# mumianyuxin/M3DSSD

Hardware: AMD Instinct MI355X
Metric: images/sec at 1280x384 bs=8, 1/2/4/8 MI355X; 3D-box Linf vs ref (higher is better)
Workload: dtype f32; 1 GPU; BASELINE.json configs[1]: full M3d_inference_align (DLA-34 + DCNv2 align + ANAB) forward + decode + top-3000 + NMS, bs=8/GPU, 1280x384, fp32, random-init synthetic weights and frames; per_gpu_batch=8, global_batch=8, parallelism=dp1 (batch sharded, 1 all-gather of [B,40,14] detections)

## Files before the change

### include/m3dssd_hip.h

```cpp
#ifndef M3DSSD_HIP_H
#define M3DSSD_HIP_H

#include <stdint.h>

#ifdef __cplusplus
extern "C" {
#endif

typedef void *m3d_stream_t;

enum {
    M3D_OK = 0,
    M3D_E_ARG = -1,
    M3D_E_HIP = -2,
    M3D_E_WORKSPACE = -3
};

const char *m3d_last_error(void);
#define M3D_ABI_VERSION 5
int m3d_abi_version(void);
const char *m3d_source_hashes(void);

typedef struct m3d_conv_desc {
    const float *in;
    int in_cs;
    int N, H, W, Cin;
    const float *wgt;
    long long wgt_img_stride;
    int Cout, Cout_pad;
    int kh, kw, stride, pad, dil;
    int Ho, Wo;
    float *out;
    int out_cs;
    int out_nchw;
    long long out_img_stride;
    const float *scale;
    const float *shift;
    const float *res;
    int res_cs;
    int res_mode;
    int act;
    int sigmoid_from;
    const float *dcn_offmask;
    int dcn_om_cs;
    float *splitk_ws;
    long long splitk_ws_bytes;
} m3d_conv_desc;

int m3d_conv2d_forward(const m3d_conv_desc *d, m3d_stream_t stream);
int m3d_conv2d_splitk_plan(const m3d_conv_desc *d, int *splits, long long *ws_bytes);

int m3d_conv_wave_applicable(const m3d_conv_desc *d);
int m3d_conv_wave_splitk_plan(const m3d_conv_desc *d, int *splits, long long *ws_bytes);
int m3d_conv_wave_forward(const m3d_conv_desc *d, m3d_stream_t stream);
int m3d_conv_wave_forward_wgsplit(const m3d_conv_desc *d, m3d_stream_t stream);
int m3d_conv_wave_wgsplit_width(const m3d_conv_desc *d, int *slices, int *width);

int m3d_wino_conv3x3_forward(const m3d_conv_desc *d, m3d_stream_t stream);
int m3d_wino_conv3x3_variant(const m3d_conv_desc *d);
int m3d_wino_conv3x3_splitk_plan(const m3d_conv_desc *d, int *splits, long long *ws_bytes);
int m3d_wino_conv3x3_forward_ex(const m3d_conv_desc *d, int variant, m3d_stream_t stream);
int m3d_wino44_applicable(const m3d_conv_desc *d);
int m3d_wino44_conv3x3_forward(const m3d_conv_desc *d, m3d_stream_t stream);
int m3d_wino44_conv3x3_forward_ex(const m3d_conv_desc *d, int nb, m3d_stream_t stream);
int m3d_wino44_kpair(const m3d_conv_desc *d);
int m3d_wino44_splitk_plan(const m3d_conv_desc *d, int *splits, long long *ws_bytes);
int m3d_wino44_conv3x3_forward_touch(const m3d_conv_desc *d, int nb, const void *touch, long long touch_bytes, m3d_stream_t stream);

int m3d_cache_touch(const void *p, long long bytes, m3d_stream_t stream);
int m3d_upload_indirect(const void *const *src_slot, void *dst, long long bytes, m3d_stream_t stream);

int m3d_conv2d_tile(const m3d_conv_desc *d, int *bm, int *bn, int *bk, int *grid);

typedef struct m3d_conv_bf16_desc {
    const void *in;
    int in_cs;
    int N, H, W, Cin;
    const void *wgt;
    long long wgt_img_stride;
    int Cout, Cout_pad, Kpad;
    int kh, kw, stride, pad;
    int Ho, Wo;
    void *out;
    int out_cs;
    int out_mode;
    long long out_img_stride;
    const float *scale;
    const float *shift;
    const void *res;
    int res_cs;
    int res_mode;
    int act;
    int sigmoid_from;
    const float *dcn_offmask;
    int dcn_om_cs;
    int groups;
    long long in_group_off, wgt_group_off, out_group_off;
    int ss_group_off;
    const void *wgt_f16;
    void *dcn_ws;
    long long dcn_ws_bytes;
    const void *wgt_wave;
} m3d_conv_bf16_desc;
int m3d_conv_bf16_forward(const m3d_conv_bf16_desc *d, m3d_stream_t stream);
long long m3d_conv_bf16_dcn_ws_bytes(int N, int Ho, int Wo);
int m3d_conv_bf16_variant(const m3d_conv_bf16_desc *d);

typedef struct m3d_tree_entry_bf16_desc {
    const void *in;
    int in_cs, N, H, W, Cin, Cout;
    const void *wfrag;
    const float *shift1, *shiftp;
    void *t; int t_cs;
    void *res; int res_cs;
    void *bottom; int bottom_cs;
} m3d_tree_entry_bf16_desc;
int m3d_tree_entry_bf16_applicable(const m3d_tree_entry_bf16_desc *d);
int m3d_tree_entry_bf16_forward(const m3d_tree_entry_bf16_desc *d, m3d_stream_t stream);

typedef struct m3d_head_bf16_desc {
    const void *in;
    int in_cs;
    long long M;
    int Cin;
    const void *w1, *w2, *w3;
    const float *s1, *t1, *s2, *t2, *s3, *t3;
    int Cout, Cout_pad;
    float *out;
    long long out_group_off, out_img_stride;
    int HW;
    int groups;
} m3d_head_bf16_desc;
int m3d_head_mlp_bf16_forward(const m3d_head_bf16_desc *d, m3d_stream_t stream);
typedef struct m3d_head2_bf16_desc {
    const void *in;
    int in_cs;
    long long M;
    const void *w1f, *w2f, *w3;
    const float *t1, *t2, *t3;
    int Cout;
    float *out;
    long long out_group_off, out_img_stride;
    int HW;
    int groups;
} m3d_head2_bf16_desc;
int m3d_head_mlp2_bf16_forward(const m3d_head2_bf16_desc *d, m3d_stream_t stream);
int m3d_head_mlp2_bf16_forward_rows(const m3d_head2_bf16_desc *d, const int *rows, const int *n_rows, m3d_stream_t stream);
typedef struct m3d_tail2_bf16_desc {
    const void *in;
    int in_cs;
    long long M;
    const void *waf, *wbf;
    const float *t1, *t2;
    int Cout;
    float *out;
    long long out_img_stride;
    int HW;
} m3d_tail2_bf16_desc;
int m3d_head_tail2_bf16_forward(const m3d_tail2_bf16_desc *d, m3d_stream_t stream);
typedef struct m3d_qkvs_bf16_desc {
    const void *in;
    int in_cs;
    long long M;
    const void *wf;
    void *q; int q_cs, q_rows;
    void *kv; int kv_cs, kv_rows;
    float *s; int s_cs, s_rows;
} m3d_qkvs_bf16_desc;
int m3d_anab_qkvs_bf16_forward(const m3d_qkvs_bf16_desc *d, m3d_stream_t stream);

int m3d_stem_conv7x7_bf16(const void *img, int is_u8, int img_h, int img_w, const float *mean3, const float *stds3,
                          const float *wgt, const float *scale, const float *shift, void *out, int out_cs, int N, int H, int W,
                          m3d_stream_t stream);
int m3d_frontend2_bf16_forward(const void *img, int is_u8, int img_h, int img_w, const float *mean3, const float *stds3,
                               const void *w_stem_frag, const float *t_stem, const void *w_l0, const float *t_l0,
                               const void *w_l1, const float *t_l1, void *out, int out_cs, int N, int H, int W,
                               m3d_stream_t stream);
int m3d_anab_attend_bf16(const void *q, int q_cs, const void *khat, const void *vhatT, int B, int HW, int Ck_pad, int keys,
                         int keys_pad, int Cv, const void *res, int res_cs, const float *scale, const float *shift, int act,
                         void *out, int out_cs, m3d_stream_t stream);
int m3d_anab_attend_bf16_rows(const void *q, int q_cs, const void *khat, const void *vhatT, int B, int HW, int Ck_pad, int keys,
                              int keys_pad, int Cv, const void *res, int res_cs, const float *scale, const float *shift, int act,
                              void *out, int out_cs, const int *rows, const int *n_rows, m3d_stream_t stream);
int m3d_maxpool2x2_bf16(const void *in, int in_cs, void *out, int out_cs, int N, int H, int W, int C, m3d_stream_t stream);
int m3d_upsample2x_add_bf16(const void *in, int in_cs, const float *wgt , const void *skip, int skip_cs,
                            void *out, int out_cs, int N, int H, int W, int C, m3d_stream_t stream);
int m3d_f32_to_bf16(const float *src, void *dst, long long n , m3d_stream_t stream);
int m3d_softmax_rows_bf16(const float *x, int rows, int valid, int cs, void *out, int out_cs, m3d_stream_t stream);

typedef struct m3d_mlp_desc {
    const float *in;
    int in_cs;
    long long M;
    int Cin;
    const float *w1, *s1, *t1;
    const float *w2, *s2, *t2;
    const float *w3, *s3, *t3;
    int Cout, Cout_pad;
    float *out;
    long long out_img_stride;
    int HW;
} m3d_mlp_desc;
int m3d_head_mlp_forward(const m3d_mlp_desc *d, m3d_stream_t stream);
int m3d_head_mlp_forward_batched(const m3d_mlp_desc *d, int n, m3d_stream_t stream);
int m3d_head_mlp_forward_rows(const m3d_mlp_desc *d, int n, const int *rows, const int *n_rows, unsigned int sparse_head_mask,
                              m3d_stream_t stream);

long long m3d_dcn_v2_workspace_bytes(int batch, int channels, int height, int width, int channels_out,
                                     int kernel_h, int kernel_w, int stride, int pad, int dilation);
long long m3d_dcn_v2_workspace_bytes_grouped(int batch, int channels, int height, int width, int channels_out,
                                             int kernel_h, int kernel_w, int stride, int pad, int dilation,
                                             int deformable_group);
int m3d_dcn_v2_forward(const float *input, const float *weight, const float *bias, const float *offset,
                       const float *mask, float *output, int batch, int channels, int height, int width,
                       int channels_out, int kernel_h, int kernel_w, int stride_h, int stride_w, int pad_h,
                       int pad_w, int dilation_h, int dilation_w, int deformable_group, void *workspace,
                       long long workspace_bytes, m3d_stream_t stream);

long long m3d_dcn_v2_backward_workspace_bytes(int batch, int channels, int height, int width, int channels_out,
                                              int kernel_h, int kernel_w, int stride, int pad, int dilation,
                                              int deformable_group);
int m3d_dcn_v2_backward(const float *input, const float *weight, const float *offset, const float *mask,
                        const float *grad_output,
                        float *grad_input, float *grad_offset, float *grad_mask, float *grad_weight, float *grad_bias,
                        int batch, int channels, int height, int width, int channels_out, int kernel_h, int kernel_w,
                        int stride_h, int stride_w, int pad_h, int pad_w, int dilation_h, int dilation_w,
                        int deformable_group, void *workspace, long long workspace_bytes, m3d_stream_t stream);

long long m3d_dcn_v2_workspace_bytes_bf16(int batch, int channels, int height, int width, int channels_out,
                                          int kernel_h, int kernel_w, int stride, int pad, int dilation, int deformable_group);
int m3d_dcn_v2_forward_bf16(const void *input, const void *weight, const float *bias, const void *offset, int offset_is_bf16,
                            const void *mask, int mask_is_bf16, void *output, int batch, int channels, int height, int width,
                            int channels_out, int kernel_h, int kernel_w, int stride_h, int stride_w, int pad_h, int pad_w,
                            int dilation_h, int dilation_w, int deformable_group, void *workspace, long long workspace_bytes,
                            m3d_stream_t stream);
long long m3d_dcn_v2_backward_workspace_bytes_bf16(int batch, int channels, int height, int width, int channels_out,
                                                   int kernel_h, int kernel_w, int stride, int pad, int dilation,
                                                   int deformable_group);
int m3d_dcn_v2_backward_bf16(const void *input, const void *weight, const void *offset, int offset_is_bf16, const void *mask,
                             int mask_is_bf16, const void *grad_output,
                             void *grad_input, float *grad_offset, float *grad_mask, void *grad_weight, float *grad_bias,
                             int batch, int channels, int height, int width, int channels_out, int kernel_h, int kernel_w,
                             int stride_h, int stride_w, int pad_h, int pad_w, int dilation_h, int dilation_w,
                             int deformable_group, void *workspace, long long workspace_bytes, m3d_stream_t stream);

long long m3d_dcn_v2_psroi_pooling_workspace_bytes(int batch, int channels, int height, int width, int num_rois,
                                                   int num_classes, int output_dim, int group_size, int pooled_size,
                                                   int backward);
int m3d_dcn_v2_psroi_pooling_forward(const float *data, const float *rois, const float *trans, float *out, float *top_count,
                                     int batch, int channels, int height, int width, int num_rois, int trans_rows,
                                     int num_classes, int no_trans, float spatial_scale, int output_dim, int group_size,
                                     int pooled_size, int part_size, int sample_per_part, float trans_std, void *workspace,
                                     long long workspace_bytes, m3d_stream_t stream);
int m3d_dcn_v2_psroi_pooling_backward(const float *grad_out, const float *data, const float *rois, const float *trans,
                                      float *grad_data, float *grad_trans, int batch, int channels, int height, int width,
                                      int num_rois, int trans_rows, int num_classes, int no_trans, float spatial_scale,
                                      int output_dim, int group_size, int pooled_size, int part_size, int sample_per_part,
                                      float trans_std, void *workspace, long long workspace_bytes, m3d_stream_t stream);

#define M3D_RPN_MAX_GT 128
#define M3D_RPN_GT_COLS 12
enum {
    M3D_RPN_CONF_MEANS = 0,
    M3D_RPN_CONF_STDS = 11,
    M3D_RPN_CONF_FG_THRESH = 22,
    M3D_RPN_CONF_IGN_THRESH = 23,
    M3D_RPN_CONF_BG_LO = 24,
    M3D_RPN_CONF_BG_HI = 25,
    M3D_RPN_CONF_BEST_THRESH = 26,
    M3D_RPN_CONF_BOX_SAMPLES = 27,
    M3D_RPN_CONF_FG_FRACTION = 28,
    M3D_RPN_CONF_FOCAL = 29,
    M3D_RPN_CONF_LAMBDA_CLS = 30,
    M3D_RPN_CONF_LAMBDA_IOU = 31,
    M3D_RPN_CONF_LAMBDA_2D = 32,
    M3D_RPN_CONF_LAMBDA_3D = 33,
    M3D_RPN_CONF_STRIDE = 34,
    M3D_RPN_CONF_COUNT = 35
};
enum {
    M3D_RPN_STAT_LOSS = 0,
    M3D_RPN_STAT_CLS = 1,
    M3D_RPN_STAT_BBOX_2D = 2,
    M3D_RPN_STAT_BBOX_3D = 3,
    M3D_RPN_STAT_IOU_LOSS = 4,
    M3D_RPN_STAT_Z = 5,
    M3D_RPN_STAT_RY = 6,
    M3D_RPN_STAT_IOU_ACC = 7,
    M3D_RPN_STAT_ACC_FG = 8,
    M3D_RPN_STAT_ACC_BG = 9,
    M3D_RPN_STAT_N_FG = 10,
    M3D_RPN_STAT_N_BG = 11,
    M3D_RPN_STAT_FG_NUM = 12,
    M3D_RPN_STAT_BG_NUM = 13,
    M3D_RPN_STAT_N_ACTIVE = 14,
    M3D_RPN_STAT_FG_WEIGHT = 15,
    M3D_RPN_STAT_COUNT = 16
};
long long m3d_rpn_loss_workspace_bytes(int B, long long R);
int m3d_rpn_targets(const double *anchors, int A, int H, int W, const double *conf, int n_conf, const double *gt_table, int B,
                    int Gmax, const float *cls, const float *prob, int C, short *labels, short *gt_index, float *targets,
                    float *scores, void *workspace, long long workspace_bytes, m3d_stream_t stream);
int m3d_rpn_loss(const double *anchors, int A, int H, int W, const double *conf, int n_conf, const double *gt_table, int B,
                 int Gmax, const float *cls, const float *bbox_2d, const float *bbox_3d, int C, const short *labels,
                 const float *targets, const float *scores, unsigned char *sampled, float *grad_cls, float *grad_bbox_2d,
                 float *grad_bbox_3d, float *loss, double *stats, void *workspace, long long workspace_bytes,
                 m3d_stream_t stream);

enum {
    M3D_RPN_SMP_STAT_BAD_LABELS = 16,
    M3D_RPN_SMP_STAT_COUNT = 17
};
int m3d_rpn_precompute_targets(const double *anchors, int A, int H, int W, const double *conf, int n_conf,
                               const double *gt_table, int B, int Gmax, short *labels, short *gt_index, float *bbox_2d_tar,
                               float *bbox_3d_tar, int *any_val, void *workspace, long long workspace_bytes,
                               m3d_stream_t stream);
int m3d_rpn_loss_smp(const double *anchors, int A, int H, int W, const double *conf, int n_conf, int B, const void *labels_in,
                     int label_bytes, const float *bbox_2d_tar, const float *bbox_3d_tar, const int *any_val, const float *cls,
                     const float *prob, const float *bbox_2d, const float *bbox_3d, int C, short *labels, float *targets,
                     float *scores, unsigned char *sampled, float *grad_cls, float *grad_bbox_2d, float *grad_bbox_3d,
                     float *loss, double *stats, void *workspace, long long workspace_bytes, m3d_stream_t stream);

#define M3D_RPN_TARGET_STATS_COLS 23
long long m3d_rpn_target_stats_workspace_bytes(int B, long long R);
int m3d_rpn_target_stats(const double *anchors, int A, int H, int W, const double *conf, int n_conf, const double *gt_table, int B,
                         int Gmax, const double *center, double *out, void *workspace, long long workspace_bytes,
                         m3d_stream_t stream);

int m3d_pack_conv_weight(const float *w, float *packed, int Cout, int Cout_pad, int Cin, int Cin_pad, int kh,
                         int kw, m3d_stream_t stream);
int m3d_nchw_to_nhwc(const float *in, float *out, int N, int C, int H, int W, int out_cs, m3d_stream_t stream);
int m3d_nhwc_to_nchw(const float *in, int in_cs, float *out, int N, int C, int H, int W, m3d_stream_t stream);

int m3d_stem_conv7x7(const float *img_nchw, const float *wgt , const float *scale,
                     const float *shift, float *out, int out_cs, int N, int H, int W, m3d_stream_t stream);
int m3d_preprocess_u8(const unsigned char *frames_bgr, int N, int img_h, int img_w, const float *mean3, const float *stds3,
                      float *out_nchw, int H, int W, m3d_stream_t stream);
int m3d_stem_conv7x7_u8(const unsigned char *frames_bgr, int img_h, int img_w, const float *mean3, const float *stds3,
                        const float *wgt, const float *scale, const float *shift, float *out, int out_cs, int N, int H, int W,
                        m3d_stream_t stream);
#define M3D_AUGMENT_PARAMS 14
int m3d_augment_u8(const unsigned char *frames_bgr, int N, int hmax, int wmax, const double *params, int param_stride,
                   const float *mean3, const float *stds3, float *out_nchw, int H, int W, m3d_stream_t stream);
int m3d_conv3x3_c16(const float *in, int in_cs, const float *wgt, const float *scale, const float *shift, float *out,
                    int out_cs, int N, int H, int W, m3d_stream_t stream);
int m3d_conv3x3_c16_wino(const float *in, int in_cs, const float *U, const float *scale, const float *shift, float *out,
                         int out_cs, int N, int H, int W, m3d_stream_t stream);
int m3d_maxpool2x2(const float *in, int in_cs, float *out, int out_cs, int N, int H, int W, int C,
                   m3d_stream_t stream);
int m3d_upsample2x_add(const float *in, int in_cs, const float *wgt, const float *skip, int skip_cs,
                       float *out, int out_cs, int N, int H, int W, int C, m3d_stream_t stream);

int m3d_anchor_select(const float *cls_planar, int B, int A, int num_classes, int HW, int *sel_idx,
                      float *sel_prob, float *fg_all, m3d_stream_t stream);
int m3d_anchor_select_keys(const float *cls_planar, int B, int A, int HW, int *sel_idx, float *sel_prob,
                           unsigned int *score_bits, m3d_stream_t stream);
int m3d_fg_top1(const float *prob, int B, int A, int HW, int *idx, float *val, m3d_stream_t stream);
int m3d_align_offsets(int mode, const int *sel_idx, const float *sel_prob, float thresh, const float *table,
                      const float *bbox_x, const float *bbox_y, const float *anchor_wh, float mean_x,
                      float std_x, float mean_y, float std_y, float *offmask, int om_cs, int B, int A, int HW,
                      int kk, long long box_img_stride, m3d_stream_t stream);
int m3d_align_offsets_gated(const int *sel_idx, const float *sel_prob, float thresh, const float *bbox_x, const float *bbox_y,
                            const float *anchor_wh, float mean_x, float std_x, float mean_y, float std_y,
                            const unsigned char *need, float *offmask, int om_cs, int B, int A, int HW,
                            long long box_img_stride, m3d_stream_t stream);

int m3d_anab_pool_partial(const float *kv, int kv_cs, const float *s, int s_cs, const int *items, int n_items,
                          const int *bin_scale, int n_bins, float *partial, int max_slots, int B, int H, int W,
                          int C, m3d_stream_t stream);
int m3d_anab_pool_finish(const float *partial, const int *bin_slots, const float *bin_inv_area, int n_bins,
                         int max_slots, int Ck, int Cv, float *khat, int keys_pad, int ck_pad, float *vhatT,
                         int B, int frag, m3d_stream_t stream);
long long m3d_anab_pool_nested_scratch_bytes(int B, int C);
int m3d_anab_pool_nested(const float *kv, int kv_cs, const float *s, int s_cs, int B, int H, int W, int Ck, int Cv,
                         float *scratch, float *khat, int keys_pad, int ck_pad, float *vhatT, int frag, m3d_stream_t stream);
int m3d_anab_pool_nested_bf16(const void *kv, int kv_cs, const float *s, int s_cs, int B, int H, int W, int Ck, int Cv,
                              float *scratch, float *khat, int keys_pad, int ck_pad, float *vhatT, int frag, m3d_stream_t stream);
int m3d_anab_pool_nested_bf16_ex(const void *kv, int kv_cs, const float *s, int s_cs, int B, int H, int W, int Ck, int Cv,
                                 float *scratch, float *khat, int keys_pad, int ck_pad, float *vhatT, int frag,
                                 void *khat16, void *vhat16, m3d_stream_t stream);
int m3d_anab_attend_f32(const float *q, int q_cs, const float *khat, int k_cs, const float *vhatT, int B, int HW, int Ck,
                        int keys, int keys_pad, int Cv, const float *res, int res_cs, int res_mode, const float *scale,
                        const float *shift, int act, float *out, int out_cs, m3d_stream_t stream);
int m3d_anab_attend_f32_rows(const float *q, int q_cs, const float *khat, int k_cs, const float *vhatT, int B, int HW, int Ck,
                             int keys, int keys_pad, int Cv, const float *res, int res_cs, int res_mode, const float *scale,
                             const float *shift, int act, float *out, int out_cs, const int *rows, const int *n_rows,
                             m3d_stream_t stream);
long long m3d_anab_attention_workspace_bytes(int B, int H, int W, int Ck, int Cv, int backward);
int m3d_anab_attention_forward(const float *q, const float *k, const float *v, const float *g, float *out, int B, int H, int W, int Ck,
                               int Cv, int q_cs, int k_cs, int v_cs, int g_cs, int out_cs, void *workspace, long long workspace_bytes,
                               m3d_stream_t stream);
int m3d_anab_attention_backward(const float *q, const float *k, const float *v, const float *g, const float *grad_out, float *grad_q,
                                float *grad_k, float *grad_v, float *grad_g, int B, int H, int W, int Ck, int Cv, int q_cs, int k_cs,
                                int v_cs, int g_cs, int go_cs, int gq_cs, int gk_cs, int gv_cs, int gg_cs, void *workspace,
                                long long workspace_bytes, m3d_stream_t stream);
long long m3d_anab_attention_workspace_bytes_bf16(int B, int H, int W, int Ck, int Cv, int backward);
int m3d_anab_attention_forward_bf16(const void *q, const void *k, const void *v, const void *g, void *out, int B, int H, int W, int Ck,
                                    int Cv, int q_cs, int k_cs, int v_cs, int g_cs, int out_cs, void *workspace,
                                    long long workspace_bytes, m3d_stream_t stream);
int m3d_anab_attention_backward_bf16(const void *q, const void *k, const void *v, const void *g, const void *grad_out, void *grad_q,
                                     void *grad_k, void *grad_v, void *grad_g, int B, int H, int W, int Ck, int Cv, int q_cs, int k_cs,
                                     int v_cs, int g_cs, int go_cs, int gq_cs, int gk_cs, int gv_cs, int gg_cs, void *workspace,
                                     long long workspace_bytes, m3d_stream_t stream);
int m3d_softmax_rows(float *x, int rows, int valid, int cs, m3d_stream_t stream);

int m3d_bundle_outputs(const float *cls_planar, const float *box_planar, float *cls, float *prob, float *bbox_2d,
                       float *bbox_3d, unsigned int *score_bits, int B, int A, int HW, m3d_stream_t stream);
int m3d_score_keys_planar(const float *cls_planar, unsigned int *score_bits, int B, int A, int HW, m3d_stream_t stream);
long long m3d_topk_decode_workspace_bytes(int B, int R);
int m3d_topk_decode(const unsigned int *score_bits, const float *prob, const float *bbox_2d, const float *bbox_3d,
                    const float *rois , const float *anchors , const float *means ,
                    const float *stds , float *aboxes, int *rows_out, void *workspace, long long workspace_bytes,
                    int B, int R, int k, m3d_stream_t stream);
int m3d_topk_decode_scaled(const unsigned int *score_bits, const float *prob, const float *bbox_2d, const float *bbox_3d,
                           const float *rois, const float *anchors, const float *means, const float *stds, const float *scale,
                           float *aboxes, int *rows_out, void *workspace, long long workspace_bytes, int B, int R, int k,
                           m3d_stream_t stream);
int m3d_topk_decode_planar(const unsigned int *score_bits, const float *cls_planar, const float *box_planar, const float *rois,
                           const float *anchors, const float *means, const float *stds, const float *scale, float *aboxes,
                           int *rows_out, void *workspace, long long workspace_bytes, int B, int A, int HW, int k,
                           m3d_stream_t stream);
long long m3d_topk_decode_mw_workspace_bytes(int B, int R, int k);
int m3d_topk_decode_planar_mw(const unsigned int *score_bits, const float *cls_planar, const float *box_planar, const float *rois,
                              const float *anchors, const float *means, const float *stds, const float *scale, float *aboxes,
                              int *rows_out, void *workspace, long long workspace_bytes, int B, int A, int HW, int k,
                              int wgs_per_image, m3d_stream_t stream);
long long m3d_need_rows_workspace_bytes(int B, int HW);
int m3d_need_rows(const unsigned int *score_bits, int B, int A, int HW, int k, unsigned int *thresh, unsigned char *need,
                  int *rows, int *n_rows, void *workspace, long long workspace_bytes, m3d_stream_t stream);
int m3d_decode_rows(const long long *rows , const float *prob, const float *bbox_2d,
                    const float *bbox_3d, const float *rois , const float *anchors ,
                    const float *means , const float *stds , float *aboxes, int B, int R,
                    int n_rows, m3d_stream_t stream);

long long m3d_nms_workspace_bytes(int B, int n);
int m3d_nms_sorted_dev(const float *boxes_dev, int B, int n, int box_stride, float thresh, void *mask_ws,
                       int *keep_dev, int *num_keep_dev, m3d_stream_t stream);
int m3d_select_post(const float *aboxes , const int *keep , const int *num_keep , int B, int n,
                    int post, float *block, int *counts, m3d_stream_t stream);
void _nms(int *keep_out, int *num_out, const float *boxes_host, int boxes_num, int boxes_dim,
          float nms_overlap_thresh, int device_id);

int m3d_refine_3d(const float *aboxes, const int *counts, int B, int K, const double *p2, const double *p2_inv,
                  double score_thresh, int hill_climbing, double step_r_init, double r_lim, double *out, m3d_stream_t stream);
int m3d_refine_3d_ex(const float *aboxes, const int *counts, int B, int K, const double *p2, const double *p2_inv,
                     const float *scale, const float *clip_wh, double score_thresh, int hill_climbing, double step_r_init,
                     double r_lim, double *out, m3d_stream_t stream);
int m3d_refine_3d_host(const float *aboxes, const int *counts, int B, int K, const double *p2, const double *p2_inv,
                       const float *scale, const float *clip_wh, double score_thresh, int hill_climbing, double step_r_init,
                       double r_lim, double *out);

int m3d_rotate_iou_eval(const float *boxes_dev, int N, const float *qboxes_dev, int K, int criterion, float *iou_dev,
                        m3d_stream_t stream);
int m3d_eval_image_box_overlap(const double *boxes, int N, const double *q, int K, int criterion, double *out);
int m3d_eval_d3_overlap(const double *boxes, int N, const double *qboxes, int K, double *rinc, int criterion);
int m3d_eval_statistics(const double *overlaps, long long ov_stride, const double *gt_datas, int gt_size, const double *dt_datas,
                        int det_size, const long long *ignored_gt, const long long *ignored_det, const double *dc_bboxes, int n_dc,
                        int metric, double min_overlap, double thresh, int compute_fp, int compute_aos, double *stats,
                        double *thresholds_out, int *n_thresholds);
int m3d_eval_fused_statistics(const double *overlaps, long long ov_stride, double *pr, const long long *gt_nums,
                              const long long *dt_nums, const long long *dc_nums, int n_images, const double *gt_datas,
                              const double *dt_datas, const double *dontcares, const long long *ignored_gts,
                              const long long *ignored_dets, int metric, double min_overlap, const double *thresholds,
                              int n_thresholds, int compute_aos);

int m3d_clock_probe(long long *out4_dev, double seconds, m3d_stream_t stream);
int m3d_event_create(void **ev);
int m3d_event_record(void *ev, m3d_stream_t stream);
int m3d_event_elapsed_ms(void *start, void *stop, float *ms);
int m3d_event_destroy(void *ev);

#ifdef __cplusplus
}
#endif
#endif
```

### m3dssd_amd/_hip.py

```python
import ctypes
import os
import subprocess

_HERE = os.path.dirname(os.path.abspath(__file__))
CSRC = os.path.join(_HERE, "csrc")
SO_PATH = os.environ.get("M3D_HIP_LIB") or os.path.join(CSRC, "build", "libm3dssd_hip.so")
HEADER = os.path.join(os.path.dirname(_HERE), "include", "m3dssd_hip.h")

c_int, c_float, c_ll, c_void_p = ctypes.c_int, ctypes.c_float, ctypes.c_longlong, ctypes.c_void_p


class ConvDesc(ctypes.Structure):
    _fields_ = [
        ("inp", c_void_p), ("in_cs", c_int),
        ("N", c_int), ("H", c_int), ("W", c_int), ("Cin", c_int),
        ("wgt", c_void_p), ("wgt_img_stride", c_ll),
        ("Cout", c_int), ("Cout_pad", c_int),
        ("kh", c_int), ("kw", c_int), ("stride", c_int), ("pad", c_int), ("dil", c_int),
        ("Ho", c_int), ("Wo", c_int),
        ("out", c_void_p), ("out_cs", c_int), ("out_nchw", c_int), ("out_img_stride", c_ll),
        ("scale", c_void_p), ("shift", c_void_p),
        ("res", c_void_p), ("res_cs", c_int), ("res_mode", c_int),
        ("act", c_int), ("sigmoid_from", c_int),
        ("dcn_offmask", c_void_p), ("dcn_om_cs", c_int),
        ("splitk_ws", c_void_p), ("splitk_ws_bytes", c_ll),
    ]


class MlpDesc(ctypes.Structure):
    _fields_ = [
        ("inp", c_void_p), ("in_cs", c_int), ("M", c_ll), ("Cin", c_int),
        ("w1", c_void_p), ("s1", c_void_p), ("t1", c_void_p),
        ("w2", c_void_p), ("s2", c_void_p), ("t2", c_void_p),
        ("w3", c_void_p), ("s3", c_void_p), ("t3", c_void_p),
        ("Cout", c_int), ("Cout_pad", c_int),
        ("out", c_void_p), ("out_img_stride", c_ll), ("HW", c_int),
    ]


class ConvBf16Desc(ctypes.Structure):
    _fields_ = [
        ("inp", c_void_p), ("in_cs", c_int),
        ("N", c_int), ("H", c_int), ("W", c_int), ("Cin", c_int),
        ("wgt", c_void_p), ("wgt_img_stride", c_ll),
        ("Cout", c_int), ("Cout_pad", c_int), ("Kpad", c_int),
        ("kh", c_int), ("kw", c_int), ("stride", c_int), ("pad", c_int),
        ("Ho", c_int), ("Wo", c_int),
        ("out", c_void_p), ("out_cs", c_int), ("out_mode", c_int), ("out_img_stride", c_ll),
        ("scale", c_void_p), ("shift", c_void_p),
        ("res", c_void_p), ("res_cs", c_int), ("res_mode", c_int),
        ("act", c_int), ("sigmoid_from", c_int),
        ("dcn_offmask", c_void_p), ("dcn_om_cs", c_int),
        ("groups", c_int),
        ("in_group_off", c_ll), ("wgt_group_off", c_ll), ("out_group_off", c_ll),
        ("ss_group_off", c_int),
        ("wgt_f16", c_void_p), ("dcn_ws", c_void_p), ("dcn_ws_bytes", c_ll),
        ("wgt_wave", c_void_p),
    ]


class HeadBf16Desc(ctypes.Structure):
    _fields_ = [
        ("inp", c_void_p), ("in_cs", c_int), ("M", c_ll), ("Cin", c_int),
        ("w1", c_void_p), ("w2", c_void_p), ("w3", c_void_p),
        ("s1", c_void_p), ("t1", c_void_p), ("s2", c_void_p), ("t2", c_void_p), ("s3", c_void_p), ("t3", c_void_p),
        ("Cout", c_int), ("Cout_pad", c_int),
        ("out", c_void_p), ("out_group_off", c_ll), ("out_img_stride", c_ll),
        ("HW", c_int), ("groups", c_int),
    ]


class Head2Bf16Desc(ctypes.Structure):
    _fields_ = [
        ("inp", c_void_p), ("in_cs", c_int), ("M", c_ll),
        ("w1f", c_void_p), ("w2f", c_void_p), ("w3", c_void_p),
        ("t1", c_void_p), ("t2", c_void_p), ("t3", c_void_p),
        ("Cout", c_int),
        ("out", c_void_p), ("out_group_off", c_ll), ("out_img_stride", c_ll),
        ("HW", c_int), ("groups", c_int),
    ]


class Tail2Bf16Desc(ctypes.Structure):
    _fields_ = [
        ("inp", c_void_p), ("in_cs", c_int), ("M", c_ll),
        ("waf", c_void_p), ("wbf", c_void_p), ("t1", c_void_p), ("t2", c_void_p),
        ("Cout", c_int),
        ("out", c_void_p), ("out_img_stride", c_ll),
        ("HW", c_int),
    ]


class TreeEntryBf16Desc(ctypes.Structure):
    _fields_ = [
        ("inp", c_void_p), ("in_cs", c_int), ("N", c_int), ("H", c_int), ("W", c_int), ("Cin", c_int), ("Cout", c_int),
        ("wfrag", c_void_p), ("shift1", c_void_p), ("shiftp", c_void_p),
        ("t", c_void_p), ("t_cs", c_int), ("res", c_void_p), ("res_cs", c_int), ("bottom", c_void_p), ("bottom_cs", c_int),
    ]


class QkvsBf16Desc(ctypes.Structure):
    _fields_ = [
        ("inp", c_void_p), ("in_cs", c_int), ("M", c_ll), ("wf", c_void_p),
        ("q", c_void_p), ("q_cs", c_int), ("q_rows", c_int),
        ("kv", c_void_p), ("kv_cs", c_int), ("kv_rows", c_int),
        ("s", c_void_p), ("s_cs", c_int), ("s_rows", c_int),
    ]


P = c_void_p
SIGNATURES = {
    "m3d_last_error": (ctypes.c_char_p, []),
    "m3d_abi_version": (c_int, []),
    "m3d_source_hashes": (ctypes.c_char_p, []),
    "m3d_conv2d_forward": (c_int, [ctypes.POINTER(ConvDesc), P]),
    "m3d_conv_bf16_forward": (c_int, [ctypes.POINTER(ConvBf16Desc), P]),
    "m3d_conv_bf16_dcn_ws_bytes": (c_ll, [c_int, c_int, c_int]),
    "m3d_conv_bf16_variant": (c_int, [ctypes.POINTER(ConvBf16Desc)]),
    "m3d_head_mlp_bf16_forward": (c_int, [ctypes.POINTER(HeadBf16Desc), P]),
    "m3d_head_mlp2_bf16_forward": (c_int, [ctypes.POINTER(Head2Bf16Desc), P]),
    "m3d_head_mlp2_bf16_forward_rows": (c_int, [ctypes.POINTER(Head2Bf16Desc), P, P, P]),
    "m3d_tree_entry_bf16_applicable": (c_int, [ctypes.POINTER(TreeEntryBf16Desc)]),
    "m3d_tree_entry_bf16_forward": (c_int, [ctypes.POINTER(TreeEntryBf16Desc), P]),
    "m3d_anab_qkvs_bf16_forward": (c_int, [ctypes.POINTER(QkvsBf16Desc), P]),
    "m3d_head_tail2_bf16_forward": (c_int, [ctypes.POINTER(Tail2Bf16Desc), P]),
    "m3d_stem_conv7x7_bf16": (c_int, [P, c_int, c_int, c_int, ctypes.POINTER(ctypes.c_float), ctypes.POINTER(ctypes.c_float),
                                      P, P, P, P, c_int, c_int, c_int, c_int, P]),
    "m3d_frontend2_bf16_forward": (c_int, [P, c_int, c_int, c_int, ctypes.POINTER(ctypes.c_float), ctypes.POINTER(ctypes.c_float)]
                                   + [P] * 7 + [c_int] * 4 + [P]),
    "m3d_anab_attend_bf16": (c_int, [P, c_int, P, P, c_int, c_int, c_int, c_int, c_int, c_int, P, c_int, P, P, c_int, P, c_int, P]),
    "m3d_anab_attend_bf16_rows": (c_int, [P, c_int, P, P, c_int, c_int, c_int, c_int, c_int, c_int, P, c_int, P, P, c_int, P, c_int,
                                          P, P, P]),
    "m3d_maxpool2x2_bf16": (c_int, [P, c_int, P, c_int] + [c_int] * 4 + [P]),
    "m3d_upsample2x_add_bf16": (c_int, [P, c_int, P, P, c_int, P, c_int] + [c_int] * 4 + [P]),
    "m3d_f32_to_bf16": (c_int, [P, P, c_ll, P]),
    "m3d_softmax_rows_bf16": (c_int, [P, c_int, c_int, c_int, P, c_int, P]),
    "m3d_head_mlp_forward": (c_int, [ctypes.POINTER(MlpDesc), P]),
    "m3d_head_mlp_forward_batched": (c_int, [ctypes.POINTER(MlpDesc), c_int, P]),
    "m3d_head_mlp_forward_rows": (c_int, [ctypes.POINTER(MlpDesc), c_int, P, P, ctypes.c_uint, P]),
    "m3d_wino_conv3x3_forward": (c_int, [ctypes.POINTER(ConvDesc), P]),
    "m3d_wino_conv3x3_forward_ex": (c_int, [ctypes.POINTER(ConvDesc), c_int, P]),
    "m3d_wino_conv3x3_splitk_plan": (c_int, [ctypes.POINTER(ConvDesc), ctypes.POINTER(c_int), ctypes.POINTER(c_ll)]),
    "m3d_wino_conv3x3_variant": (c_int, [ctypes.POINTER(ConvDesc)]),
    "m3d_wino44_applicable": (c_int, [ctypes.POINTER(ConvDesc)]),
    "m3d_wino44_conv3x3_forward": (c_int, [ctypes.POINTER(ConvDesc), P]),
    "m3d_wino44_conv3x3_forward_ex": (c_int, [ctypes.POINTER(ConvDesc), c_int, P]),
    "m3d_wino44_kpair": (c_int, [ctypes.POINTER(ConvDesc)]),
    "m3d_wino44_conv3x3_forward_touch": (c_int, [ctypes.POINTER(ConvDesc), c_int, P, c_ll, P]),
    "m3d_cache_touch": (c_int, [P, c_ll, P]),
    "m3d_upload_indirect": (c_int, [P, P, c_ll, P]),
    "m3d_wino44_splitk_plan": (c_int, [ctypes.POINTER(ConvDesc), ctypes.POINTER(c_int), ctypes.POINTER(c_ll)]),
    "m3d_conv_wave_applicable": (c_int, [ctypes.POINTER(ConvDesc)]),
    "m3d_conv_wave_splitk_plan": (c_int, [ctypes.POINTER(ConvDesc), ctypes.POINTER(c_int), ctypes.POINTER(c_ll)]),
    "m3d_conv_wave_forward": (c_int, [ctypes.POINTER(ConvDesc), P]),
    "m3d_conv_wave_forward_wgsplit": (c_int, [ctypes.POINTER(ConvDesc), P]),
    "m3d_conv_wave_wgsplit_width": (c_int, [ctypes.POINTER(ConvDesc), ctypes.POINTER(c_int), ctypes.POINTER(c_int)]),
    "m3d_conv2d_tile": (c_int, [ctypes.POINTER(ConvDesc)] + [ctypes.POINTER(c_int)] * 4),
    "m3d_conv2d_splitk_plan": (c_int, [ctypes.POINTER(ConvDesc), ctypes.POINTER(c_int), ctypes.POINTER(c_ll)]),
    "m3d_dcn_v2_workspace_bytes": (c_ll, [c_int] * 10),
    "m3d_dcn_v2_workspace_bytes_grouped": (c_ll, [c_int] * 11),
    "m3d_dcn_v2_forward": (c_int, [P] * 6 + [c_int] * 14 + [P, c_ll, P]),
    "m3d_dcn_v2_backward_workspace_bytes": (c_ll, [c_int] * 11),
    "m3d_dcn_v2_backward": (c_int, [P] * 10 + [c_int] * 14 + [P, c_ll, P]),
    "m3d_dcn_v2_workspace_bytes_bf16": (c_ll, [c_int] * 11),
    "m3d_dcn_v2_forward_bf16": (c_int, [P, P, P, P, c_int, P, c_int, P] + [c_int] * 14 + [P, c_ll, P]),
    "m3d_dcn_v2_backward_workspace_bytes_bf16": (c_ll, [c_int] * 11),
    "m3d_dcn_v2_backward_bf16": (c_int, [P, P, P, c_int, P, c_int, P] + [P] * 5 + [c_int] * 14 + [P, c_ll, P]),
    "m3d_dcn_v2_psroi_pooling_workspace_bytes": (c_ll, [c_int] * 10),
    "m3d_dcn_v2_psroi_pooling_forward": (c_int, [P] * 5 + [c_int] * 8 + [c_float] + [c_int] * 5 + [c_float, P, c_ll, P]),
    "m3d_dcn_v2_psroi_pooling_backward": (c_int, [P] * 6 + [c_int] * 8 + [c_float] + [c_int] * 5 + [c_float, P, c_ll, P]),
    "m3d_rpn_loss_workspace_bytes": (c_ll, [c_int, c_ll]),
    "m3d_rpn_targets": (c_int, [P, c_int, c_int, c_int, P, c_int, P, c_int, c_int, P, P, c_int, P, P, P, P, P, c_ll, P]),
    "m3d_rpn_loss": (c_int, [P, c_int, c_int, c_int, P, c_int, P, c_int, c_int, P, P, P, c_int, P, P, P, P, P, P, P, P, P, P, c_ll, P]),
    "m3d_rpn_precompute_targets": (c_int, [P, c_int, c_int, c_int, P, c_int, P, c_int, c_int, P, P, P, P, P, P, c_ll, P]),
    "m3d_rpn_loss_smp": (c_int, [P, c_int, c_int, c_int, P, c_int, c_int, P, c_int, P, P, P, P, P, P, P, c_int] + [P] * 10 + [c_ll, P]),
    "m3d_rpn_target_stats_workspace_bytes": (c_ll, [c_int, c_ll]),
    "m3d_rpn_target_stats": (c_int, [P, c_int, c_int, c_int, P, c_int, P, c_int, c_int, P, P, P, c_ll, P]),
    "m3d_pack_conv_weight": (c_int, [P, P] + [c_int] * 6 + [P]),
    "m3d_nchw_to_nhwc": (c_int, [P, P] + [c_int] * 5 + [P]),
    "m3d_nhwc_to_nchw": (c_int, [P, c_int, P] + [c_int] * 4 + [P]),
    "m3d_stem_conv7x7": (c_int, [P, P, P, P, P] + [c_int] * 4 + [P]),
    "m3d_refine_3d": (c_int, [P, P, c_int, c_int, P, P, ctypes.c_double, c_int, ctypes.c_double, ctypes.c_double, P, P]),
    "m3d_refine_3d_ex": (c_int, [P, P, c_int, c_int, P, P, P, P, ctypes.c_double, c_int, ctypes.c_double, ctypes.c_double, P, P]),
    "m3d_refine_3d_host": (c_int, [P, P, c_int, c_int, P, P, P, P, ctypes.c_double, c_int, ctypes.c_double, ctypes.c_double, P]),
    "m3d_preprocess_u8": (c_int, [P, c_int, c_int, c_int, ctypes.POINTER(ctypes.c_float), ctypes.POINTER(ctypes.c_float), P, c_int,
                                  c_int, P]),
    "m3d_augment_u8": (c_int, [P, c_int, c_int, c_int, ctypes.POINTER(ctypes.c_double), c_int, ctypes.POINTER(ctypes.c_float),
                               ctypes.POINTER(ctypes.c_float), P, c_int, c_int, P]),
    "m3d_stem_conv7x7_u8": (c_int, [P, c_int, c_int, ctypes.POINTER(ctypes.c_float), ctypes.POINTER(ctypes.c_float), P, P, P, P,
                                    c_int, c_int, c_int, c_int, P]),
    "m3d_conv3x3_c16": (c_int, [P, c_int, P, P, P, P, c_int, c_int, c_int, c_int, P]),
    "m3d_conv3x3_c16_wino": (c_int, [P, c_int, P, P, P, P, c_int, c_int, c_int, c_int, P]),
    "m3d_maxpool2x2": (c_int, [P, c_int, P, c_int] + [c_int] * 4 + [P]),
    "m3d_upsample2x_add": (c_int, [P, c_int, P, P, c_int, P, c_int] + [c_int] * 4 + [P]),
    "m3d_anchor_select": (c_int, [P] + [c_int] * 4 + [P, P, P, P]),
    "m3d_anchor_select_keys": (c_int, [P] + [c_int] * 3 + [P, P, P, P]),
    "m3d_fg_top1": (c_int, [P, c_int, c_int, c_int, P, P, P]),
    "m3d_align_offsets": (c_int, [c_int, P, P, c_float, P, P, P, P] + [c_float] * 4 + [P] + [c_int] * 5 + [c_ll, P]),
    "m3d_align_offsets_gated": (c_int, [P, P, c_float, P, P, P] + [c_float] * 4 + [P, P] + [c_int] * 4 + [c_ll, P]),
    "m3d_anab_pool_partial": (c_int, [P, c_int, P, c_int, P, c_int, P, c_int, P] + [c_int] * 5 + [P]),
    "m3d_anab_pool_finish": (c_int, [P, P, P] + [c_int] * 4 + [P, c_int, c_int, P, c_int, c_int, P]),
    "m3d_anab_pool_nested_scratch_bytes": (c_ll, [c_int, c_int]),
    "m3d_anab_pool_nested": (c_int, [P, c_int, P, c_int, c_int, c_int, c_int, c_int, c_int, P, P, c_int, c_int, P, c_int, P]),
    "m3d_anab_attend_f32": (c_int, [P, c_int, P, c_int, P, c_int, c_int, c_int, c_int, c_int, c_int, P, c_int, c_int, P, P, c_int, P, c_int, P]),
    "m3d_anab_attend_f32_rows": (c_int, [P, c_int, P, c_int, P, c_int, c_int, c_int, c_int, c_int, c_int, P, c_int, c_int, P, P, c_int, P, c_int,
                                         P, P, P]),
    "m3d_anab_pool_nested_bf16": (c_int, [P, c_int, P, c_int, c_int, c_int, c_int, c_int, c_int, P, P, c_int, c_int, P, c_int, P]),
    "m3d_anab_pool_nested_bf16_ex": (c_int, [P, c_int, P, c_int, c_int, c_int, c_int, c_int, c_int, P, P, c_int, c_int, P, c_int, P, P, P]),
    "m3d_anab_attention_workspace_bytes": (c_ll, [c_int] * 6),
    "m3d_anab_attention_forward": (c_int, [P] * 5 + [c_int] * 10 + [P, c_ll, P]),
    "m3d_anab_attention_backward": (c_int, [P] * 9 + [c_int] * 14 + [P, c_ll, P]),
    "m3d_anab_attention_workspace_bytes_bf16": (c_ll, [c_int] * 6),
    "m3d_anab_attention_forward_bf16": (c_int, [P] * 5 + [c_int] * 10 + [P, c_ll, P]),
    "m3d_anab_attention_backward_bf16": (c_int, [P] * 9 + [c_int] * 14 + [P, c_ll, P]),
    "m3d_softmax_rows": (c_int, [P, c_int, c_int, c_int, P]),
    "m3d_bundle_outputs": (c_int, [P] * 7 + [c_int] * 3 + [P]),
    "m3d_decode_rows": (c_int, [P] * 9 + [c_int] * 3 + [P]),
    "m3d_topk_decode_workspace_bytes": (c_ll, [c_int, c_int]),
    "m3d_topk_decode": (c_int, [P] * 11 + [c_ll] + [c_int] * 3 + [P]),
    "m3d_topk_decode_scaled": (c_int, [P] * 12 + [c_ll] + [c_int] * 3 + [P]),
    "m3d_score_keys_planar": (c_int, [P, P, c_int, c_int, c_int, P]),
    "m3d_topk_decode_planar": (c_int, [P] * 11 + [c_ll] + [c_int] * 4 + [P]),
    "m3d_topk_decode_mw_workspace_bytes": (c_ll, [c_int, c_int, c_int]),
    "m3d_need_rows_workspace_bytes": (c_ll, [c_int, c_int]),
    "m3d_need_rows": (c_int, [P] + [c_int] * 4 + [P] * 5 + [c_ll, P]),
    "m3d_topk_decode_planar_mw": (c_int, [P] * 11 + [c_ll] + [c_int] * 5 + [P]),
    "m3d_select_post": (c_int, [P] * 3 + [c_int] * 3 + [P, P, P]),
    "m3d_nms_workspace_bytes": (c_ll, [c_int, c_int]),
    "m3d_nms_sorted_dev": (c_int, [P, c_int, c_int, c_int, c_float, P, P, P, P]),
    "_nms": (None, [P, P, P, c_int, c_int, c_float, c_int]),
    "m3d_rotate_iou_eval": (c_int, [P, c_int, P, c_int, c_int, P, P]),
    "m3d_eval_image_box_overlap": (c_int, [P, c_int, P, c_int, c_int, P]),
    "m3d_eval_d3_overlap": (c_int, [P, c_int, P, c_int, P, c_int]),
    "m3d_eval_statistics": (c_int, [P, c_ll, P, c_int, P, c_int, P, P, P, c_int, c_int, ctypes.c_double, ctypes.c_double,
                                    c_int, c_int, P, P, ctypes.POINTER(c_int)]),
    "m3d_eval_fused_statistics": (c_int, [P, c_ll, P, P, P, P, c_int, P, P, P, P, P, c_int, ctypes.c_double, P, c_int, c_int]),
    "m3d_clock_probe": (c_int, [P, ctypes.c_double, P]),
    "m3d_event_create": (c_int, [ctypes.POINTER(c_void_p)]),
    "m3d_event_record": (c_int, [P, P]),
    "m3d_event_elapsed_ms": (c_int, [P, P, ctypes.POINTER(c_float)]),
    "m3d_event_destroy": (c_int, [P]),
}

_lib = None


def build(force=False, verbose=False):
    jobs = min(16, int(os.environ.get("MAX_JOBS") or 0) or os.cpu_count() or 4)
    cmd = ["make", "-C", CSRC, "-j", str(jobs)] + (["-B"] if force else [])
    res = subprocess.run(cmd, stdout=subprocess.PIPE, stderr=subprocess.STDOUT, text=True)
    if verbose or res.returncode != 0:
        print(res.stdout)
    if res.returncode != 0:
        raise RuntimeError("building libm3dssd_hip.so failed")
    return SO_PATH


def lib():
    global _lib
    if _lib is None:
        if not os.path.exists(SO_PATH):
            raise RuntimeError(
                "libm3dssd_hip.so is missing (%s): run `python -c 'import __graft_entry__ as g; g.build()'`; "
                "there is no non-HIP fallback for the M3DSSD hot path" % SO_PATH)
        import torch
        L = ctypes.CDLL(SO_PATH)
        for name, (res, args) in SIGNATURES.items():
            fn = getattr(L, name)
            fn.restype, fn.argtypes = res, args
        _lib = L
    return _lib


def lib_source_hashes():
    txt = lib().m3d_source_hashes().decode()
    return dict(item.split(":", 1) for item in txt.split(";") if item)


def tree_source_hashes():
    import hashlib
    files = [os.path.join(CSRC, f) for f in sorted(os.listdir(CSRC)) if f.endswith(".hip") or f.endswith(".h")] + [HEADER]
    return {os.path.basename(f): hashlib.sha256(open(f, "rb").read()).hexdigest()[:16] for f in files}


def check(status):
    if status != 0:
        raise RuntimeError("m3dssd_hip error %d: %s" % (status, lib().m3d_last_error().decode()))
```

### m3dssd_amd/csrc/common.h

```cpp
#pragma once
#include <hip/hip_runtime.h>
#include <stdarg.h>
#include <stdio.h>

#include <algorithm>

#include "m3dssd_hip.h"
#include "per_device.h"

typedef float f32x4 __attribute__((ext_vector_type(4)));
typedef float f32x16 __attribute__((ext_vector_type(16)));
typedef float f32x2 __attribute__((ext_vector_type(2)));
typedef unsigned u32x4 __attribute__((ext_vector_type(4)));

__device__ __forceinline__ int sign_smear(int x)
{
    int m;
    asm("v_ashrrev_i32 %0, 31, %1" : "=v"(m) : "v"(x));
    return m;
}
__device__ __forceinline__ void dcn_corners(float h_im, float w_im, int H, int W, int drop_all, float (&w)[4], int (&o)[4],
                                            int (&drop)[4])
{
    const float tin = fminf(fminf(h_im, w_im) + 1.f, -fmaxf(h_im - (float)H, w_im - (float)W));
    const unsigned xin = __float_as_uint(tin);
    const unsigned nonfinite = __float_as_uint((h_im - h_im) + (w_im - w_im)) & 0x7fffffffu;
    const int out = sign_smear((int)((xin - 1u) | xin)) | sign_smear(-(int)nonfinite) | drop_all;
    const int hl = (int)floorf(h_im), wl = (int)floorf(w_im);
    const float lh = h_im - (float)hl, lw = w_im - (float)wl;
    const float uh = 1.f - lh, uw = 1.f - lw;
    const int hr = (int)((unsigned)(H - 2) - (unsigned)hl), wr = (int)((unsigned)(W - 2) - (unsigned)wl);
    drop[0] = sign_smear(hl | wl) | out;
    drop[1] = sign_smear(hl | wr) | out;
    drop[2] = sign_smear(hr | wl) | out;
    drop[3] = sign_smear(hr | wr) | out;
    const unsigned row0 = (unsigned)__mul24(hl, W) + (unsigned)wl, row1 = row0 + (unsigned)W;
    o[0] = (int)row0; o[1] = (int)(row0 + 1u); o[2] = (int)row1; o[3] = (int)(row1 + 1u);
    const float wf[4] = {uh * uw, uh * lw, lh * uw, lh * lw};
#pragma unroll
    for (int q = 0; q < 4; ++q) w[q] = __uint_as_float(__float_as_uint(wf[q]) & ~(unsigned)drop[q]);
}

#define M3D_BUF_OOB 0x80000000u
__device__ __forceinline__ __amdgpu_buffer_rsrc_t make_rsrc(const void *base, unsigned bytes)
{
    return __builtin_amdgcn_make_buffer_rsrc(const_cast<void *>(base), 0, bytes, 0x00020000);
}
__device__ __forceinline__ void buf_store_f32x4_nop(f32x4 v, __amdgpu_buffer_rsrc_t r, unsigned voffset, unsigned soffset)
{
    asm volatile("buffer_store_dwordx4 %0, %1, %2, %3 offen\n\ts_nop 1" : : "v"(v), "v"(voffset), "s"(r), "s"(soffset) : "memory");
}
__device__ __forceinline__ void global_store_u32x4_nop(void *p, u32x4 v)
{
    asm volatile("global_store_dwordx4 %0, %1, off\n\ts_nop 1" : : "v"(p), "v"(v) : "memory");
}

__device__ __forceinline__ f32x4 buf_load_f32x4(__amdgpu_buffer_rsrc_t r, unsigned voffset, unsigned soffset)
{
    return __builtin_bit_cast(f32x4, __builtin_amdgcn_raw_buffer_load_b128(r, voffset, soffset, 0));
}
__device__ __forceinline__ f32x2 pk_sub2(f32x2 a, f32x2 b)
{
    f32x2 r;
    asm("v_pk_add_f32 %0, %1, %2 neg_lo:[0,1] neg_hi:[0,1]" : "=v"(r) : "v"(a), "v"(b));
    return r;
}
__device__ __forceinline__ f32x4 pk_sub(f32x4 a, f32x4 b)
{
    const f32x2 lo = pk_sub2(__builtin_shufflevector(a, a, 0, 1), __builtin_shufflevector(b, b, 0, 1));
    const f32x2 hi = pk_sub2(__builtin_shufflevector(a, a, 2, 3), __builtin_shufflevector(b, b, 2, 3));
    return __builtin_shufflevector(lo, hi, 0, 1, 2, 3);
}
__device__ __forceinline__ f32x4 pk_mul_s(float w, f32x4 x)
{
    const f32x2 w2 = {w, w};
    const f32x2 lo = w2 * __builtin_shufflevector(x, x, 0, 1), hi = w2 * __builtin_shufflevector(x, x, 2, 3);
    return __builtin_shufflevector(lo, hi, 0, 1, 2, 3);
}
__device__ __forceinline__ f32x4 pk_fma_s(float w, f32x4 x, f32x4 c)
{
    const f32x2 w2 = {w, w};
    const f32x2 lo = __builtin_elementwise_fma(w2, __builtin_shufflevector(x, x, 0, 1), __builtin_shufflevector(c, c, 0, 1));
    const f32x2 hi = __builtin_elementwise_fma(w2, __builtin_shufflevector(x, x, 2, 3), __builtin_shufflevector(c, c, 2, 3));
    return __builtin_shufflevector(lo, hi, 0, 1, 2, 3);
}
__device__ __forceinline__ f32x4 pk_add(f32x4 a, f32x4 b)
{
    const f32x2 lo = __builtin_shufflevector(a, a, 0, 1) + __builtin_shufflevector(b, b, 0, 1);
    const f32x2 hi = __builtin_shufflevector(a, a, 2, 3) + __builtin_shufflevector(b, b, 2, 3);
    return __builtin_shufflevector(lo, hi, 0, 1, 2, 3);
}

#define M3D_LEAKY_SLOPE 0.01f

void m3d_set_error(const char *fmt, ...);
int m3d_nchw_to_nhwc_slice(const float *in, int Ctot, int c0, float *out, int N, int C, int H, int W, int out_cs, m3d_stream_t stream);
int m3d_pack_conv_weight_slice(const float *w, int Ctot, int c0, float *packed, int Cout, int Cout_pad, int Cin, int Cin_pad, int kh,
                               int kw, m3d_stream_t stream);

#define M3D_REQUIRE(cond, ...)        \
    do {                              \
        if (!(cond)) {                \
            m3d_set_error(__VA_ARGS__); \
            return M3D_E_ARG;         \
        }                             \
    } while (0)

#define M3D_HIP(call)                                                             \
    do {                                                                          \
        hipError_t e__ = (call);                                                  \
        if (e__ != hipSuccess) {                                                  \
            m3d_set_error("%s failed: %s (%s:%d)", #call, hipGetErrorString(e__), \
                          __FILE__, __LINE__);                                    \
            return M3D_E_HIP;                                                     \
        }                                                                         \
    } while (0)

#define M3D_LAUNCH_CHECK()                                                          \
    do {                                                                            \
        hipError_t e__ = hipGetLastError();                                         \
        if (e__ != hipSuccess) {                                                    \
            m3d_set_error("kernel launch failed: %s (%s:%d)", hipGetErrorString(e__), \
                          __FILE__, __LINE__);                                      \
            return M3D_E_HIP;                                                       \
        }                                                                           \
    } while (0)

typedef PerDevice<int> m3d_lds_state;
int m3d_raise_dyn_lds_(const void *kernel, int bytes, m3d_lds_state &state, const char *what, const char *file, int line);
#define m3d_raise_dyn_lds(kernel, bytes, state) \
    m3d_raise_dyn_lds_(reinterpret_cast<const void *>(kernel), bytes, state, #kernel, __FILE__, __LINE__)
int m3d_cu_count();
int m3d_scratch_bytes_(const void *const *kernels, int n);
template <typename... K>
static inline int m3d_scratch_bytes(K... kernels)
{
    const void *const k[] = {reinterpret_cast<const void *>(kernels)...};
    return m3d_scratch_bytes_(k, (int)sizeof...(K));
}
int m3d_env_int(const char *name, int dflt);
static inline int m3d_knob_ablate() { static const int v = m3d_env_int("M3D_ABLATE", 0); return v; }

static inline int cdiv(long long a, long long b) { return (int)((a + b - 1) / b); }
static inline int imin(int a, int b) { return a < b ? a : b; }

__device__ __forceinline__ float leaky(float v) { return fmaxf(v, v * M3D_LEAKY_SLOPE); }
__device__ __forceinline__ float sigmoidf_(float v) { return 1.0f / (1.0f + expf(-v)); }

template <typename T>
__device__ __forceinline__ T conv_epi_affine(T v, T sc, T sh, T rv, bool has_res, int res_mode)
{
    if (has_res) return res_mode ? (v + rv) * sc + sh : v * sc + sh + rv;
    return v * sc + sh;
}
__device__ __forceinline__ float conv_epi_act(float v, bool sig, float slope) { return sig ? sigmoidf_(v) : fmaxf(v, v * slope); }
__device__ __forceinline__ f32x4 conv_epi_act4(f32x4 v, int c0, int sigmoid_from, bool any_sig, float slope)
{
    if (any_sig) {
#pragma unroll
        for (int e = 0; e < 4; ++e) v[e] = conv_epi_act(v[e], c0 + e >= sigmoid_from, slope);
        return v;
    }
    return __builtin_elementwise_max(v, v * slope);
}

__device__ __forceinline__ f32x4 class_softmax4(f32x4 l)
{
    const float mx = fmaxf(fmaxf(l[0], l[1]), fmaxf(l[2], l[3]));
    f32x4 e;
    float s = 0.f;
#pragma unroll
    for (int c = 0; c < 4; ++c) { e[c] = expf(l[c] - mx); s += e[c]; }
    f32x4 pr;
#pragma unroll
    for (int c = 0; c < 4; ++c) pr[c] = e[c] / s;
    return pr;
}
__device__ __forceinline__ float fg_score(f32x4 pr) { return fmaxf(fmaxf(pr[1], pr[2]), pr[3]); }
__device__ __forceinline__ unsigned int f32_sortable(float f)
{
    unsigned int u = __float_as_uint(f);
    return (u & 0x80000000u) ? ~u : (u | 0x80000000u);
}

__device__ __forceinline__ int rows_lower_bound(const int *rows, const int n, const int target)
{
    const int lane = threadIdx.x & 63;
    int lo = 0, len = n;
    while (len > 0) {
        const int step = (len + 63) >> 6;
        const int idx = lo + (lane + 1) * step - 1;
        const bool less = idx < lo + len && rows[idx] < target;
        const int c = __popcll(__ballot(less));
        const int end = lo + len;
        lo += c * step;
        len = min(step - 1, end - lo);
    }
    return __builtin_amdgcn_readfirstlane(lo);
}

struct SplitkReduceArgs {
    const float *ws, *scale, *shift, *res;
    float *out;
    int M, Cout, Cout_pad, splits, out_cs, res_cs, res_mode, act, sigmoid_from;
};
int m3d_launch_splitk_reduce(const SplitkReduceArgs &a, hipStream_t stream);
```

### m3dssd_amd/csrc/dcn_wave.hip

```cpp

#include <type_traits>

#include "common.h"

struct ConvWaveArgs {
    const float *in, *wfrag, *scale, *shift, *res, *om;
    float *out;
    int in_cs, out_cs, res_cs, om_cs;
    int H, W, Cin, Ho, Wo, HoWo, Cout;
    int kh, kw, stride, pad, dil;
    int M, KG, tiles_n;
    int act, res_mode, sigmoid_from;
    int vec_out;
    long long w_img_stride;
    unsigned in_bytes, out_bytes, res_bytes, w_bytes;
    float *ws;
    int splits, ss_per, base_waves;
    unsigned ws_bytes;
#ifdef CONV_TRACE
    long long *trace;
#endif
};


#ifdef CONV_TRACE
static long long *g_conv_trace = nullptr;
extern "C" void m3d_conv_wave_set_trace(void *buf) { g_conv_trace = (long long *)buf; }
static int g_conv_variant = 0;
extern "C" void m3d_conv_wave_set_variant(int v) { g_conv_variant = v; }
#define TRACE_INIT() long long *trp = (a.trace && threadIdx.x < 64) ? a.trace + (size_t)blockIdx.x * 128 : nullptr; int tri = 0
#define TRACE() do { if (trp && lane == 0 && tri < 128) trp[tri++] = __builtin_readcyclecounter(); } while (0)
#else
#define TRACE_INIT()
#define TRACE()
#endif

template <bool DEFORM, int NT, int NCQ = 4, int WPE = (DEFORM ? 2 : 3), int S = 1>
__global__ __launch_bounds__(64 * S) __attribute__((amdgpu_waves_per_eu(WPE))) void conv_wave_kernel(const ConvWaveArgs a)
{
    __shared__ __attribute__((aligned(16))) float tileS[S * 32 * 32];
    __shared__ __attribute__((aligned(16))) float tapst[(DEFORM ? 9 : 1) * 32 * 8];
    const int lane = threadIdx.x & 63, l31 = lane & 31, h = lane >> 5;
    const int wv = S > 1 ? __builtin_amdgcn_readfirstlane((int)threadIdx.x >> 6) : 0;
    float *const tileA = tileS + wv * 1024;
    const int gp = lane >> 3, gc = lane & 7;
    TRACE_INIT();
    TRACE();
    int blk;
    {
        const int nblk = gridDim.x, bid = blockIdx.x;
        const int q = nblk >> 3, r = nblk & 7, xcd = bid & 7, loc = bid >> 3;
        blk = (xcd < r ? xcd * (q + 1) : r * (q + 1) + (xcd - r) * q) + loc;
    }
    int split = wv;
    if (S == 1 && a.splits > 1) {
        split = blk / a.base_waves;
        blk -= split * a.base_waves;
    }
    const int bm = blk / a.tiles_n, bn = blk - bm * a.tiles_n;
    const int m0 = bm * 32;
    const int KK = a.kh * a.kw, C32 = a.Cin / 32;
    const bool idle = S > 1 && wv >= a.splits;
    const int ss0 = idle ? 0 : split * a.ss_per, ss1 = idle ? 0 : min(KK * C32, ss0 + a.ss_per);

    const __amdgpu_buffer_rsrc_t rin = make_rsrc(a.in, a.in_bytes);
    const __amdgpu_buffer_rsrc_t rw =
        make_rsrc(a.wfrag + (size_t)(m0 / a.HoWo) * a.w_img_stride + (size_t)bn * NT * a.KG * 256, a.w_bytes);
    const unsigned wlane = (unsigned)lane * 16u;
    const unsigned wstride = (unsigned)a.KG * 1024u;

    int o_pix = 0, o_hi0 = 0, o_wi0 = 0;
    bool o_valid = false;
    int o_inv = -1;
    const float *o_om = a.om;
    int g_pix[4], g_hi0[4], g_wi0[4];
    bool g_valid[4];
    {
        const int m = m0 + l31;
        o_valid = m < a.M;
        o_inv = sign_smear(a.M - 1 - m);
        const int mm = o_valid ? m : 0;
        const int n = mm / a.HoWo, rem = mm - n * a.HoWo;
        const int ho = rem / a.Wo, wo = rem - ho * a.Wo;
        o_pix = n * a.H * a.W;
        o_hi0 = ho * a.stride - a.pad;
        o_wi0 = wo * a.stride - a.pad;
        if (DEFORM) o_om = a.om + (size_t)mm * a.om_cs;
    }
    if constexpr (!DEFORM) {
#pragma unroll
        for (int g = 0; g < 4; ++g) {
            const int m = m0 + 8 * g + gp;
            g_valid[g] = m < a.M;
            const int mm = g_valid[g] ? m : 0;
            const int n = mm / a.HoWo, rem = mm - n * a.HoWo;
            const int ho = rem / a.Wo, wo = rem - ho * a.Wo;
            g_pix[g] = n * a.H * a.W;
            g_hi0[g] = ho * a.stride - a.pad;
            g_wi0[g] = wo * a.stride - a.pad;
        }
    }

    unsigned doff[4][DEFORM ? 4 : 1];
    float bw[DEFORM ? 4 : 1][4];
    if constexpr (DEFORM) {
        constexpr int TPW = (9 + S - 1) / S;
        float raws[TPW][3];
#pragma unroll
        for (int i = 0; i < TPW; ++i) {
            const int tp = min(wv + i * S, KK - 1);
            raws[i][0] = o_om[2 * tp];
            raws[i][1] = o_om[2 * tp + 1];
            raws[i][2] = o_om[2 * KK + tp];
        }
#pragma unroll
        for (int i = 0; i < TPW; ++i) {
            const int t = wv + i * S;
            if (t < KK) {
                const int ti = t / a.kw, tj = t - ti * a.kw;
                const float mk = raws[i][2];
                const float h_im = (float)(o_hi0 + ti * a.dil) + raws[i][0];
                const float w_im = (float)(o_wi0 + tj * a.dil) + raws[i][1];
                float wq[4];
                int oq[4], drop[4];
                dcn_corners(h_im, w_im, a.H, a.W, o_inv, wq, oq, drop);
                u32x4 ob;
#pragma unroll
                for (int q = 0; q < 4; ++q) {
                    const unsigned off = ((unsigned)o_pix + (unsigned)oq[q]) * (unsigned)a.in_cs * 4u;
                    ob[q] = (off & ~(unsigned)drop[q]) | (M3D_BUF_OOB & (unsigned)drop[q]);
                }
                if (h == 0) {
                    *reinterpret_cast<u32x4 *>(&tapst[t * 256 + l31 * 8]) = ob;
                    *reinterpret_cast<f32x4 *>(&tapst[t * 256 + l31 * 8 + 4]) = f32x4{wq[0] * mk, wq[1] * mk, wq[2] * mk, wq[3] * mk};
                }
            }
        }
        if constexpr (S > 1) __syncthreads();
    }
    auto setup_tap = [&](int tap) {
        if constexpr (DEFORM) {
#pragma unroll
            for (int g = 0; g < 4; ++g) {
                const u32x4 ov = *reinterpret_cast<const u32x4 *>(&tapst[tap * 256 + (8 * g + gp) * 8]);
                const f32x4 wv = *reinterpret_cast<const f32x4 *>(&tapst[tap * 256 + (8 * g + gp) * 8 + 4]);
#pragma unroll
                for (int q = 0; q < 4; ++q) {
                    doff[g][q] = ov[q] + (unsigned)gc * 16u;
                    bw[g][q] = wv[q];
                }
            }
        } else {
            const int ti = tap / a.kw, tj = tap - ti * a.kw;
#pragma unroll
            for (int g = 0; g < 4; ++g) {
                const int hi = g_hi0[g] + ti * a.dil, wi = g_wi0[g] + tj * a.dil;
                const bool ok = g_valid[g] && hi >= 0 && hi < a.H && wi >= 0 && wi < a.W;
                doff[g][0] = ok ? ((unsigned)(g_pix[g] + hi * a.W + wi) * (unsigned)a.in_cs + (unsigned)gc * 4u) * 4u
                                : M3D_BUF_OOB;
            }
        }
    };

    constexpr int NC = DEFORM ? NCQ : 1;
    f32x4 cr[4][NC];
    f32x4 bfA[NT], bfB[NT];
    auto issue_gather = [&](int c32) {
#pragma unroll
        for (int g = 0; g < 4; ++g)
#pragma unroll
            for (int q = 0; q < NC; ++q) cr[g][q] = buf_load_f32x4(rin, doff[g][q], (unsigned)c32 * 128u);
    };
    auto issue_b = [&](int kg, f32x4 (&bf)[NT]) {
        const unsigned bsoff = (unsigned)min(kg, a.KG - 1) * 1024u;
#pragma unroll
        for (int nt = 0; nt < NT; ++nt) bf[nt] = buf_load_f32x4(rw, wlane, bsoff + nt * wstride);
    };

    f32x16 acc[NT];
#pragma unroll
    for (int nt = 0; nt < NT; ++nt)
#pragma unroll
        for (int r = 0; r < 16; ++r) acc[nt][r] = 0.f;

    int tap, c32;
    constexpr bool cmaj = DEFORM;
    if constexpr (cmaj) { c32 = ss0 / KK; tap = ss0 - c32 * KK; }
    else { tap = ss0 / C32; c32 = ss0 - tap * C32; }
    setup_tap(tap);
    issue_gather(c32);
    issue_b((tap * C32 + c32) * 4, bfA);

    unsigned wr_off[4], rd_off[4];
#pragma unroll
    for (int g = 0; g < 4; ++g) {
        const int r = 8 * g + gp;
        wr_off[g] = (unsigned)(r * 32 + ((gc ^ ((r >> 1) & 7)) * 4));
    }
#pragma unroll
    for (int j = 0; j < 4; ++j) rd_off[j] = (unsigned)(l31 * 32 + (((2 * j + h) ^ ((l31 >> 1) & 7)) * 4));

    TRACE();
    for (int st = ss0; st < ss1; ++st) {
        TRACE();
        const int kg0 = (tap * C32 + c32) * 4;
#pragma unroll
        for (int g = 0; g < 4; ++g) {
            f32x4 v;
            if constexpr (DEFORM && NCQ == 4)
                v = pk_fma_s(bw[g][0], cr[g][0], pk_fma_s(bw[g][1], cr[g][1], pk_fma_s(bw[g][2], cr[g][2], pk_mul_s(bw[g][3], cr[g][3]))));
            else if constexpr (DEFORM && NCQ == 2)
                v = pk_fma_s(bw[g][0], cr[g][0], pk_mul_s(bw[g][1], cr[g][1]));
            else if constexpr (DEFORM)
                v = pk_mul_s(bw[g][0], cr[g][0]);
            else
                v = cr[g][0];
            *reinterpret_cast<f32x4 *>(&tileA[wr_off[g]]) = v;
        }
        if constexpr (cmaj) {
            if (++tap == KK) { tap = 0; ++c32; }
            setup_tap(tap);
            issue_gather(min(c32, C32 - 1));
        } else {
            if (++c32 == C32) {
                c32 = 0;
                ++tap;
                setup_tap(min(tap, KK - 1));
            }
            issue_gather(c32);
        }
        const int kgn = (min(tap, KK - 1) * C32 + min(c32, C32 - 1)) * 4;
        TRACE();
        f32x4 A[4];
#pragma unroll
        for (int j = 0; j < 4; ++j) A[j] = *reinterpret_cast<const f32x4 *>(&tileA[rd_off[j]]);
        __builtin_amdgcn_sched_barrier(0);
        auto group = [&](int j, int kg_next, f32x4 (&bf)[NT], f32x4 (&bfn)[NT]) {
            issue_b(kg_next, bfn);
            __builtin_amdgcn_sched_barrier(0);
#pragma unroll
            for (int t = 0; t < 4; ++t)
#pragma unroll
                for (int nt = 0; nt < NT; ++nt)
                    acc[nt] = __builtin_amdgcn_mfma_f32_32x32x2f32(A[j][t], bf[nt][t], acc[nt], 0, 0, 0);
            __builtin_amdgcn_sched_barrier(0);
        };
        group(0, kg0 + 1, bfA, bfB);
        group(1, kg0 + 2, bfB, bfA);
        group(2, kg0 + 3, bfA, bfB);
        group(3, kgn, bfB, bfA);
    }

    TRACE();
    const __amdgpu_buffer_rsrc_t rout = make_rsrc(a.out, a.out_bytes);
    const __amdgpu_buffer_rsrc_t rres = make_rsrc(a.res ? a.res : a.out, a.res ? a.res_bytes : 0u);
    const int n0 = bn * 32 * NT;
    const int mb = m0 + 4 * h;
    if constexpr (S > 1) {
        constexpr int Q = S == 2 ? 2 : 1;
        const int tid = threadIdx.x;
        const bool worker = S < 8 || wv < 4;
        const float slope = a.act == 1 ? M3D_LEAKY_SLOPE : 1.f;
        const int c4 = lane & 7;
        int px[Q];
        unsigned oq[Q], rq[Q];
#pragma unroll
        for (int q = 0; q < Q; ++q) {
            px[q] = ((tid + q * 64 * S) >> 3) & 31;
            const int m = m0 + px[q];
            const bool ok = worker && m < a.M;
            oq[q] = ok ? (unsigned)m * (unsigned)a.out_cs * 4u : M3D_BUF_OOB;
            rq[q] = ok ? (unsigned)m * (unsigned)a.res_cs * 4u : M3D_BUF_OOB;
        }
        f32x4 scv[NT], shv[NT];
#pragma unroll
        for (int nt = 0; nt < NT; ++nt) {
            const int c = n0 + nt * 32 + 4 * c4;
            scv[nt] = f32x4{1.f, 1.f, 1.f, 1.f};
            shv[nt] = f32x4{0.f, 0.f, 0.f, 0.f};
            if (a.vec_out && c + 3 < a.Cout) {
                if (a.scale) scv[nt] = *reinterpret_cast<const f32x4 *>(a.scale + c);
                if (a.shift) shv[nt] = *reinterpret_cast<const f32x4 *>(a.shift + c);
            } else {
#pragma unroll
                for (int e = 0; e < 4; ++e)
                    if (c + e < a.Cout) {
                        if (a.scale) scv[nt][e] = a.scale[c + e];
                        if (a.shift) shv[nt][e] = a.shift[c + e];
                    }
            }
        }
#pragma unroll
        for (int nt = 0; nt < NT; ++nt) {
            const int c = n0 + nt * 32 + 4 * c4;
            const bool full = a.vec_out && c + 3 < a.Cout;
            f32x4 rv[Q];
            if (a.res) {
#pragma unroll
                for (int q = 0; q < Q; ++q) {
                    if (full) {
                        rv[q] = __builtin_bit_cast(f32x4, __builtin_amdgcn_raw_buffer_load_b128(rres, rq[q] + (unsigned)c * 4u, 0, 0));
                    } else {
#pragma unroll
                        for (int e = 0; e < 4; ++e)
                            rv[q][e] = __builtin_bit_cast(float, __builtin_amdgcn_raw_buffer_load_b32(
                                rres, c + e < a.Cout ? rq[q] + (unsigned)(c + e) * 4u : M3D_BUF_OOB, 0, 0));
                    }
                }
            }
            if (nt) __syncthreads();
#pragma unroll
            for (int r = 0; r < 16; ++r) tileA[((r & 3) + 8 * (r >> 2) + 4 * h) * 32 + l31] = acc[nt][r];
            __syncthreads();
            if (worker) {
                const bool tile_sig = a.sigmoid_from >= 0 && n0 + nt * 32 + 31 >= a.sigmoid_from;
#pragma unroll
                for (int q = 0; q < Q; ++q) {
                    const float *p = &tileS[px[q] * 32 + 4 * c4];
                    f32x4 v = *reinterpret_cast<const f32x4 *>(p);
#pragma unroll
                    for (int s = 1; s < S; ++s)
                        if (s < a.splits) v = v + *reinterpret_cast<const f32x4 *>(p + s * 1024);
                    v = conv_epi_affine(v, scv[nt], shv[nt], a.res ? rv[q] : v, a.res != nullptr, a.res_mode);
                    v = conv_epi_act4(v, c, a.sigmoid_from, tile_sig, slope);
                    if (full) {
                        __builtin_amdgcn_raw_buffer_store_b128(__builtin_bit_cast(u32x4, v), rout, oq[q] + (unsigned)c * 4u, 0, 0);
                    } else {
#pragma unroll
                        for (int e = 0; e < 4; ++e) {
                            const float pe = v[e];
                            __builtin_amdgcn_raw_buffer_store_b32(__builtin_bit_cast(unsigned, pe), rout,
                                                                  c + e < a.Cout ? oq[q] + (unsigned)(c + e) * 4u : M3D_BUF_OOB, 0, 0);
                        }
                    }
                }
            }
        }
        TRACE();
        return;
    }
    if (a.splits > 1) {
        const __amdgpu_buffer_rsrc_t rws = make_rsrc(a.ws, a.ws_bytes);
        const unsigned sbase = (unsigned)split * (unsigned)a.M;
        const unsigned cpad = (unsigned)(a.tiles_n * 32 * NT);
#pragma unroll
        for (int nt = 0; nt < NT; ++nt) {
            const unsigned co = (unsigned)(n0 + nt * 32 + l31);
#pragma unroll
            for (int r = 0; r < 16; ++r) {
                const int m = mb + (r & 3) + 8 * (r >> 2);
                const unsigned oo = m < a.M ? ((sbase + (unsigned)m) * cpad + co) * 4u : M3D_BUF_OOB;
                const float pv = acc[nt][r];
                __builtin_amdgcn_raw_buffer_store_b32(__builtin_bit_cast(unsigned, pv), rws, oo, 0, 0);
            }
        }
        return;
    }
    if (a.vec_out) {
        const float slope = a.act == 1 ? M3D_LEAKY_SLOPE : 1.f;
        const int pr = lane >> 3, c4 = lane & 7;
        unsigned oq[4], rq[4];
#pragma unroll
        for (int q = 0; q < 4; ++q) {
            const int m = m0 + pr + 8 * q;
            oq[q] = m < a.M ? (unsigned)m * (unsigned)a.out_cs * 4u : M3D_BUF_OOB;
            rq[q] = m < a.M ? (unsigned)m * (unsigned)a.res_cs * 4u : M3D_BUF_OOB;
        }
        f32x4 scv[NT], shv[NT];
#pragma unroll
        for (int nt = 0; nt < NT; ++nt) {
            const int c = n0 + nt * 32 + 4 * c4;
            scv[nt] = f32x4{1.f, 1.f, 1.f, 1.f};
            shv[nt] = f32x4{0.f, 0.f, 0.f, 0.f};
            if (c + 3 < a.Cout) {
                if (a.scale) scv[nt] = *reinterpret_cast<const f32x4 *>(a.scale + c);
                if (a.shift) shv[nt] = *reinterpret_cast<const f32x4 *>(a.shift + c);
            } else {
#pragma unroll
                for (int e = 0; e < 4; ++e)
                    if (c + e < a.Cout) {
                        if (a.scale) scv[nt][e] = a.scale[c + e];
                        if (a.shift) shv[nt][e] = a.shift[c + e];
                    }
            }
        }
#pragma unroll
        for (int nt = 0; nt < NT; ++nt) {
            const int c = n0 + nt * 32 + 4 * c4;
            f32x4 rv[4];
            if (a.res) {
#pragma unroll
                for (int q = 0; q < 4; ++q) {
                    if (c + 3 < a.Cout) {
                        rv[q] = __builtin_bit_cast(f32x4, __builtin_amdgcn_raw_buffer_load_b128(rres, rq[q] + (unsigned)c * 4u, 0, 0));
                    } else {
#pragma unroll
                        for (int e = 0; e < 4; ++e)
                            rv[q][e] = __builtin_bit_cast(float, __builtin_amdgcn_raw_buffer_load_b32(
                                rres, c + e < a.Cout ? rq[q] + (unsigned)(c + e) * 4u : M3D_BUF_OOB, 0, 0));
                    }
                }
            }
#pragma unroll
            for (int r = 0; r < 16; ++r) tileA[((r & 3) + 8 * (r >> 2) + 4 * h) * 32 + l31] = acc[nt][r];
            const bool tile_sig = a.sigmoid_from >= 0 && n0 + nt * 32 + 31 >= a.sigmoid_from;
#pragma unroll
            for (int q = 0; q < 4; ++q) {
                f32x4 v = *reinterpret_cast<const f32x4 *>(&tileA[(pr + 8 * q) * 32 + 4 * c4]);
                v = conv_epi_affine(v, scv[nt], shv[nt], a.res ? rv[q] : v, a.res != nullptr, a.res_mode);
                v = conv_epi_act4(v, c, a.sigmoid_from, tile_sig, slope);
                if (c + 3 < a.Cout) {
                    __builtin_amdgcn_raw_buffer_store_b128(__builtin_bit_cast(u32x4, v), rout, oq[q] + (unsigned)c * 4u, 0, 0);
                } else {
#pragma unroll
                    for (int e = 0; e < 4; ++e) {
                        const float pe = v[e];
                        __builtin_amdgcn_raw_buffer_store_b32(__builtin_bit_cast(unsigned, pe), rout,
                                                              c + e < a.Cout ? oq[q] + (unsigned)(c + e) * 4u : M3D_BUF_OOB, 0, 0);
                    }
                }
            }
        }
        TRACE();
        return;
    }
#pragma unroll
    for (int nt = 0; nt < NT; ++nt) {
        const int co = n0 + nt * 32 + l31;
        const bool cok = co < a.Cout;
        const float sc = (cok && a.scale) ? a.scale[co] : 1.f;
        const float sh = (cok && a.shift) ? a.shift[co] : 0.f;
        float rv[16];
        if (a.res) {
#pragma unroll
            for (int r = 0; r < 16; ++r) {
                const int m = mb + (r & 3) + 8 * (r >> 2);
                const unsigned ro = (cok && m < a.M) ? ((unsigned)m * (unsigned)a.res_cs + (unsigned)co) * 4u : M3D_BUF_OOB;
                rv[r] = __builtin_bit_cast(float, __builtin_amdgcn_raw_buffer_load_b32(rres, ro, 0, 0));
            }
        }
#pragma unroll
        for (int r = 0; r < 16; ++r) {
            const int m = mb + (r & 3) + 8 * (r >> 2);
            float v = conv_epi_affine(acc[nt][r], sc, sh, a.res ? rv[r] : 0.f, a.res != nullptr, a.res_mode);
            v = conv_epi_act(v, a.sigmoid_from >= 0 && co >= a.sigmoid_from, a.act == 1 ? M3D_LEAKY_SLOPE : 1.f);
            const unsigned oo = (cok && m < a.M) ? ((unsigned)m * (unsigned)a.out_cs + (unsigned)co) * 4u : M3D_BUF_OOB;
            __builtin_amdgcn_raw_buffer_store_b32(__builtin_bit_cast(unsigned, v), rout, oo, 0, 0);
        }
    }
    TRACE();
}

static int conv_wave_plan(const m3d_conv_desc *d, bool enforce_min, int *splits, int *ss_per, bool allow32 = false)
{
    *splits = 1;
    *ss_per = d->kh * d->kw * (d->Cin / 32);
    if (d->out_nchw) return 0;
    if (d->dcn_offmask && d->kh * d->kw > 9) return 0;
    if (d->Cin % 32 != 0 || d->Cout_pad % 32 != 0) return 0;
    if (d->Cout_pad % 64 != 0 && (!allow32 || d->dcn_offmask || d->wgt_img_stride)) return 0;
    const int cw = d->Cout_pad % 128 == 0 ? 128 : (d->Cout_pad % 64 == 0 ? 64 : 32);
    if (d->wgt_img_stride && (d->Ho * d->Wo) % 32 != 0) return 0;
    const long long M = (long long)d->N * d->Ho * d->Wo;
    const long long base = ((M + 31) / 32) * (d->Cout_pad / cw);
    if (base >= (1ll << 28)) return 0;
    static const int wave_min = m3d_env_int("M3D_CONV_WAVE_MIN", 900);
    static const int dcn_min = m3d_env_int("M3D_DCN_WAVE_MIN", 1500);
    static const int splitk = m3d_env_int("M3D_CONV_WAVE_SPLITK", 1);
    const long long need = d->dcn_offmask ? dcn_min : wave_min;
    const int nss = *ss_per;
    if (base < need && splitk && d->splitk_ws) {
        int s = (int)((1800 + base - 1) / base);
        if (s > nss / 4) s = nss / 4;
        if (s > 8) s = 8;
        if (s >= 2) {
            *ss_per = (nss + s - 1) / s;
            *splits = (nss + *ss_per - 1) / *ss_per;
        }
    }
    if (enforce_min && base * *splits < need) { *splits = 1; *ss_per = nss; return 0; }
    return (int)(base * *splits);
}

extern "C" int m3d_conv_wave_applicable(const m3d_conv_desc *d)
{
    int s, p;
    return d ? conv_wave_plan(d, true, &s, &p) : 0;
}

extern "C" int m3d_conv_wave_splitk_plan(const m3d_conv_desc *d, int *splits, long long *ws_bytes)
{
    M3D_REQUIRE(d && splits && ws_bytes, "conv_wave_splitk_plan: null pointer");
    m3d_conv_desc t = *d;
    static float dummy;
    t.splitk_ws = &dummy;
    int p;
    const int waves = conv_wave_plan(&t, true, splits, &p, true);
    if (waves == 0) *splits = 1;
    *ws_bytes = (*splits > 1 && d->Cout_pad % 64 == 0) ? (long long)*splits * d->N * d->Ho * d->Wo * d->Cout_pad * 4 : 0;
    return M3D_OK;
}

template <bool DEFORM, int NT>
static void launch_wgsplit(const ConvWaveArgs &a, int S, int wgs, hipStream_t stream)
{
    constexpr int WPE = DEFORM ? 2 : 3;
    switch (S) {
    case 2: hipLaunchKernelGGL((conv_wave_kernel<DEFORM, NT, 4, WPE, 2>), dim3(wgs), dim3(128), 0, stream, a); break;
    case 4: hipLaunchKernelGGL((conv_wave_kernel<DEFORM, NT, 4, WPE, 4>), dim3(wgs), dim3(256), 0, stream, a); break;
    default: hipLaunchKernelGGL((conv_wave_kernel<DEFORM, NT, 4, WPE, 8>), dim3(wgs), dim3(512), 0, stream, a); break;
    }
}

static int conv_wave_run(const m3d_conv_desc *d_, hipStream_t stream, bool wgsplit)
{
    M3D_REQUIRE(d_ && d_->in && d_->wgt && d_->out, "conv_wave: null pointer");
    m3d_conv_desc dd = *d_;
    static float dummy;
    if (wgsplit) { dd.splitk_ws = &dummy; dd.splitk_ws_bytes = 0; }
    const m3d_conv_desc *d = &dd;
    int splits = 1, ss_per = 0;
    const int waves = conv_wave_plan(d, false, &splits, &ss_per, wgsplit);
    M3D_REQUIRE(waves > 0, "conv_wave: needs Cin %% 32 == 0, Cout_pad %% 64 == 0 (%% 32: plain, shared weights, wgsplit entry), NHWC output, "
                           "Ho*Wo %% 32 == 0 with per-image weights");
    const int ho = (d->H + 2 * d->pad - (d->dil * (d->kh - 1) + 1)) / d->stride + 1;
    const int wo = (d->W + 2 * d->pad - (d->dil * (d->kw - 1) + 1)) / d->stride + 1;
    M3D_REQUIRE(ho == d->Ho && wo == d->Wo, "conv_wave: Ho/Wo mismatch");
    M3D_REQUIRE(d->in_cs % 32 == 0 && d->in_cs >= d->Cin && ((uintptr_t)d->in & 127) == 0 && ((uintptr_t)d->wgt & 15) == 0,
                "conv_wave: the input view must be 128-byte aligned with in_cs %% 32 == 0");
    const long long M = (long long)d->N * d->Ho * d->Wo;
    M3D_REQUIRE(!d->wgt_img_stride || (d->wgt_img_stride % 4 == 0 && d->stride == 1 && d->Ho == d->H && d->Wo == d->W),
                "conv_wave: per-image weights need an image-aligned 16-byte stride and a same-size output");
    M3D_REQUIRE((long long)d->N * d->H * d->W * d->in_cs * 4 < (1ll << 31) && M * d->out_cs * 4 < (1ll << 31) &&
                M * d->res_cs * 4 < (1ll << 31) && (long long)d->Cout_pad * d->kh * d->kw * d->Cin * 4 < (1ll << 31),
                "conv_wave: views must be < 2 GiB");
    ConvWaveArgs a;
    a.in = d->in; a.wfrag = d->wgt; a.scale = d->scale; a.shift = d->shift; a.res = d->res; a.om = d->dcn_offmask;
    a.out = d->out;
    a.in_cs = d->in_cs; a.out_cs = d->out_cs; a.res_cs = d->res_cs; a.om_cs = d->dcn_om_cs;
    a.H = d->H; a.W = d->W; a.Cin = d->Cin; a.Ho = d->Ho; a.Wo = d->Wo; a.HoWo = d->Ho * d->Wo; a.Cout = d->Cout;
    a.kh = d->kh; a.kw = d->kw; a.stride = d->stride; a.pad = d->pad; a.dil = d->dil;
    const int cw = d->Cout_pad % 128 == 0 ? 128 : (d->Cout_pad % 64 == 0 ? 64 : 32);
    a.M = (int)M; a.KG = d->kh * d->kw * d->Cin / 8; a.tiles_n = d->Cout_pad / cw;
    a.act = d->act; a.res_mode = d->res_mode; a.sigmoid_from = d->sigmoid_from; a.w_img_stride = d->wgt_img_stride;
    static const int vec_epi = m3d_env_int("M3D_WAVE_VEC_EPILOGUE", 1);
    a.vec_out = vec_epi && d->out_cs % 4 == 0 && ((uintptr_t)d->out & 15) == 0 &&
                (!d->res || (d->res_cs % 4 == 0 && ((uintptr_t)d->res & 15) == 0)) &&
                (!d->scale || ((uintptr_t)d->scale & 15) == 0) && (!d->shift || ((uintptr_t)d->shift & 15) == 0);
    a.in_bytes = (unsigned)((long long)d->N * d->H * d->W * d->in_cs * 4);
    a.out_bytes = (unsigned)(M * d->out_cs * 4);
    a.res_bytes = (unsigned)(M * d->res_cs * 4);
    a.w_bytes = (unsigned)((long long)cw * d->kh * d->kw * d->Cin * 4);
#ifdef CONV_TRACE
    a.trace = g_conv_trace;
#endif
    a.ws = nullptr; a.splits = 1; a.ss_per = ss_per; a.base_waves = waves; a.ws_bytes = 0;
    if (splits > 1 && wgsplit) {
        const int S = splits <= 2 ? 2 : (splits <= 4 ? 4 : 8);
        M3D_REQUIRE(splits <= 8, "conv_wave: %d K slices do not fit a workgroup", splits);
        a.splits = splits; a.base_waves = waves / splits;
        if (cw == 128) {
            if (d->dcn_offmask) launch_wgsplit<true, 4>(a, S, a.base_waves, stream);
            else launch_wgsplit<false, 4>(a, S, a.base_waves, stream);
        } else if (cw == 64) {
            if (d->dcn_offmask) launch_wgsplit<true, 2>(a, S, a.base_waves, stream);
            else launch_wgsplit<false, 2>(a, S, a.base_waves, stream);
        } else {
            launch_wgsplit<false, 1>(a, S, a.base_waves, stream);
        }
        M3D_LAUNCH_CHECK();
        return M3D_OK;
    }
    if (splits > 1) {
        const long long need = (long long)splits * M * d->Cout_pad * 4;
        M3D_REQUIRE(need <= d->splitk_ws_bytes && need < (1ll << 31) && ((uintptr_t)d->splitk_ws & 15) == 0,
                    "conv_wave: split-K workspace too small (%lld bytes, see m3d_conv_wave_splitk_plan), >= 2 GiB or misaligned",
                    d->splitk_ws_bytes);
        a.ws = d->splitk_ws; a.splits = splits; a.base_waves = waves / splits; a.ws_bytes = (unsigned)need;
    }
#ifdef CONV_TRACE
    if (g_conv_variant && d->dcn_offmask && cw == 128) {
        switch (g_conv_variant) {
        case 1: hipLaunchKernelGGL((conv_wave_kernel<true, 4, 1, 2>), dim3(waves), dim3(64), 0, stream, a); break;
        case 2: hipLaunchKernelGGL((conv_wave_kernel<true, 4, 1, 3>), dim3(waves), dim3(64), 0, stream, a); break;
        case 3: hipLaunchKernelGGL((conv_wave_kernel<true, 4, 2, 2>), dim3(waves), dim3(64), 0, stream, a); break;
        case 4: hipLaunchKernelGGL((conv_wave_kernel<true, 4, 2, 3>), dim3(waves), dim3(64), 0, stream, a); break;
        default: hipLaunchKernelGGL((conv_wave_kernel<true, 4, 4, 3>), dim3(waves), dim3(64), 0, stream, a); break;
        }
        M3D_LAUNCH_CHECK();
        return M3D_OK;
    }
#endif
    if (cw == 128) {
        if (d->dcn_offmask) hipLaunchKernelGGL((conv_wave_kernel<true, 4>), dim3(waves), dim3(64), 0, stream, a);
        else hipLaunchKernelGGL((conv_wave_kernel<false, 4>), dim3(waves), dim3(64), 0, stream, a);
    } else if (cw == 32) {
        hipLaunchKernelGGL((conv_wave_kernel<false, 1>), dim3(waves), dim3(64), 0, stream, a);
    } else {
        if (d->dcn_offmask) hipLaunchKernelGGL((conv_wave_kernel<true, 2>), dim3(waves), dim3(64), 0, stream, a);
        else hipLaunchKernelGGL((conv_wave_kernel<false, 2>), dim3(waves), dim3(64), 0, stream, a);
    }
    M3D_LAUNCH_CHECK();
    if (splits > 1) {
        SplitkReduceArgs r;
        r.ws = a.ws; r.scale = d->scale; r.shift = d->shift; r.res = d->res; r.out = d->out;
        r.M = (int)M; r.Cout = d->Cout; r.Cout_pad = d->Cout_pad; r.splits = splits; r.out_cs = d->out_cs; r.res_cs = d->res_cs;
        r.res_mode = d->res_mode; r.act = d->act; r.sigmoid_from = d->sigmoid_from;
        return m3d_launch_splitk_reduce(r, stream);
    }
    return M3D_OK;
}

extern "C" int m3d_conv_wave_forward(const m3d_conv_desc *d, m3d_stream_t stream)
{
    return conv_wave_run(d, (hipStream_t)stream, false);
}

extern "C" int m3d_conv_wave_wgsplit_width(const m3d_conv_desc *d, int *slices, int *width)
{
    M3D_REQUIRE(d && slices && width, "conv_wave_wgsplit_width: null pointer");
    m3d_conv_desc t = *d;
    static float dummy;
    t.splitk_ws = &dummy;
    int p;
    const int waves = conv_wave_plan(&t, false, slices, &p, true);
    M3D_REQUIRE(waves > 0 && *slices <= 8, "conv_wave_wgsplit_width: the wave kernel does not apply to this descriptor");
    *width = *slices <= 1 ? 1 : (*slices <= 2 ? 2 : (*slices <= 4 ? 4 : 8));
    return M3D_OK;
}

extern "C" int m3d_conv_wave_forward_wgsplit(const m3d_conv_desc *d, m3d_stream_t stream)
{
    return conv_wave_run(d, (hipStream_t)stream, true);
}
```

### m3dssd_amd/csrc/wino44_conv.hip

```cpp
#include <type_traits>

#include "common.h"

struct Wino44Args {
    const float *in;
    const float *U;
    float *out;
    const float *scale, *shift, *res;
    int in_cs, out_cs, res_cs;
    unsigned in_bytes, out_bytes, res_bytes;
    int N, H, W, Cin, Cout;
    int TH, TW, NT;
    int act, res_mode;
    int nsl;
    long long ws_slice;
    const char *touch;
    int touch_lines;
#ifdef WINO_TRACE
    long long *trace;
#endif
};

#define W44_LA 4

#ifdef WINO_TRACE
static long long *g_w44_trace = nullptr;
extern "C" void m3d_wino44_set_trace(void *p) { g_w44_trace = (long long *)p; }
#define W44_TRACE_INIT() long long *trp = (a.trace && (wave == 0 || wave == 3)) ? a.trace + ((size_t)(blockIdx.y * gridDim.x + blockIdx.x) * 2 + (wave ? 1 : 0)) * 64 : nullptr; int tri = 0
#define W44_TRACE() do { if (trp && lane == 0 && tri < 64) trp[tri++] = __builtin_readcyclecounter(); } while (0)
#else
#define W44_TRACE_INIT()
#define W44_TRACE()
#endif

__device__ __forceinline__ void w44_load_dword(float &dst, __amdgpu_buffer_rsrc_t r, unsigned voff, unsigned soff)
{
    asm volatile("buffer_load_dword %0, %1, %2, %3 offen" : "=v"(dst) : "v"(voff), "s"(r), "s"(soff) : "memory");
}
__device__ __forceinline__ void w44_load_x4(f32x4 &dst, __amdgpu_buffer_rsrc_t r, unsigned voff, unsigned soff)
{
    asm volatile("buffer_load_dwordx4 %0, %1, %2, %3 offen" : "=v"(dst) : "v"(voff), "s"(r), "s"(soff) : "memory");
}
template <int N, int NB>
__device__ __forceinline__ void w44_wait(f32x4 (&u)[2])
{
    if constexpr (NB == 2) asm volatile("s_waitcnt vmcnt(%2)" : "+v"(u[0]), "+v"(u[1]) : "n"(N));
    else asm volatile("s_waitcnt vmcnt(%1)" : "+v"(u[0]) : "n"(N));
}

template <int I, int N, typename F>
__device__ __forceinline__ void w44_static_for(F &&f)
{
    if constexpr (I < N) {
        f(std::integral_constant<int, I>{});
        w44_static_for<I + 1, N>(f);
    }
}

__device__ __forceinline__ int w44_vswz(int t, int c) { return c ^ ((t >> 3) << 3); }

__device__ __forceinline__ void w44_bt(const float x0, const float x1, const float x2, const float x3, const float x4, const float x5,
                                       float &y0, float &y1, float &y2, float &y3, float &y4, float &y5)
{
    y0 = fmaf(4.f, x0, fmaf(-5.f, x2, x4));
    const float a = fmaf(-4.f, x2, x4), b = fmaf(-4.f, x1, x3);
    y1 = a + b;
    y2 = a - b;
    const float c = x4 - x2, e = x3 - x1;
    y3 = fmaf(2.f, e, c);
    y4 = fmaf(-2.f, e, c);
    y5 = fmaf(4.f, x1, fmaf(-5.f, x3, x5));
}
template <typename VT>
__device__ __forceinline__ void w44_at(const VT m0, const VT m1, const VT m2, const VT m3, const VT m4, const VT m5,
                                       VT &y0, VT &y1, VT &y2, VT &y3)
{
    const VT s1 = m1 + m2, d1 = m1 - m2, s2 = m3 + m4, d2 = m3 - m4;
    y0 = m0 + s1 + s2;
    y1 = d2 * 2.f + d1;
    y2 = s2 * 4.f + s1;
    y3 = d2 * 8.f + d1 + m5;
}

template <int NB, int OCC, int KS = 1>
__global__ __launch_bounds__(256 * KS) __attribute__((amdgpu_waves_per_eu(OCC, OCC))) void wino44_kernel(const Wino44Args a)
{
    static_assert(KS == 1 || (KS == 2 && NB == 1 && OCC == 2), "K-pair form: 64-channel waves, two per SIMD");
    __shared__ __attribute__((aligned(16))) float Vs_all[KS * 2 * 36 * 256];
    __shared__ int pixb[16];
    const int tid8 = threadIdx.x, lane = tid8 & 63;
    const int kh = KS == 2 ? __builtin_amdgcn_readfirstlane(tid8 >> 8) : 0;
    const int tid = tid8 & 255;
    float *const Vs = Vs_all + kh * (2 * 36 * 256);
    const int wave = __builtin_amdgcn_readfirstlane(tid >> 6);
    const int NS = a.nsl;
    int bx = blockIdx.x, by = blockIdx.y, bz = blockIdx.z;
    {
        const int X = gridDim.x, C = gridDim.y * gridDim.z;
        if (gridDim.z > 1 && (C & 7) == 0) {
            const int lin = (blockIdx.z * gridDim.y + blockIdx.y) * X + blockIdx.x, xcd = lin & 7, idx = lin >> 3;
            const int combo = xcd * (C >> 3) + idx / X;
            bx = idx % X;
            by = combo % (int)gridDim.y;
            bz = combo / (int)gridDim.y;
        }
    }
    const int s0 = (bz * KS + kh) * a.nsl;
    W44_TRACE_INIT();
    W44_TRACE();

    const int ut = tid >> 4, uc = tid & 15;
    unsigned vM[6], v0[6], v5[6];
    {
        const int t = bx * 16 + ut;
        const bool tv = t < a.NT;
        const int tt = tv ? t : 0;
        const int n = tt / (a.TH * a.TW), rem = tt - n * a.TH * a.TW;
        const int ty = rem / a.TW, tx = rem - ty * a.TW;
        if (uc == 0 && kh == 0) pixb[ut] = tv ? (n * a.H + 4 * ty) * a.W + 4 * tx : -1;
        const bool c5ok = 4 * tx + 4 < a.W;
#pragma unroll
        for (int r = 0; r < 6; ++r) {
            const int hi = 4 * ty - 1 + r;
            const bool ok = tv && hi >= 0 && hi < a.H;
            const unsigned base = ((unsigned)((n * a.H + hi) * a.W + 4 * tx) * (unsigned)a.in_cs + (unsigned)uc) * 4u;
            vM[r] = ok ? base : M3D_BUF_OOB;
            v0[r] = (ok && tx > 0) ? base - (unsigned)a.in_cs * 4u : M3D_BUF_OOB;
            v5[r] = (ok && c5ok) ? base : M3D_BUF_OOB;
        }
    }
    const unsigned cs4 = (unsigned)a.in_cs * 4u;
    const __amdgpu_buffer_rsrc_t rin = make_rsrc(a.in + s0 * 16, a.in_bytes - (unsigned)s0 * 64u);
    const int cb16 = (by * 4 + wave) * NB;
    const int cb32 = cb16 >> 1, j0 = cb16 & 1;
    const __amdgpu_buffer_rsrc_t ru = make_rsrc(a.U + ((size_t)cb32 * (a.Cin >> 4) + s0) * (36 * 2 * 256), (unsigned)NS * (36u * 2u * 1024u));
    const unsigned ulane = (unsigned)lane * 16u + (unsigned)j0 * 1024u;

    float d[36];
    auto load_patch = [&](int s) __attribute__((always_inline)) {
        const unsigned so = (unsigned)s * 64u;
#pragma unroll
        for (int r = 0; r < 6; ++r) {
            w44_load_dword(d[r * 6 + 0], rin, v0[r], so);
#pragma unroll
            for (int c = 1; c < 5; ++c) w44_load_dword(d[r * 6 + c], rin, vM[r], so + (unsigned)(c - 1) * cs4);
            w44_load_dword(d[r * 6 + 5], rin, v5[r], so + 4u * cs4);
        }
    };
    auto load_patch_one = [&](int s, auto qtag) __attribute__((always_inline)) {
        constexpr int q = decltype(qtag)::value, r = q / 6, c = q % 6;
        const unsigned so = (unsigned)s * 64u;
        if constexpr (c == 0) w44_load_dword(d[q], rin, v0[r], so);
        else if constexpr (c == 5) w44_load_dword(d[q], rin, v5[r], so + 4u * cs4);
        else w44_load_dword(d[q], rin, vM[r], so + (unsigned)(c - 1) * cs4);
    };
    auto transform_col = [&](auto ctag) __attribute__((always_inline)) {
        constexpr int c = decltype(ctag)::value;
        float t0, t1, t2, t3, t4, t5;
        w44_bt(d[0 * 6 + c], d[1 * 6 + c], d[2 * 6 + c], d[3 * 6 + c], d[4 * 6 + c], d[5 * 6 + c], t0, t1, t2, t3, t4, t5);
        d[0 * 6 + c] = t0; d[1 * 6 + c] = t1; d[2 * 6 + c] = t2; d[3 * 6 + c] = t3; d[4 * 6 + c] = t4; d[5 * 6 + c] = t5;
    };
    auto transform_row = [&](int buf, auto rtag) __attribute__((always_inline)) {
        constexpr int r = decltype(rtag)::value;
        float *vb = Vs + buf * (36 * 256) + ut * 16 + w44_vswz(ut, uc);
        float v[6];
        w44_bt(d[r * 6 + 0], d[r * 6 + 1], d[r * 6 + 2], d[r * 6 + 3], d[r * 6 + 4], d[r * 6 + 5], v[0], v[1], v[2], v[3], v[4], v[5]);
#pragma unroll
        for (int c = 0; c < 6; ++c) vb[(r * 6 + c) * 256] = v[c];
    };
    auto transform_store = [&](int buf) __attribute__((always_inline)) {
        transform_col(std::integral_constant<int, 0>{}); transform_col(std::integral_constant<int, 1>{});
        transform_col(std::integral_constant<int, 2>{}); transform_col(std::integral_constant<int, 3>{});
        transform_col(std::integral_constant<int, 4>{}); transform_col(std::integral_constant<int, 5>{});
        transform_row(buf, std::integral_constant<int, 0>{}); transform_row(buf, std::integral_constant<int, 1>{});
        transform_row(buf, std::integral_constant<int, 2>{}); transform_row(buf, std::integral_constant<int, 3>{});
        transform_row(buf, std::integral_constant<int, 4>{}); transform_row(buf, std::integral_constant<int, 5>{});
    };
    auto tie_patch = [&]() __attribute__((always_inline)) {
        asm volatile("" : "+v"(d[0]), "+v"(d[1]), "+v"(d[2]), "+v"(d[3]), "+v"(d[4]), "+v"(d[5]), "+v"(d[6]), "+v"(d[7]), "+v"(d[8]),
                          "+v"(d[9]), "+v"(d[10]), "+v"(d[11]), "+v"(d[12]), "+v"(d[13]), "+v"(d[14]), "+v"(d[15]), "+v"(d[16]), "+v"(d[17]));
        asm volatile("" : "+v"(d[18]), "+v"(d[19]), "+v"(d[20]), "+v"(d[21]), "+v"(d[22]), "+v"(d[23]), "+v"(d[24]), "+v"(d[25]), "+v"(d[26]),
                          "+v"(d[27]), "+v"(d[28]), "+v"(d[29]), "+v"(d[30]), "+v"(d[31]), "+v"(d[32]), "+v"(d[33]), "+v"(d[34]), "+v"(d[35]));
    };

    f32x4 Uf[4][2];
    auto load_u = [&](int s, int xi, auto slot_tag) __attribute__((always_inline)) {
        constexpr int SL = decltype(slot_tag)::value;
        const unsigned so = (unsigned)__builtin_amdgcn_readfirstlane((s * 36 + xi) * 2) * 1024u;
        w44_load_x4(Uf[SL][0], ru, ulane, so);
        if constexpr (NB == 2) w44_load_x4(Uf[SL][1], ru, ulane, so + 1024u);
    };

    float touched = 0.f;
    if (a.touch) {
        const int nwg = gridDim.x * gridDim.y * gridDim.z;
        const int wg = (blockIdx.z * gridDim.y + blockIdx.y) * gridDim.x + blockIdx.x;
        for (int i = wg * (256 * KS) + tid8; i < a.touch_lines; i += nwg * (256 * KS))
            asm volatile("global_load_dword %0, %1, off" : "=v"(touched) : "v"(a.touch + (size_t)i * 128) : "memory");
    }
    load_patch(0);
    f32x4 acc[36][NB];
#pragma unroll
    for (int x = 0; x < 36; ++x)
#pragma unroll
        for (int j = 0; j < NB; ++j) acc[x][j] = f32x4{0.f, 0.f, 0.f, 0.f};
    asm volatile("s_waitcnt vmcnt(0)" : "+v"(touched) : : "memory");
    tie_patch();
    W44_TRACE();
    transform_store(0);
    W44_TRACE();
    constexpr bool INTERLEAVE = NB == 1;
    if (INTERLEAVE && NS > 1) load_patch(1);
    load_u(0, 0, std::integral_constant<int, 0>{});
    load_u(0, 1, std::integral_constant<int, 1>{});
    load_u(0, 2, std::integral_constant<int, 2>{});
    load_u(0, 3, std::integral_constant<int, 3>{});
    if (!INTERLEAVE && NS > 1) load_patch(1);
    __syncthreads();
    W44_TRACE();

    const int atile = lane & 15, aq = lane >> 4;
    auto stage = [&](int s, auto last_tag, auto issue_tag) __attribute__((always_inline)) {
        constexpr bool LAST = decltype(last_tag)::value, ISSUE = decltype(issue_tag)::value;
        const float *vbuf = Vs + (s & 1) * (36 * 256) + atile * 16 + w44_vswz(atile, aq * 4);
        f32x4 anext = *reinterpret_cast<const f32x4 *>(vbuf);
        w44_static_for<0, 36>([&](auto xtag) __attribute__((always_inline)) {
            constexpr int xi = decltype(xtag)::value;
            constexpr int nx = xi + W44_LA;
            constexpr int plo = xi - 4 > 17 ? xi - 4 : 17, phi = xi - 1 < 28 ? xi - 1 : 28;
            constexpr int pyoung = !INTERLEAVE ? (xi < W44_LA ? 36 : 0)
                                               : ((ISSUE && phi >= plo) ? 3 * (phi - plo + 1) : 0);
            if constexpr (!LAST) w44_wait<3 * NB + pyoung, NB>(Uf[xi % 4]);
            else if constexpr (xi <= 32) w44_wait<3 * NB, NB>(Uf[xi % 4]);
            else w44_wait<(35 - xi) * NB, NB>(Uf[xi % 4]);
            const f32x4 av = anext;
            if constexpr (xi + 1 < 36) anext = *reinterpret_cast<const f32x4 *>(vbuf + (xi + 1) * 256);
            __builtin_amdgcn_sched_barrier(0);
#pragma unroll
            for (int e = 0; e < 4; ++e)
#pragma unroll
                for (int j = 0; j < NB; ++j)
                    acc[xi][j] = __builtin_amdgcn_mfma_f32_16x16x4f32(av[e], Uf[xi % 4][j][e], acc[xi][j], 0, 0, 0);
            if constexpr (!LAST) {
                if constexpr (xi == 4) tie_patch();
                if constexpr (xi >= 5 && xi <= 10) transform_col(std::integral_constant<int, xi - 5>{});
                if constexpr (xi >= 11 && xi <= 16) transform_row((s + 1) & 1, std::integral_constant<int, xi - 11>{});
            }
            __builtin_amdgcn_sched_barrier(0);
            if constexpr (nx < 36) load_u(s, nx, std::integral_constant<int, nx % 4>{});
            else if constexpr (!LAST) load_u(s + 1, nx - 36, std::integral_constant<int, nx % 4>{});
            if constexpr (INTERLEAVE && ISSUE && xi >= 17 && xi <= 28) {
                load_patch_one(s + 2, std::integral_constant<int, 3 * (xi - 17)>{});
                load_patch_one(s + 2, std::integral_constant<int, 3 * (xi - 17) + 1>{});
                load_patch_one(s + 2, std::integral_constant<int, 3 * (xi - 17) + 2>{});
            }
            __builtin_amdgcn_sched_barrier(0);
        });
        W44_TRACE();
        if constexpr (!LAST) {
            if constexpr (!INTERLEAVE) { if (s + 2 < NS) load_patch(s + 2); }
            __builtin_amdgcn_sched_barrier(0);
            W44_TRACE();
            __syncthreads();
            W44_TRACE();
        }
    };
    if constexpr (INTERLEAVE) {
        for (int s = 0; s + 2 < NS; ++s) stage(s, std::false_type{}, std::true_type{});
        if (NS > 1) stage(NS - 2, std::false_type{}, std::false_type{});
    } else {
        for (int s = 0; s + 1 < NS; ++s) stage(s, std::false_type{}, std::false_type{});
    }
    stage(NS - 1, std::true_type{}, std::false_type{});

    __syncthreads();
    constexpr int NI = KS == 2 ? 2 : 4;
    constexpr int NTW = KS == 2 ? 8 : 16;
    using VT = std::conditional_t<KS == 2, f32x2, f32x4>;
    const int ioff = KS == 2 ? 2 * kh : 0;
    VT accv[36][NB];
    if constexpr (KS == 2) {
        f32x2 *xb = reinterpret_cast<f32x2 *>(Vs_all);
#pragma unroll
        for (int x = 0; x < 36; ++x) {
            const f32x4 v = acc[x][0];
            xb[(kh * 36 + x) * 256 + tid] = kh == 0 ? f32x2{v[2], v[3]} : f32x2{v[0], v[1]};
        }
        __syncthreads();
#pragma unroll
        for (int x = 0; x < 36; ++x) {
            const f32x4 v = acc[x][0];
            const f32x2 o = xb[((kh ^ 1) * 36 + x) * 256 + tid];
            accv[x][0] = (kh == 0 ? f32x2{v[0], v[1]} : f32x2{v[2], v[3]}) + o;
            if (x % 6 == 5) __builtin_amdgcn_sched_barrier(0);
        }
        __syncthreads();
    } else {
#pragma unroll
        for (int x = 0; x < 36; ++x)
#pragma unroll
            for (int j = 0; j < NB; ++j) accv[x][j] = __builtin_bit_cast(VT, acc[x][j]);
    }
    const __amdgpu_buffer_rsrc_t rout = make_rsrc(a.out + (size_t)bz * a.ws_slice, a.out_bytes);
    const __amdgpu_buffer_rsrc_t rres = make_rsrc(a.res ? a.res : a.out, a.res ? a.res_bytes : 0u);
    float *ot = Vs_all + (kh * 4 + wave) * (NTW * 272);
    const int opx = lane >> 2, ocq = lane & 3;
    const unsigned pixoff = (unsigned)((opx >> 2) * a.W + (opx & 3));
    auto tile_of = [&](int lt) __attribute__((always_inline)) { return KS == 2 ? 4 * (lt >> 1) + ioff + (lt & 1) : lt; };
#pragma unroll
    for (int j = 0; j < NB; ++j) {
        const int c0 = (cb16 + j) * 16 + ocq * 4;
        const bool blockfull = (cb16 + j) * 16 + 16 <= a.Cout;
        const unsigned ovoff = (pixoff * (unsigned)a.out_cs + (unsigned)c0) * 4u, rvoff = (pixoff * (unsigned)a.res_cs + (unsigned)c0) * 4u;
        f32x4 rvv[NTW];
        {
            VT z[4][6];
#pragma unroll
            for (int b = 0; b < 6; ++b)
                w44_at(accv[0 * 6 + b][j], accv[1 * 6 + b][j], accv[2 * 6 + b][j], accv[3 * 6 + b][j], accv[4 * 6 + b][j], accv[5 * 6 + b][j],
                       z[0][b], z[1][b], z[2][b], z[3][b]);
            if (a.res && blockfull) {
#pragma unroll
                for (int k = 0; k < NTW; ++k) {
                    const int pb = __builtin_amdgcn_readfirstlane(pixb[tile_of(k)]);
                    rvv[k] = buf_load_f32x4(rres, rvoff, pb >= 0 ? (unsigned)pb * (unsigned)a.res_cs * 4u : M3D_BUF_OOB);
                }
            }
            float *op = ot + (NI * aq) * 272 + atile;
#pragma unroll
            for (int yy = 0; yy < 4; ++yy) {
                VT y[4];
                w44_at(z[yy][0], z[yy][1], z[yy][2], z[yy][3], z[yy][4], z[yy][5], y[0], y[1], y[2], y[3]);
#pragma unroll
                for (int xx = 0; xx < 4; ++xx)
#pragma unroll
                    for (int i = 0; i < NI; ++i) op[i * 272 + (yy * 4 + xx) * 16] = y[xx][i];
            }
        }
        f32x4 sc = {1.f, 1.f, 1.f, 1.f}, sh = {0.f, 0.f, 0.f, 0.f};
#pragma unroll
        for (int e = 0; e < 4; ++e)
            if (c0 + e < a.Cout) {
                if (a.scale) sc[e] = a.scale[c0 + e];
                if (a.shift) sh[e] = a.shift[c0 + e];
            }
        if (blockfull) {
            const float slope = a.act == 1 ? M3D_LEAKY_SLOPE : 1.f;
            auto body = [&](auto mode_tag) __attribute__((always_inline)) {
                constexpr int MODE = decltype(mode_tag)::value;
#pragma unroll
                for (int k = 0; k < NTW; ++k) {
                    const int pb = __builtin_amdgcn_readfirstlane(pixb[tile_of(k)]);
                    const unsigned osoff = pb >= 0 ? (unsigned)pb * (unsigned)a.out_cs * 4u : M3D_BUF_OOB;
                    f32x4 v = *reinterpret_cast<const f32x4 *>(ot + k * 272 + lane * 4);
                    if constexpr (MODE == 2) v = (v + rvv[k]) * sc + sh;
                    else if constexpr (MODE == 1) v = v * sc + sh + rvv[k];
                    else v = v * sc + sh;
                    v = __builtin_elementwise_max(v, v * slope);
                    buf_store_f32x4_nop(v, rout, ovoff, osoff);
                }
            };
            if (!a.res) body(std::integral_constant<int, 0>{});
            else if (a.res_mode) body(std::integral_constant<int, 2>{});
            else body(std::integral_constant<int, 1>{});
        } else {
            for (int k = 0; k < NTW; ++k) {
                const int pb = __builtin_amdgcn_readfirstlane(pixb[tile_of(k)]);
                const unsigned osoff = pb >= 0 ? (unsigned)pb * (unsigned)a.out_cs * 4u : M3D_BUF_OOB;
                const unsigned rsoff = pb >= 0 ? (unsigned)pb * (unsigned)a.res_cs * 4u : M3D_BUF_OOB;
                const f32x4 v0 = *reinterpret_cast<const f32x4 *>(ot + k * 272 + lane * 4);
#pragma unroll
                for (int e = 0; e < 4; ++e) {
                    const unsigned em = c0 + e < a.Cout ? (unsigned)e * 4u : M3D_BUF_OOB;
                    float v = v0[e];
                    if (a.res) {
                        const float rv = __builtin_bit_cast(float, __builtin_amdgcn_raw_buffer_load_b32(rres, rvoff + em, rsoff, 0));
                        if (a.res_mode) v = fmaf(v + rv, sc[e], sh[e]);
                        else v = fmaf(v, sc[e], sh[e]) + rv;
                    } else {
                        v = fmaf(v, sc[e], sh[e]);
                    }
                    if (a.act == 1) v = fmaxf(v, v * M3D_LEAKY_SLOPE);
                    __builtin_amdgcn_raw_buffer_store_b32(__builtin_bit_cast(unsigned, v), rout, ovoff + em, osoff, 0);
                }
            }
        }
    }
    W44_TRACE();
}

__device__ __forceinline__ void w44_at1(const float m0, const float m1, const float m2, const float m3, const float m4, const float m5,
                                        float &y0, float &y1, float &y2, float &y3)
{
    const float s1 = m1 + m2, d1 = m1 - m2, s2 = m3 + m4, d2 = m3 - m4;
    y0 = m0 + s1 + s2;
    y1 = fmaf(2.f, d2, d1);
    y2 = fmaf(4.f, s2, s1);
    y3 = fmaf(8.f, d2, d1) + m5;
}

struct Wino44C16Args {
    const float *in, *U, *scale, *shift;
    float *out;
    int in_cs, out_cs;
    unsigned in_bytes, out_bytes;
    int H, W, TH, TW, NT;
};

__global__ __launch_bounds__(256) void wino44_c16_kernel(const Wino44C16Args a)
{
    __shared__ __attribute__((aligned(16))) float Vs[36 * 256];
    const int tid = threadIdx.x, lane = tid & 63;
    const int wave = __builtin_amdgcn_readfirstlane(tid >> 6);
    const int ut = tid >> 4, uc = tid & 15;
    f32x4 ub[9];
#pragma unroll
    for (int k = 0; k < 9; ++k) ub[k] = *reinterpret_cast<const f32x4 *>(a.U + ((wave * 9 + k) * 64 + lane) * 4);

    const int t = blockIdx.x * 16 + ut;
    const bool tv = t < a.NT;
    const int tt = tv ? t : 0;
    const int n = tt / (a.TH * a.TW), rem = tt - n * a.TH * a.TW;
    const int ty = rem / a.TW, tx = rem - ty * a.TW;
    const __amdgpu_buffer_rsrc_t rin = make_rsrc(a.in, a.in_bytes);
    const unsigned cs4 = (unsigned)a.in_cs * 4u;
    float d[36];
    {
        const unsigned org = tv ? ((unsigned)((n * a.H + 4 * ty) * a.W + 4 * tx) * (unsigned)a.in_cs + (unsigned)uc) * 4u : M3D_BUF_OOB;
        const bool r0ok = tv && ty > 0, r5ok = 4 * ty + 4 < a.H, c0ok = tv && tx > 0, c5ok = 4 * tx + 4 < a.W;
        const unsigned rowb = (unsigned)a.W * cs4;
        const unsigned orgR = r0ok ? org - rowb : M3D_BUF_OOB, orgC = c0ok ? org - cs4 : M3D_BUF_OOB;
        const unsigned orgRC = (r0ok && c0ok) ? org - rowb - cs4 : M3D_BUF_OOB;
#pragma unroll
        for (int r = 0; r < 6; ++r)
#pragma unroll
            for (int c = 0; c < 6; ++c) {
                unsigned vo = (r == 0 && c == 0) ? orgRC : (r == 0 ? orgR : (c == 0 ? orgC : org));
                if (r == 5) vo = r5ok ? vo : M3D_BUF_OOB;
                if (c == 5) vo = c5ok ? vo : M3D_BUF_OOB;
                const int rr = r == 0 ? 0 : r - 1, cc = c == 0 ? 0 : c - 1;
                const unsigned so = (unsigned)__builtin_amdgcn_readfirstlane(rr * a.W + cc) * cs4;
                d[r * 6 + c] = __builtin_bit_cast(float, __builtin_amdgcn_raw_buffer_load_b32(rin, vo, so, 0));
            }
    }
#pragma unroll
    for (int c = 0; c < 6; ++c) {
        float t0, t1, t2, t3, t4, t5;
        w44_bt(d[0 * 6 + c], d[1 * 6 + c], d[2 * 6 + c], d[3 * 6 + c], d[4 * 6 + c], d[5 * 6 + c], t0, t1, t2, t3, t4, t5);
        d[0 * 6 + c] = t0; d[1 * 6 + c] = t1; d[2 * 6 + c] = t2; d[3 * 6 + c] = t3; d[4 * 6 + c] = t4; d[5 * 6 + c] = t5;
    }
    float *vb = Vs + ut * 16 + w44_vswz(ut, uc);
#pragma unroll
    for (int r = 0; r < 6; ++r) {
        float v[6];
        w44_bt(d[r * 6 + 0], d[r * 6 + 1], d[r * 6 + 2], d[r * 6 + 3], d[r * 6 + 4], d[r * 6 + 5], v[0], v[1], v[2], v[3], v[4], v[5]);
#pragma unroll
        for (int c = 0; c < 6; ++c) vb[(r * 6 + c) * 256] = v[c];
    }
    __syncthreads();

    {
        const int atile = lane & 15, aq = lane >> 4;
        float *slot = Vs + wave * 9 * 256;
        f32x4 av[9];
#pragma unroll
        for (int k = 0; k < 9; ++k) av[k] = *reinterpret_cast<const f32x4 *>(slot + k * 256 + atile * 16 + w44_vswz(atile, aq * 4));
#pragma unroll
        for (int k = 0; k < 9; ++k) {
            f32x4 acc = {0.f, 0.f, 0.f, 0.f};
#pragma unroll
            for (int e = 0; e < 4; ++e) acc = __builtin_amdgcn_mfma_f32_16x16x4f32(av[k][e], ub[k][e], acc, 0, 0, 0);
#pragma unroll
            for (int i = 0; i < 4; ++i) slot[k * 256 + (4 * aq + i) * 16 + atile] = acc[i];
        }
    }
    __syncthreads();

    {
        float m[36];
#pragma unroll
        for (int x = 0; x < 36; ++x) m[x] = Vs[x * 256 + ut * 16 + uc];
        float z[4][6];
#pragma unroll
        for (int b = 0; b < 6; ++b)
            w44_at1(m[0 * 6 + b], m[1 * 6 + b], m[2 * 6 + b], m[3 * 6 + b], m[4 * 6 + b], m[5 * 6 + b], z[0][b], z[1][b], z[2][b], z[3][b]);
        const float sc = a.scale[uc], sh = a.shift[uc];
        const __amdgpu_buffer_rsrc_t rout = make_rsrc(a.out, a.out_bytes);
        const unsigned obase = tv ? ((unsigned)((n * a.H + 4 * ty) * a.W + 4 * tx) * (unsigned)a.out_cs + (unsigned)uc) * 4u : M3D_BUF_OOB;
        const unsigned ocs4 = (unsigned)a.out_cs * 4u;
#pragma unroll
        for (int yy = 0; yy < 4; ++yy) {
            float y[4];
            w44_at1(z[yy][0], z[yy][1], z[yy][2], z[yy][3], z[yy][4], z[yy][5], y[0], y[1], y[2], y[3]);
#pragma unroll
            for (int xx = 0; xx < 4; ++xx) {
                float v = fmaf(y[xx], sc, sh);
                v = fmaxf(v, v * M3D_LEAKY_SLOPE);
                __builtin_amdgcn_raw_buffer_store_b32(__builtin_bit_cast(unsigned, v), rout, obase,
                                                      (unsigned)__builtin_amdgcn_readfirstlane(yy * a.W + xx) * ocs4, 0);
            }
        }
    }
}

extern "C" int m3d_conv3x3_c16_wino(const float *in, int in_cs, const float *U, const float *scale, const float *shift, float *out,
                                    int out_cs, int N, int H, int W, m3d_stream_t stream)
{
    M3D_REQUIRE(in && U && scale && shift && out && in_cs >= 16 && out_cs >= 16 && N >= 1, "conv3x3_c16_wino: bad arguments");
    M3D_REQUIRE(H % 4 == 0 && W % 4 == 0 && H >= 4 && W >= 4, "conv3x3_c16_wino: H and W must be multiples of 4");
    M3D_REQUIRE(((uintptr_t)U & 15) == 0, "conv3x3_c16_wino: U must be 16-byte aligned");
    const long long ib = (long long)N * H * W * in_cs * 4, ob = (long long)N * H * W * out_cs * 4;
    M3D_REQUIRE(ib < (1ll << 31) && ob < (1ll << 31), "conv3x3_c16_wino: views must be < 2 GiB");
    Wino44C16Args a;
    a.in = in; a.U = U; a.scale = scale; a.shift = shift; a.out = out; a.in_cs = in_cs; a.out_cs = out_cs;
    a.in_bytes = (unsigned)ib; a.out_bytes = (unsigned)ob;
    a.H = H; a.W = W; a.TH = H / 4; a.TW = W / 4; a.NT = N * a.TH * a.TW;
    hipLaunchKernelGGL(wino44_c16_kernel, dim3(cdiv(a.NT, 16)), dim3(256), 0, (hipStream_t)stream, a);
    M3D_LAUNCH_CHECK();
    return M3D_OK;
}

static int w44_scratch_bytes()
{
#ifndef WINO_TRACE
    static const int v = m3d_scratch_bytes(&wino44_kernel<1, 1>, &wino44_kernel<2, 1>, &wino44_kernel<1, 2>, &wino44_kernel<1, 2, 2>);
    return v < 0 ? 0 : v;
#else
    return 0;
#endif
}
static int w44_build_ok() { return w44_scratch_bytes() == 0 ? 1 : 0; }

extern "C" int m3d_wino44_applicable(const m3d_conv_desc *d)
{
    if (!d || d->kh != 3 || d->kw != 3 || d->stride != 1 || d->pad != 1 || d->dil > 1) return 0;
    if (d->dcn_offmask || d->out_nchw || d->wgt_img_stride || d->sigmoid_from >= 0) return 0;
    if (d->H % 4 || d->W % 4 || d->Cin % 16 || d->Cout_pad % 64 || d->in_cs % 4) return 0;
    return w44_build_ok();
}

static int w44_split_nb() { static const int v = m3d_env_int("M3D_W44_SPLIT_NB", 1); return (v == 2 || v == 3) ? v : 1; }
static int w44_occ2() { static const int v = m3d_env_int("M3D_W44_OCC2", 1); return v; }
static int w44_split_fill()
{
    static const int v = m3d_env_int("M3D_W44_SPLIT_FILL", 0);
    return v > 0 ? v : (w44_split_nb() == 1 ? 400 : 200);
}

extern "C" int m3d_wino44_splitk_plan(const m3d_conv_desc *d, int *splits, long long *ws_bytes)
{
    M3D_REQUIRE(d && splits && ws_bytes, "wino44_splitk_plan: null pointer");
    *splits = 1; *ws_bytes = 0;
    const int cw = w44_split_nb() == 2 ? 128 : 64;
    if (!m3d_wino44_applicable(d) || d->Cout_pad % cw) return M3D_OK;
    const long long wgs = (long long)cdiv(d->N * (d->H / 4) * (d->W / 4), 16) * (d->Cout_pad / cw);
    const int kp = w44_split_nb() == 3 ? 2 : 1;
    const int ns = d->Cin / 16 / kp, fill = w44_split_fill();
    if (wgs >= fill || (d->Cin / 16) % kp) return M3D_OK;
    for (int sp = 2; sp <= 8; sp *= 2) {
        if (ns % sp || ns / sp < 4) break;
        if (wgs * sp >= fill) {
            const long long need = (long long)sp * d->N * d->H * d->W * d->Cout_pad * 4;
            if (need / sp < (1ll << 31)) { *splits = sp; *ws_bytes = need; }
            break;
        }
    }
    return M3D_OK;
}

extern "C" int m3d_wino44_kpair(const m3d_conv_desc *d)
{
    if (!d || !m3d_wino44_applicable(d)) return 0;
    static const int kpair_max = m3d_env_int("M3D_W44_KPAIR_MAX", 300);
    const int ns = d->Cin / 16;
    const long long wgs = (long long)cdiv(d->N * (d->H / 4) * (d->W / 4), 16) * (d->Cout_pad / 64);
    return (w44_occ2() && wgs <= kpair_max && ns % 2 == 0 && ns / 2 >= 4) ? 1 : 0;
}

extern "C" int m3d_wino44_conv3x3_forward_touch(const m3d_conv_desc *d, int nb, const void *touch, long long touch_bytes,
                                                m3d_stream_t stream)
{
    M3D_REQUIRE(d && d->in && d->wgt && d->out, "wino44: null pointer");
    M3D_REQUIRE(m3d_wino44_applicable(d), "wino44: 3x3 / stride 1 / pad 1, H %% 4 == W %% 4 == 0, Cin %% 16 == 0, Cout_pad %% 64 == 0 only");
    M3D_REQUIRE(d->Ho == d->H && d->Wo == d->W, "wino44: Ho/Wo mismatch");
    Wino44Args a;
    a.in = d->in; a.U = d->wgt; a.out = d->out; a.scale = d->scale; a.shift = d->shift; a.res = d->res;
    a.in_cs = d->in_cs; a.out_cs = d->out_cs; a.res_cs = d->res_cs;
    const long long pix = (long long)d->N * d->H * d->W;
    M3D_REQUIRE(pix * d->in_cs * 4 < (1ll << 31) && pix * d->out_cs * 4 < (1ll << 31), "wino44: views must be < 2 GiB");
    a.in_bytes = (unsigned)(pix * d->in_cs * 4);
    a.out_bytes = (unsigned)(pix * d->out_cs * 4);
    a.res_bytes = d->res ? (unsigned)(pix * d->res_cs * 4) : 0u;
    a.N = d->N; a.H = d->H; a.W = d->W; a.Cin = d->Cin; a.Cout = d->Cout;
    a.TH = d->H / 4; a.TW = d->W / 4; a.NT = d->N * a.TH * a.TW;
    a.act = d->act; a.res_mode = d->res_mode;
    a.nsl = d->Cin / 16; a.ws_slice = 0;
    M3D_REQUIRE(touch_bytes >= 0 && touch_bytes / 128 < (1ll << 31), "wino44: touch range");
    a.touch = touch_bytes >= 128 ? (const char *)touch : nullptr; a.touch_lines = touch ? (int)(touch_bytes / 128) : 0;
#ifdef WINO_TRACE
    a.trace = g_w44_trace;
#endif
    M3D_REQUIRE(w44_scratch_bytes() == 0, "wino44: this build of the kernel uses %d bytes of scratch memory per lane (register spills)",
                w44_scratch_bytes());
    const int strips = cdiv(a.NT, 16);
    M3D_REQUIRE(nb >= 0 && nb <= 2 && !(nb == 2 && d->Cout_pad % 128), "wino44: nb = 0 (automatic), 1 or 2 (needs Cout_pad %% 128 == 0)");
    if (d->splitk_ws && (nb == 0 || nb == (w44_split_nb() == 2 ? 2 : 1))) {
        int splits = 1;
        long long need = 0;
        if (const int rc = m3d_wino44_splitk_plan(d, &splits, &need)) return rc;
        if (splits > 1) {
            M3D_REQUIRE(need <= d->splitk_ws_bytes && ((uintptr_t)d->splitk_ws & 15) == 0,
                        "wino44: split-K workspace too small (%lld bytes, see m3d_wino44_splitk_plan) or misaligned", d->splitk_ws_bytes);
            a.out = d->splitk_ws; a.out_cs = d->Cout_pad; a.out_bytes = (unsigned)(pix * d->Cout_pad * 4);
            a.ws_slice = pix * d->Cout_pad; a.nsl = d->Cin / 16 / splits;
            a.scale = a.shift = a.res = nullptr; a.res_bytes = 0; a.act = 0; a.res_mode = 0; a.Cout = d->Cout_pad;
            if (w44_split_nb() == 1)
                hipLaunchKernelGGL((wino44_kernel<1, 2>), dim3(strips, d->Cout_pad / 64, splits), dim3(256), 0, (hipStream_t)stream, a);
            else if (w44_split_nb() == 3) {
                a.nsl = d->Cin / 16 / (splits * 2);
                hipLaunchKernelGGL((wino44_kernel<1, 2, 2>), dim3(strips, d->Cout_pad / 64, splits), dim3(512), 0, (hipStream_t)stream, a);
            } else
                hipLaunchKernelGGL((wino44_kernel<2, 1>), dim3(strips, d->Cout_pad / 128, splits), dim3(256), 0, (hipStream_t)stream, a);
            M3D_LAUNCH_CHECK();
            SplitkReduceArgs r;
            r.ws = d->splitk_ws; r.scale = d->scale; r.shift = d->shift; r.res = d->res; r.out = d->out;
            r.M = (int)pix; r.Cout = d->Cout; r.Cout_pad = d->Cout_pad; r.splits = splits; r.out_cs = d->out_cs;
            r.res_cs = d->res_cs; r.res_mode = d->res_mode; r.act = d->act; r.sigmoid_from = d->sigmoid_from;
            return m3d_launch_splitk_reduce(r, (hipStream_t)stream);
        }
    }
    const bool nb2 = d->Cout_pad % 128 == 0 && nb == 2;
    if (!nb2 && m3d_wino44_kpair(d)) {
        a.nsl = d->Cin / 16 / 2;
        hipLaunchKernelGGL((wino44_kernel<1, 2, 2>), dim3(strips, d->Cout_pad / 64), dim3(512), 0, (hipStream_t)stream, a);
        M3D_LAUNCH_CHECK();
        return M3D_OK;
    }
    if (nb2) hipLaunchKernelGGL((wino44_kernel<2, 1>), dim3(strips, d->Cout_pad / 128), dim3(256), 0, (hipStream_t)stream, a);
    else if (w44_occ2()) hipLaunchKernelGGL((wino44_kernel<1, 2>), dim3(strips, d->Cout_pad / 64), dim3(256), 0, (hipStream_t)stream, a);
    else hipLaunchKernelGGL((wino44_kernel<1, 1>), dim3(strips, d->Cout_pad / 64), dim3(256), 0, (hipStream_t)stream, a);
    M3D_LAUNCH_CHECK();
    return M3D_OK;
}

extern "C" int m3d_wino44_conv3x3_forward_ex(const m3d_conv_desc *d, int nb, m3d_stream_t stream)
{
    return m3d_wino44_conv3x3_forward_touch(d, nb, nullptr, 0, stream);
}

extern "C" int m3d_wino44_conv3x3_forward(const m3d_conv_desc *d, m3d_stream_t stream)
{
    return m3d_wino44_conv3x3_forward_touch(d, 0, nullptr, 0, stream);
}
```

### m3dssd_amd/engine.py

```python
import ctypes
import math
import os

import numpy as np
import torch

from . import _hip
from ._hip import ConvDesc, MlpDesc
from .config import model_flags

BN_EPS = 1e-5
SELECT_KEYS = os.environ.get("M3D_SELECT_KEYS", "1") != "0"
SPARSE_HEADS_MAX_FRACTION = 0.5
PSP_SIZES = (1, 4, 8, 16)
BACKBONE_CHANNELS = {"dla34": (16, 32, 64, 128, 256, 512), "dla102": (16, 32, 128, 256, 512, 1024)}
DLA102_LEVELS = (1, 1, 1, 3, 4, 1)


def _rup(a, b):
    return (a + b - 1) // b * b


class View:
    __slots__ = ("t", "ptr", "n", "h", "w", "c", "cs", "keep")

    def __init__(self, t, n, h, w, c, cs=None, ptr=None):
        self.t, self.n, self.h, self.w, self.c = t, n, h, w, c
        self.cs = c if cs is None else cs
        self.ptr = t.data_ptr() if ptr is None else ptr

    def slice(self, c0, c):
        assert c0 % 4 == 0 and c0 + c <= self.cs
        return View(self.t, self.n, self.h, self.w, c, self.cs, self.ptr + 4 * c0)

    def torch_nchw(self):
        full = self.t.view(self.n, self.h, self.w, self.cs)
        off = (self.ptr - self.t.data_ptr()) // 4
        return full[..., off:off + self.c].permute(0, 3, 1, 2).contiguous()


class _Stream:
    @staticmethod
    def current(device=None):
        return ctypes.c_void_p(torch.cuda.current_stream(device).cuda_stream)


class PackedConv:

    def __init__(self, eng, weight, bias=None, bn=None, cout_pad_to=32, cin_pad=None):
        w = weight.detach().to(eng.device, torch.float32).contiguous()
        self.cout, self.cin, self.kh, self.kw = w.shape
        self.cin_pad = self.cin if cin_pad is None else cin_pad
        self.cout_pad = _rup(self.cout, cout_pad_to)
        self.wp = torch.empty(self.cout_pad * self.kh * self.kw * self.cin_pad, device=eng.device, dtype=torch.float32)
        _hip.check(eng.L.m3d_pack_conv_weight(w.data_ptr(), self.wp.data_ptr(), self.cout, self.cout_pad, self.cin,
                                              self.cin_pad, self.kh, self.kw, _Stream.current()))
        scale = torch.ones(self.cout, device=eng.device, dtype=torch.float32)
        shift = torch.zeros(self.cout, device=eng.device, dtype=torch.float32)
        if bias is not None:
            shift = bias.detach().to(eng.device, torch.float32).clone()
        if bn is not None:
            g, b, m, v = (t.detach().to(eng.device, torch.float32) for t in bn)
            s = g / torch.sqrt(v + BN_EPS)
            shift = (shift - m) * s + b
            scale = s
        self.scale, self.shift = scale.contiguous(), shift.contiguous()
        self.has_affine = (bias is not None) or (bn is not None)
        self._eng_device = eng.device
        self._frag = None
        self.wino = None
        self._w_cpu = None
        if USE_WINO and self.kh == 3 and self.kw == 3 and self.cin_pad == self.cin and self.cin % 16 == 0 and self.cin >= 32:
            self.wino = pack_wino(w, self.cout_pad, eng.device)
            if USE_WINO44 and self.cout_pad % 64 == 0:
                self._w_cpu = w.detach().cpu()
        self._wino44 = None

    def wino44(self):
        if self._wino44 is None and self._w_cpu is not None:
            self._wino44 = pack_wino44(self._w_cpu, self.cout_pad, self._eng_device)
        return self._wino44


    def frag(self):
        if self._frag is None:
            k = self.kh * self.kw * self.cin_pad
            self._frag = pack_frag(self.wp.view(self.cout_pad, k), self.cout_pad, self._eng_device)
        return self._frag


def pack_frag(weight2d, rows_pad, device):
    w = weight2d.detach().to(device, torch.float32)
    r, k = w.shape
    assert k % 8 == 0 and rows_pad % 32 == 0 and rows_pad >= r
    if rows_pad != r:
        w = torch.cat([w, w.new_zeros(rows_pad - r, k)], 0)
    return w.view(rows_pad // 32, 32, k // 8, 2, 4).permute(0, 2, 3, 1, 4).contiguous().view(-1)


_WINO_G = torch.tensor([[1.0, 0.0, 0.0], [0.5, 0.5, 0.5], [0.5, -0.5, 0.5], [0.0, 0.0, 1.0]], dtype=torch.float64)


def pack_wino(weight, cout_pad, device):
    g = weight.detach().to("cpu", torch.float64)
    co, ci = g.shape[0], g.shape[1]
    assert g.shape[2:] == (3, 3) and ci % 8 == 0 and cout_pad % 32 == 0 and cout_pad >= co
    u = torch.einsum("ai,ocij,bj->aboc", _WINO_G, g, _WINO_G).reshape(16, co, ci)
    if cout_pad != co:
        u = torch.cat([u, u.new_zeros(16, cout_pad - co, ci)], 1)
    u = u.view(16, cout_pad // 32, 32, ci // 8, 2, 4).permute(0, 1, 3, 4, 2, 5).contiguous()
    return u.to(torch.float32).reshape(-1).to(device)


_WINO44_G = torch.tensor([[1 / 4, 0, 0], [-1 / 6, -1 / 6, -1 / 6], [-1 / 6, 1 / 6, -1 / 6], [1 / 24, 1 / 12, 1 / 6], [1 / 24, -1 / 12, 1 / 6],
                          [0, 0, 1]], dtype=torch.float64)


def pack_wino44(weight, cout_pad, device):
    g = weight.detach().to("cpu", torch.float64)
    co, ci = g.shape[0], g.shape[1]
    assert g.shape[2:] == (3, 3) and ci % 16 == 0 and cout_pad % 32 == 0 and cout_pad >= co
    u = torch.einsum("ai,ocij,bj->aboc", _WINO44_G, g, _WINO44_G).reshape(36, co, ci)
    if cout_pad != co:
        u = torch.cat([u, u.new_zeros(36, cout_pad - co, ci)], 1)
    u = u.view(36, cout_pad // 32, 2, 16, ci // 16, 4, 4).permute(1, 4, 0, 2, 5, 3, 6).contiguous()
    return u.to(torch.float32).reshape(-1).to(device)


def pack_wino44_c16(weight, device):
    g = weight.detach().to("cpu", torch.float64)
    assert tuple(g.shape) == (16, 16, 3, 3)
    u = torch.einsum("ai,ocij,bj->abco", _WINO44_G, g, _WINO44_G).reshape(36, 4, 4, 16)
    return u.permute(0, 1, 3, 2).contiguous().to(torch.float32).reshape(-1).to(device)


WINO_MIN_BLOCKS = int(os.environ.get("M3D_WINO_MIN_BLOCKS", "128"))
FUSED_ANAB = os.environ.get("M3D_FUSED_ANAB", "1") != "0"
ANAB_ROWS = os.environ.get("M3D_ANAB_ROWS", "1") != "0"
USE_ANAB_WAVE = os.environ.get("M3D_ANAB_WAVE", "1") != "0"
USE_ANAB_NESTED = os.environ.get("M3D_ANAB_NESTED", "1") != "0"
USE_DCN_WAVE = os.environ.get("M3D_DCN_WAVE", "1") != "0"
USE_CONV_WAVE = os.environ.get("M3D_CONV_WAVE", "1") != "0"
USE_CONV_WAVE_WGSPLIT = os.environ.get("M3D_CONV_WAVE_WGSPLIT", "1") != "0"
USE_OFFMASK_WAVE = os.environ.get("M3D_OFFMASK_WAVE", "1") != "0"
USE_WINO = os.environ.get("M3D_WINO", "1") != "0"
USE_WINO44 = os.environ.get("M3D_WINO44", "1") != "0"
WINO44_TOUCH = os.environ.get("M3D_WINO44_TOUCH", "1") != "0"
WINO44_TOUCH_SPAN = int(os.environ.get("M3D_WINO44_TOUCH_SPAN", "2"))
USE_WINO44_SPLITK = os.environ.get("M3D_WINO44_SPLITK", "1") != "0"
W44_SPLIT_NB = 2 if os.environ.get("M3D_W44_SPLIT_NB", "1") == "2" else 1
W44_SPLIT_KPAIR = os.environ.get("M3D_W44_SPLIT_NB", "1") == "3"
WINO44_MIN_WGS = int(os.environ.get("M3D_WINO44_MIN_WGS", "1000000"))
WINO44_MIN_WGS_NB1 = int(os.environ.get("M3D_WINO44_MIN_WGS_NB1", "200"))


class OpCost:

    def __init__(self, hbm_bytes):
        self.hbm_bytes = int(hbm_bytes)


def lo_hi_contains(start, end, n, br):
    lo, hi = start, (n if end is None else end)
    return lo <= br[0] and br[2] <= hi


class _Plan:

    def __init__(self):
        self.ops = []
        self.keep = []
        self.named = {}
        self.w44_prev = None
        self.branches = []
        self.tail = None
        self.tail_start = None


class Engine:
    def __init__(self, state_dict, conf, device=None, backbone_only=False):
        self.L = _hip.lib()
        self.backbone_only = backbone_only
        self.device = torch.device(device if device is not None else conf.device)
        if self.device.type != "cuda":
            raise NotImplementedError("the M3DSSD HIP engine runs on a ROCm device only (got %s)" % self.device)
        if self.device.index is None:
            self.device = torch.device("cuda", torch.cuda.current_device())
        self.conf = conf
        self.back_bone = str(conf.back_bone) if "back_bone" in conf else "dla34"
        if self.back_bone not in BACKBONE_CHANNELS:
            raise NotImplementedError("back_bone %r: the engine runs %s" % (self.back_bone, " / ".join(BACKBONE_CHANNELS)))
        if getattr(self, "compute_dtype", "f32") == "bf16" and self.back_bone != "dla34":
            raise NotImplementedError("the bf16 engine runs the dla34 backbone only; run back_bone %r in fp32" % self.back_bone)
        sd = {k[7:] if k.startswith("module.") else k: v for k, v in state_dict.items()}
        self.sd = sd
        self.A = int(np.asarray(conf.anchors).shape[0]) if not backbone_only else 0
        self.NC = len(conf.lbls) + 1 if not backbone_only else 0
        self.stride = int(conf.feat_stride)
        self.flags = model_flags(conf) if not backbone_only else (False, False, False)
        with torch.cuda.device(self.device):
            self._pack(sd)
        self.plans = {}
        self.profile = None
        self.profile_kinds = None
        self._pending = []

    def _bn(self, p):
        sd = self.sd
        return (sd[p + ".weight"], sd[p + ".bias"], sd[p + ".running_mean"], sd[p + ".running_var"])

    def _pc(self, conv, bn=None, **kw):
        sd = self.sd
        return PackedConv(self, sd[conv + ".weight"], sd.get(conv + ".bias"), self._bn(bn) if bn else None, **kw)

    def _pack(self, sd):
        dev = self.device
        P = {}
        b = "base.base"
        w = sd[b + ".base_layer.0.weight"].detach().to(dev, torch.float32)
        P["stem.w"] = w.permute(2, 3, 1, 0).contiguous()
        g, be, m, v = (t.detach().to(dev, torch.float32) for t in self._bn(b + ".base_layer.1"))
        s = g / torch.sqrt(v + BN_EPS)
        P["stem.scale"], P["stem.shift"] = s.contiguous(), (be - m * s).contiguous()
        P["level0"] = self._pc(b + ".level0.0", b + ".level0.1")
        w0 = sd[b + ".level0.0.weight"].detach().to(dev, torch.float32)
        P["level0.direct"] = w0.permute(2, 3, 1, 0).contiguous() if tuple(w0.shape) == (16, 16, 3, 3) else None
        P["level0.wino44"] = pack_wino44_c16(w0, self.device) if (USE_WINO44 and tuple(w0.shape) == (16, 16, 3, 3)) else None
        P["level1"] = self._pc(b + ".level1.0", b + ".level1.1")

        def block(p):
            P[p + ".conv1"] = self._pc(p + ".conv1", p + ".bn1")
            P[p + ".conv2"] = self._pc(p + ".conv2", p + ".bn2")

        def tree1(p):
            block(p + ".tree1")
            block(p + ".tree2")
            P[p + ".root"] = self._pc(p + ".root.conv", p + ".root.bn")
            if (p + ".project.0.weight") in sd:
                P[p + ".project"] = self._pc(p + ".project.0", p + ".project.1")

        def bottleneck(p):
            for i in (1, 2, 3):
                P["%s.conv%d" % (p, i)] = self._pc("%s.conv%d" % (p, i), "%s.bn%d" % (p, i))

        def tree(p, levels):
            if levels == 1:
                bottleneck(p + ".tree1")
                bottleneck(p + ".tree2")
                P[p + ".root"] = self._pc(p + ".root.conv", p + ".root.bn")
                if (p + ".project.0.weight") in sd:
                    P[p + ".project"] = self._pc(p + ".project.0", p + ".project.1")
            else:
                tree(p + ".tree1", levels - 1)
                tree(p + ".tree2", levels - 1)

        if self.back_bone == "dla102":
            for lv in (2, 3, 4, 5):
                tree("%s.level%d" % (b, lv), DLA102_LEVELS[lv])
        else:
            tree1(b + ".level2")
            for lv in (3, 4):
                tree1("%s.level%d.tree1" % (b, lv))
                tree1("%s.level%d.tree2" % (b, lv))
            tree1(b + ".level5")

        def deform(p):
            P[p + ".om"] = self._pc(p + ".conv.conv_offset_mask")
            P[p + ".dcn"] = PackedConv(self, sd[p + ".conv.weight"], sd[p + ".conv.bias"], self._bn(p + ".actf.0"),
                                       cout_pad_to=64)

        def ida(p, n):
            for i in range(1, n):
                deform("%s.proj_%d" % (p, i))
                deform("%s.node_%d" % (p, i))
                up = sd["%s.up_%d.weight" % (p, i)].detach().to(dev, torch.float32)
                P["%s.up_%d" % (p, i)] = up[:, 0].permute(1, 2, 0).contiguous()

        ida("base.dla_up.ida_0", 2)
        ida("base.dla_up.ida_1", 3)
        ida("base.ida_up", 2)

        self.P = P
        if not self.backbone_only:
            self._pack_heads(sd, P)
        torch.cuda.synchronize(self.device)

    def _pack_anab(self, P, wq, wk, wv, ws):
        self.ck, self.cv, self.ns = wq.shape[0], wv.shape[0], ws.shape[0]
        self.ck_pad = _rup(self.ck, 32)
        cin = wq.shape[1]
        zpad = torch.zeros(self.ck_pad - self.ck, cin, 1, 1)
        wall = torch.cat([wq.detach().cpu().float(), zpad, wk.detach().cpu().float(), wv.detach().cpu().float(),
                          ws.detach().cpu().float()], 0)
        P["anab.qkvs"] = PackedConv(self, wall, None, None)
        self.anab_off = dict(q=0, k=self.ck_pad, v=self.ck_pad + self.ck, s=self.ck_pad + self.ck + self.cv)
        self.anab_ctot = wall.shape[0]

    def _pack_heads(self, sd, P):
        dev = self.device

        def head(p):
            P[p + ".0"] = self._pc(p + ".0", p + ".1")
            P[p + ".3"] = self._pc(p + ".3", p + ".4")
            P[p + ".6"] = self._pc(p + ".6", cout_pad_to=256 if p == "cls" else 64)
            for li, rows in ((".0", 256), (".3", 256), (".6", P[p + ".6"].cout_pad)):
                wt = sd[p + li + ".weight"]
                if wt.shape[2] == 1:
                    P[p + li + ".frag"] = pack_frag(wt.reshape(wt.shape[0], wt.shape[1]), rows, dev)

        self.box_heads = ["bbox_x", "bbox_y", "bbox_w", "bbox_h", "bbox_x3d", "bbox_y3d", "bbox_z3d", "bbox_w3d",
                          "bbox_h3d", "bbox_l3d", "bbox_rY3d"]
        for h in ["cls"] + self.box_heads:
            head(h)
        with_shape, with_center, with_anab = self.flags
        for p in ("shape_align",) * with_shape + ("center_align2d", "center_align3d") * with_center:
            P[p] = PackedConv(self, sd[p + ".align.weight"], sd[p + ".align.bias"], None, cout_pad_to=64)

        if with_anab:
            a = "bbox_z3d_gl.0"
            self._pack_anab(P, sd[a + ".query_conv.weight"], sd[a + ".key_conv.weight"], sd[a + ".value_conv.weight"],
                            sd[a + ".spatial_conv.weight"])
            g, be, m, v = (t.detach().to(dev, torch.float32) for t in self._bn("bbox_z3d_gl.1"))
            s = g / torch.sqrt(v + BN_EPS)
            P["anab.bn.scale"], P["anab.bn.shift"] = s.contiguous(), (be - m * s).contiguous()

        anchors = torch.as_tensor(np.asarray(self.conf.anchors), dtype=torch.float32)
        aw = (anchors[:, 2] - anchors[:, 0])
        ah = (anchors[:, 3] - anchors[:, 1])
        tab = torch.zeros(self.A, 18, dtype=torch.float32)
        h_step, w_step = ah / self.stride / 3, aw / self.stride / 3
        for i in range(3):
            for j in range(3):
                k = i * 3 + j
                tab[:, 2 * k] = (h_step - 1) * (i - 3 / 2 + 0.5)
                tab[:, 2 * k + 1] = (w_step - 1) * (j - 3 / 2 + 0.5)
        P["shape.table"] = tab.to(dev).contiguous()
        P["anchor_wh"] = torch.stack([aw / self.stride, ah / self.stride], 1).to(dev).contiguous()
        P["anchors"] = anchors.to(dev).contiguous()
        P["means"] = torch.as_tensor(np.asarray(self.conf.bbox_means), dtype=torch.float32).reshape(-1).to(dev)
        P["stds"] = torch.as_tensor(np.asarray(self.conf.bbox_stds), dtype=torch.float32).reshape(-1).to(dev)

    def _buf(self, plan, n, h, w, c, cs=None, name=None, zero=False):
        cs = c if cs is None else cs
        t = (torch.zeros if zero else torch.empty)(n * h * w * cs, device=self.device, dtype=torch.float32)
        plan.keep.append(t)
        v = View(t, n, h, w, c, cs)
        if name:
            plan.named[name] = v
        return v

    def _conv(self, plan, name, pc, x, out, stride=1, pad=0, act=0, res=None, res_mode=0, sigmoid_from=-1, om=None,
              planar=None, affine=True, wgt_ptr=None, wgt_img_stride=0, cout=None, cout_pad=None, scale=None, shift=None,
              kh=None, kw=None, cin_true=None, wgt_frag=False):
        d = ConvDesc()
        d.inp, d.in_cs, d.N, d.H, d.W, d.Cin = x.ptr, x.cs, x.n, x.h, x.w, x.c
        kh = pc.kh if kh is None else kh
        kw = pc.kw if kw is None else kw
        d.wgt = pc.wp.data_ptr() if wgt_ptr is None else wgt_ptr
        d.wgt_img_stride = wgt_img_stride
        d.Cout = pc.cout if cout is None else cout
        d.Cout_pad = pc.cout_pad if cout_pad is None else cout_pad
        d.kh, d.kw, d.stride, d.pad, d.dil = kh, kw, stride, pad, 1
        d.Ho = (x.h + 2 * pad - kh) // stride + 1
        d.Wo = (x.w + 2 * pad - kw) // stride + 1
        if planar is not None:
            t, img_stride, ch_off = planar
            d.out, d.out_nchw, d.out_img_stride = t.data_ptr() + 4 * ch_off * d.Ho * d.Wo, 1, img_stride
        else:
            assert out.h == d.Ho and out.w == d.Wo and out.c >= d.Cout, (name, out.h, out.w, d.Ho, d.Wo)
            d.out, d.out_cs = out.ptr, out.cs
        if scale is not None:
            d.scale, d.shift = scale.data_ptr(), shift.data_ptr()
            plan.keep += [scale, shift]
        elif affine and pc is not None and pc.has_affine:
            d.scale, d.shift = pc.scale.data_ptr(), pc.shift.data_ptr()
        if res is not None:
            d.res, d.res_cs, d.res_mode = res.ptr, res.cs, res_mode
        d.act, d.sigmoid_from = act, sigmoid_from
        if om is not None:
            d.dcn_offmask, d.dcn_om_cs = om.ptr, om.cs
        L = self.L
        ref = ctypes.byref(d)
        wino_blocks = -(-(x.n * x.h * x.w) // 256) * (d.Cout_pad // 32)
        strips = -(-(x.n * x.h * x.w) // 256)
        nb = 2 if (d.Cout_pad % 128 == 0 and strips * (d.Cout_pad // 128) >= WINO44_MIN_WGS) else \
            (1 if strips * (d.Cout_pad // 64) >= WINO44_MIN_WGS_NB1 else 0)
        w44ok = (pc is not None and wgt_ptr is None and getattr(pc, "_w_cpu", None) is not None and om is None and planar is None
                 and sigmoid_from < 0 and L.m3d_wino44_applicable(ref) == 1)
        ks44 = 1
        if w44ok and not nb and USE_WINO44_SPLITK:
            ssplits, sbytes = ctypes.c_int(), ctypes.c_longlong()
            _hip.check(L.m3d_wino44_splitk_plan(ref, ctypes.byref(ssplits), ctypes.byref(sbytes)))
            if ssplits.value > 1:
                ws = torch.empty(sbytes.value // 4, device=self.device, dtype=torch.float32)
                plan.keep.append(ws)
                d.splitk_ws, d.splitk_ws_bytes = ws.data_ptr(), sbytes.value
                nb, ks44 = W44_SPLIT_NB, ssplits.value
        if w44ok and nb:
            u44 = pc.wino44()
            plan.keep.append(u44)
            d.wgt = u44.data_ptr()
            flops = 2.0 * x.n * d.Ho * d.Wo * d.Cout * 9 * pc.cin
            nxt = {"ptr": None, "bytes": 0}
            if WINO44_TOUCH:
                nbytes = u44.numel() * 4
                if plan.w44_prev is not None and len(plan.ops) - plan.w44_prev[0] <= WINO44_TOUCH_SPAN:
                    plan.w44_prev[1]["ptr"], plan.w44_prev[1]["bytes"] = u44.data_ptr(), nbytes
                else:
                    plan.ops.append((name + ".touch", "touch", 0.0,
                                     lambda st: _hip.check(L.m3d_cache_touch(u44.data_ptr(), nbytes, st)), OpCost(nbytes)))
            plan.w44_prev = (len(plan.ops), nxt)
            kp = ",kpair" if (nb == 1 and ((ks44 == 1 and L.m3d_wino44_kpair(ref) == 1) or (ks44 > 1 and W44_SPLIT_KPAIR))) else ""
            plan.ops.append((name, "wino44<16,%d%s%s>" % (16 * nb, ",splitk%d" % ks44 if ks44 > 1 else "", kp), flops,
                             lambda st: _hip.check(L.m3d_wino44_conv3x3_forward_touch(ref, nb, nxt["ptr"], nxt["bytes"], st)), d))
            return
        if (pc is not None and wgt_ptr is None and getattr(pc, "wino", None) is not None and kh == 3 and kw == 3
                and stride == 1 and pad == 1 and om is None and planar is None and x.h % 2 == 0 and x.w % 2 == 0
                and wino_blocks >= WINO_MIN_BLOCKS):
            d.wgt = pc.wino.data_ptr()
            flops = 2.0 * x.n * d.Ho * d.Wo * d.Cout * 9 * pc.cin
            ssplits, sbytes = ctypes.c_int(), ctypes.c_longlong()
            _hip.check(L.m3d_wino_conv3x3_splitk_plan(ref, ctypes.byref(ssplits), ctypes.byref(sbytes)))
            if ssplits.value > 1:
                ws = torch.empty(sbytes.value // 4, device=self.device, dtype=torch.float32)
                plan.keep.append(ws)
                d.splitk_ws, d.splitk_ws_bytes = ws.data_ptr(), sbytes.value
            if L.m3d_wino_conv3x3_variant(ref) == 1:
                kind = "wino_wave<32,32%s>" % (",splitk%d" % ssplits.value if ssplits.value > 1 else "")
            else:
                kind = "wino_lds<64,32,16>"
            plan.ops.append((name, kind, flops, lambda st: _hip.check(L.m3d_wino_conv3x3_forward(ref, st)), d))
            return
        flops_true = 2.0 * x.n * d.Ho * d.Wo * d.Cout * kh * kw * (
            cin_true if cin_true is not None else (pc.cin if (pc is not None and wgt_ptr is None) else x.c))
        if wgt_frag:
            assert wgt_ptr is not None and planar is None and x.cs % 32 == 0 and x.ptr % 128 == 0, name
            if L.m3d_conv_wave_applicable(ref) <= 0:
                raise RuntimeError("%s: fragment-ordered weights but the wave kernel does not apply" % name)
            plan.ops.append((name, "conv_wave", flops_true, lambda st: _hip.check(L.m3d_conv_wave_forward(ref, st)), d))
            return
        if (pc is not None and wgt_ptr is None and planar is None and (USE_DCN_WAVE if om is not None else USE_CONV_WAVE)
                and x.cs % 32 == 0 and x.ptr % 128 == 0 and pc.cin_pad == x.c):
            wsplits, wbytes = ctypes.c_int(), ctypes.c_longlong()
            _hip.check(L.m3d_conv_wave_splitk_plan(ref, ctypes.byref(wsplits), ctypes.byref(wbytes)))
            if wsplits.value > 1 and USE_CONV_WAVE_WGSPLIT and (d.Cout_pad % 64 == 0 or (USE_OFFMASK_WAVE and wsplits.value <= 4)):
                frag = pc.frag()
                d.wgt = frag.data_ptr()
                kind = "conv_wave<%s>" % ",".join((["deform"] if om is not None else []) + ["wgsplit%d" % wsplits.value])
                plan.ops.append((name, kind, flops_true, lambda st: _hip.check(L.m3d_conv_wave_forward_wgsplit(ref, st)), d))
                return
            ws = None
            if wsplits.value > 1 and wbytes.value > 0:
                ws = torch.empty(wbytes.value // 4, device=self.device, dtype=torch.float32)
                d.splitk_ws, d.splitk_ws_bytes = ws.data_ptr(), wbytes.value
            if L.m3d_conv_wave_applicable(ref) > 0:
                frag = pc.frag()
                d.wgt = frag.data_ptr()
                if ws is not None:
                    plan.keep.append(ws)
                kind = "conv_wave%s" % ("<%s>" % ",".join(
                    (["deform"] if om is not None else []) + (["splitk%d" % wsplits.value] if wsplits.value > 1 else []))
                    if (om is not None or wsplits.value > 1) else "")
                plan.ops.append((name, kind, flops_true, lambda st: _hip.check(L.m3d_conv_wave_forward(ref, st)), d))
                return
            d.splitk_ws, d.splitk_ws_bytes = None, 0
        bm, bn, bk, grid = ctypes.c_int(), ctypes.c_int(), ctypes.c_int(), ctypes.c_int()
        _hip.check(L.m3d_conv2d_tile(ref, ctypes.byref(bm), ctypes.byref(bn), ctypes.byref(bk), ctypes.byref(grid)))
        splits, ws_bytes = ctypes.c_int(), ctypes.c_longlong()
        _hip.check(L.m3d_conv2d_splitk_plan(ref, ctypes.byref(splits), ctypes.byref(ws_bytes)))
        if splits.value > 1:
            ws = torch.empty(ws_bytes.value // 4, device=self.device, dtype=torch.float32)
            plan.keep.append(ws)
            d.splitk_ws, d.splitk_ws_bytes = ws.data_ptr(), ws_bytes.value
        kind = "igemm<%d,%d,%d%s%s%s>" % (bm.value, bn.value, bk.value, ",deform" if om is not None else "",
                                          ",planar" if planar is not None else "",
                                          ",splitk%d" % splits.value if splits.value > 1 else "")
        if cin_true is None:
            cin_true = pc.cin if (pc is not None and wgt_ptr is None) else x.c
        flops = 2.0 * x.n * d.Ho * d.Wo * d.Cout * kh * kw * cin_true
        plan.ops.append((name, kind, flops, lambda st: _hip.check(L.m3d_conv2d_forward(ref, st)), d))

    def _op(self, plan, name, kind, fn, flops=0.0, nbytes=None):
        plan.ops.append((name, kind, float(flops), fn, OpCost(nbytes) if nbytes is not None else None))

    def _build_plan(self, B, H, W):
        L, P = self.L, self.P
        plan = _Plan()
        chs = BACKBONE_CHANNELS[self.back_bone]
        b = "base.base"
        in_ptr = [0]
        plan.named["input_ptr"] = in_ptr
        s0 = self._buf(plan, B, H, W, 16)
        in_u8 = [0, 0, 0]
        plan.named["input_u8"] = in_u8
        mean3 = (ctypes.c_float * 3)(*[float(v) for v in self.conf.image_means])
        stds3 = (ctypes.c_float * 3)(*[float(v) for v in self.conf.image_stds])

        def stem(st):
            if in_u8[0]:
                _hip.check(L.m3d_stem_conv7x7_u8(in_u8[0], in_u8[1], in_u8[2], mean3, stds3, P["stem.w"].data_ptr(),
                                                 P["stem.scale"].data_ptr(), P["stem.shift"].data_ptr(), s0.ptr, s0.cs, B, H,
                                                 W, st))
            else:
                _hip.check(L.m3d_stem_conv7x7(in_ptr[0], P["stem.w"].data_ptr(), P["stem.scale"].data_ptr(),
                                              P["stem.shift"].data_ptr(), s0.ptr, s0.cs, B, H, W, st))
        self._op(plan, "stem", "stem", stem, flops=2.0 * B * H * W * 16 * 147, nbytes=B * H * W * (3 + 16) * 4)
        l0 = self._buf(plan, B, H, W, 16, name="level0")
        if P.get("level0.wino44") is not None and H % 4 == 0 and W % 4 == 0 and os.environ.get("M3D_LEVEL0_WINO44", "1") != "0":
            pc0 = P["level0"]
            self._op(plan, "level0", "wino44_c16", lambda st: _hip.check(L.m3d_conv3x3_c16_wino(
                s0.ptr, s0.cs, P["level0.wino44"].data_ptr(), pc0.scale.data_ptr(), pc0.shift.data_ptr(), l0.ptr, l0.cs,
                B, H, W, st)), flops=2.0 * B * H * W * 16 * 144, nbytes=B * H * W * 32 * 4)
        elif P["level0.direct"] is not None and os.environ.get("M3D_LEVEL0_IGEMM", "0") != "1":
            pc0 = P["level0"]
            self._op(plan, "level0", "conv3x3_c16", lambda st: _hip.check(L.m3d_conv3x3_c16(
                s0.ptr, s0.cs, P["level0.direct"].data_ptr(), pc0.scale.data_ptr(), pc0.shift.data_ptr(), l0.ptr, l0.cs,
                B, H, W, st)), flops=2.0 * B * H * W * 16 * 144, nbytes=B * H * W * 32 * 4)
        else:
            self._conv(plan, "level0", P["level0"], s0, l0, 1, 1, act=1)
        l1 = self._buf(plan, B, H // 2, W // 2, 32, name="level1")
        self._conv(plan, "level1", P["level1"], l0, l1, 2, 1, act=1)

        def maxpool(name, x, out):
            self._op(plan, name, "maxpool", lambda st: _hip.check(L.m3d_maxpool2x2(
                x.ptr, x.cs, out.ptr, out.cs, x.n, x.h, x.w, x.c, st)), nbytes=x.n * x.h * x.w * x.c * 5)

        if self.back_bone == "dla102":
            l3, l4, l5 = self._dla102_levels(plan, l1, maxpool)
        else:
            def block(p, x, res, out, stride):
                co = P[p + ".conv1"].cout
                t = self._buf(plan, B, out.h, out.w, co)
                self._conv(plan, p + ".conv1", P[p + ".conv1"], x, t, stride, 1, act=1)
                self._conv(plan, p + ".conv2", P[p + ".conv2"], t, out, 1, 1, act=1, res=res)

            def tree1(p, x, co, stride, out, bottom=None):
                h, w = x.h // stride, x.w // stride
                cat = self._buf(plan, B, h, w, 2 * co)
                x2v, x1v = cat.slice(0, co), cat.slice(co, co)
                if stride == 1:
                    bottom = x
                elif bottom is None:
                    bottom = self._buf(plan, B, h, w, x.c)
                    maxpool(p + ".downsample", x, bottom)
                if (p + ".project") in P:
                    res = self._buf(plan, B, h, w, co)
                    self._conv(plan, p + ".project", P[p + ".project"], bottom, res, 1, 0, act=0)
                else:
                    res = bottom
                block(p + ".tree1", x, res, x1v, stride)
                block(p + ".tree2", x1v, x1v, x2v, 1)
                self._conv(plan, p + ".root", P[p + ".root"], cat, out, 1, 0, act=1)

            l2 = self._buf(plan, B, H // 4, W // 4, 64, name="level2")
            tree1(b + ".level2", l1, 64, 2, l2)

            def tree2(p, x, co, out):
                ci = x.c
                h, w = x.h // 2, x.w // 2
                catb = self._buf(plan, B, h, w, 2 * co + ci + co)
                bottom = catb.slice(2 * co, ci)
                X1 = catb.slice(2 * co + ci, co)
                maxpool(p + ".downsample", x, bottom)
                tree1(p + ".tree1", x, co, 2, X1, bottom=bottom)
                x2v, x1v = catb.slice(0, co), catb.slice(co, co)
                block(p + ".tree2.tree1", X1, X1, x1v, 1)
                block(p + ".tree2.tree2", x1v, x1v, x2v, 1)
                self._conv(plan, p + ".tree2.root", P[p + ".tree2.root"], catb, out, 1, 0, act=1)

            l3 = self._buf(plan, B, H // 8, W // 8, 128, name="level3")
            tree2(b + ".level3", l2, 128, l3)
            l4 = self._buf(plan, B, H // 16, W // 16, 256, name="level4")
            tree2(b + ".level4", l3, 256, l4)
            l5 = self._buf(plan, B, H // 32, W // 32, 512, name="level5")
            h5, w5 = H // 32, W // 32
            cat5 = self._buf(plan, B, h5, w5, 1024 + 256)
            bottom5 = cat5.slice(1024, 256)
            maxpool(b + ".level5.downsample", l4, bottom5)
            res5 = self._buf(plan, B, h5, w5, 512)
            self._conv(plan, b + ".level5.project", P[b + ".level5.project"], bottom5, res5, 1, 0, act=0)
            block(b + ".level5.tree1", l4, res5, cat5.slice(512, 512), 2)
            block(b + ".level5.tree2", cat5.slice(512, 512), cat5.slice(512, 512), cat5.slice(0, 512), 1)
            self._conv(plan, b + ".level5.root", P[b + ".level5.root"], cat5, l5, 1, 0, act=1)

        def deform(p, x, out):
            om = self._buf(plan, B, x.h, x.w, 27, 28)
            self._conv(plan, p + ".offset_mask", P[p + ".om"], x, om, 1, 1, act=0, sigmoid_from=18)
            self._conv(plan, p + ".dcn", P[p + ".dcn"], x, out, 1, 1, act=1, om=om)
            plan.named[p + ".out"] = out

        def ida_step(p, i, x, skip, co):
            proj = self._buf(plan, B, x.h, x.w, co)
            deform("%s.proj_%d" % (p, i), x, proj)
            summed = self._buf(plan, B, 2 * x.h, 2 * x.w, co)
            upw = P["%s.up_%d" % (p, i)]
            self._op(plan, "%s.up_%d" % (p, i), "upsample", lambda st: _hip.check(L.m3d_upsample2x_add(
                proj.ptr, proj.cs, upw.data_ptr(), skip.ptr, skip.cs, summed.ptr, summed.cs, B, proj.h, proj.w, co, st)),
                flops=2.0 * B * 4 * proj.h * proj.w * co * 4, nbytes=B * proj.h * proj.w * co * 4 * (1 + 4 + 4))
            node = self._buf(plan, B, 2 * x.h, 2 * x.w, co)
            deform("%s.node_%d" % (p, i), summed, node)
            return node

        c3, c4 = chs[3], chs[4]
        L5a = ida_step("base.dla_up.ida_0", 1, l5, l4, c4)
        L4b = ida_step("base.dla_up.ida_1", 1, l4, l3, c3)
        L5b = ida_step("base.dla_up.ida_1", 2, L5a, L4b, c3)
        feats0 = ida_step("base.ida_up", 1, L5a, L5b, c3)
        plan.named["feats0"] = feats0

        plan.feat = (feats0.h, feats0.w)
        if self.backbone_only:
            return plan

        fh, fw = feats0.h, feats0.w
        HW = fh * fw
        A, NC = self.A, self.NC
        R = A * HW
        cls_pl = torch.empty(B * NC * A * HW, device=self.device, dtype=torch.float32)
        box_pl = torch.empty(B * 11 * A * HW, device=self.device, dtype=torch.float32)
        plan.keep += [cls_pl, box_pl]
        plan.named["cls_planar"], plan.named["box_planar"] = cls_pl, box_pl
        plan.named["planar_first_op"] = len(plan.ops)

        def head_desc(p, x, planar, first):
            t, img_stride, ch_off = planar
            d = MlpDesc()
            d.inp, d.in_cs, d.M, d.Cin = x.ptr, x.cs, B * HW, x.c
            if first is not None:
                d.w1, d.s1, d.t1 = P[p + ".0.frag"].data_ptr(), first.scale.data_ptr(), first.shift.data_ptr()
            mid, last = P[p + ".3"], P[p + ".6"]
            d.w2, d.s2, d.t2 = P[p + ".3.frag"].data_ptr(), mid.scale.data_ptr(), mid.shift.data_ptr()
            d.w3, d.s3, d.t3 = P[p + ".6.frag"].data_ptr(), last.scale.data_ptr(), last.shift.data_ptr()
            d.Cout, d.Cout_pad = last.cout, last.cout_pad
            d.out, d.out_img_stride, d.HW = t.data_ptr() + 4 * ch_off * HW, img_stride, HW
            flops = 2.0 * B * HW * ((x.c * 256 if first is not None else 0) + 256 * 256 + 256 * last.cout)
            return d, flops

        def heads(items):
            arr = (MlpDesc * len(items))()
            flops = 0.0
            for i, (p, x, planar) in enumerate(items):
                arr[i], f = head_desc(p, x, planar, P[p + ".0"])
                flops += f
            n = len(items)
            name = "+".join(p for p, _, _ in items) + ".mlp"
            plan.ops.append((name, "head_mlp<3,%d>" % arr[0].Cout_pad, flops,
                             lambda st: _hip.check(L.m3d_head_mlp_forward_batched(arr, n, st)), arr))

        def head(p, x, planar, k0=1):
            if k0 == 1:
                return heads([(p, x, planar)])
            h1 = self._buf(plan, B, fh, fw, 256)
            self._conv(plan, p + ".0", P[p + ".0"], x, h1, 1, k0 // 2, act=1)
            d, flops = head_desc(p, h1, planar, None)
            ref = ctypes.byref(d)
            plan.ops.append((p + ".mlp", "head_mlp<2,%d>" % d.Cout_pad, flops,
                             lambda st: _hip.check(L.m3d_head_mlp_forward(ref, st)), d))

        head("cls", feats0, (cls_pl, NC * A * HW, 0), 3)
        sel_idx = torch.empty(B * HW, device=self.device, dtype=torch.int32)
        sel_prob = torch.empty(B * HW, device=self.device, dtype=torch.float32)
        plan.keep += [sel_idx, sel_prob]
        plan.named["sel_idx"], plan.named["sel_prob"] = sel_idx, sel_prob
        if NC == 4 and A >= 4 and SELECT_KEYS:
            plan.named["keys_by_select"] = True
            plan.named["score_bits_first_write_op"] = len(plan.ops)
            self._op(plan, "anchor_select", "select", lambda st: _hip.check(L.m3d_anchor_select_keys(
                cls_pl.data_ptr(), B, A, HW, sel_idx.data_ptr(), sel_prob.data_ptr(), plan.named["score_bits"].data_ptr(), st)),
                nbytes=B * HW * (A * NC + 2 + A) * 4)
        else:
            self._op(plan, "anchor_select", "select", lambda st: _hip.check(L.m3d_anchor_select(
                cls_pl.data_ptr(), B, A, NC, HW, sel_idx.data_ptr(), sel_prob.data_ptr(), None, st)),
                nbytes=B * HW * (A * NC + 2) * 4)

        means = np.asarray(self.conf.bbox_means, dtype=np.float32).reshape(-1)
        stds = np.asarray(self.conf.bbox_stds, dtype=np.float32).reshape(-1)

        def box_planar(k):
            return (box_pl, 11 * A * HW, k * A)

        def box_ptr(k):
            return box_pl.data_ptr() + 4 * k * A * HW

        with_shape, with_center, with_anab = self.flags
        if with_shape:
            om_sa = self._buf(plan, B, fh, fw, 27, 28)
            self._op(plan, "shape_align.offsets", "align", lambda st: _hip.check(L.m3d_align_offsets(
                0, sel_idx.data_ptr(), sel_prob.data_ptr(), 0.5, P["shape.table"].data_ptr(), None, None, None, 0.0, 1.0, 0.0,
                1.0, om_sa.ptr, om_sa.cs, B, A, HW, 9, 0, st)), nbytes=B * HW * (2 + 28) * 4)
            feats = self._buf(plan, B, fh, fw, c3, name="feats")
            self._conv(plan, "shape_align.dcn", P["shape_align"], feats0, feats, 1, 1, act=0, res=feats0, om=om_sa)
        else:
            feats = plan.named["feats"] = feats0

        align_args = {}

        def center_align(p, x, kx, ky, mi, out):
            om = self._buf(plan, B, fh, fw, 3, 4)
            align_args[p] = (om, kx, ky, mi)
            self._op(plan, p + ".offsets", "align", lambda st: _hip.check(L.m3d_align_offsets(
                1, sel_idx.data_ptr(), sel_prob.data_ptr(), 0.5, None, box_ptr(kx), box_ptr(ky),
                P["anchor_wh"].data_ptr(), float(means[mi]), float(stds[mi]), float(means[mi + 1]),
                float(stds[mi + 1]), om.ptr, om.cs, B, A, HW, 1, 11 * A * HW, st)), nbytes=B * HW * (2 + 2 + 4) * 4)
            self._conv(plan, p + ".dcn", P[p], x, out, 1, 0, act=0, res=x, om=om)

        z3d_now = [] if with_anab else ["bbox_z3d"]
        if with_center:
            heads([("bbox_x", feats, box_planar(0)), ("bbox_y", feats, box_planar(1)),
                   ("bbox_x3d", feats, box_planar(4)), ("bbox_y3d", feats, box_planar(5))])
            f2d = self._buf(plan, B, fh, fw, c3, name="feats_align2d")
            center_align("center_align2d", feats, 0, 1, 0, f2d)
            f3d = self._buf(plan, B, fh, fw, c3, name="feats_align3d")
            center_align("center_align3d", feats, 4, 5, 4, f3d)
            heads([("bbox_w", f2d, box_planar(2)), ("bbox_h", f2d, box_planar(3))] +
                  [(h, f3d, box_planar(self.box_heads.index(h))) for h in z3d_now + ["bbox_w3d", "bbox_h3d", "bbox_l3d", "bbox_rY3d"]])
        else:
            f2d = f3d = plan.named["feats_align2d"] = plan.named["feats_align3d"] = feats
            heads([(h, feats, box_planar(k)) for k, h in enumerate(self.box_heads) if h != "bbox_z3d" or not with_anab])

        if with_anab:
            gl = self._buf(plan, B, fh, fw, c3, name="feats_gl", zero=True)
            self._anab_ops(plan, f3d, gl, P["anab.bn.scale"], P["anab.bn.shift"], act=1, res_mode=1)
            head("bbox_z3d", gl, box_planar(6))
        else:
            plan.named["feats_gl"] = f3d

        cls = torch.empty(B, R, NC, device=self.device, dtype=torch.float32)
        prob = torch.empty(B, R, NC, device=self.device, dtype=torch.float32)
        b2 = torch.empty(B, R, 4, device=self.device, dtype=torch.float32)
        b3 = torch.empty(B, R, 7, device=self.device, dtype=torch.float32)
        key = torch.empty(B, R, device=self.device, dtype=torch.int32)
        plan.named.update(cls=cls, prob=prob, bbox_2d=b2, bbox_3d=b3, score_bits=key)
        assert NC == 4, "bundle kernel is written for 4 classes (bg + 3)"
        dst = plan.named["out_dst"] = [cls, prob, b2, b3]
        self._op(plan, "bundle_outputs", "bundle", lambda st: _hip.check(L.m3d_bundle_outputs(
            cls_pl.data_ptr(), box_pl.data_ptr(), dst[0].data_ptr(), dst[1].data_ptr(), dst[2].data_ptr(), dst[3].data_ptr(),
            key.data_ptr(), B, A, HW, st)), nbytes=B * R * (NC + 11 + 2 * NC + 4 + 7 + 1) * 4)
        plan.feat = (fh, fw)

        if plan.named.get("keys_by_select"):
            t0 = plan.named["score_bits_first_write_op"] + 1
            need = torch.zeros(B * HW, device=self.device, dtype=torch.uint8)
            rows = torch.zeros(B * HW, device=self.device, dtype=torch.int32)
            n_rows = torch.zeros(1, device=self.device, dtype=torch.int32)
            thresh = torch.zeros(B, device=self.device, dtype=torch.int32)
            nb = L.m3d_need_rows_workspace_bytes(B, HW)
            ws = torch.empty(nb, device=self.device, dtype=torch.uint8)
            plan.keep += [need, rows, n_rows, thresh, ws]
            plan.named.update(need=need, need_rows=rows, n_rows=n_rows, need_thresh=thresh)
            k_pre = plan.named["sparse_k"] = [min(int(self.conf.nms_topN_pre), R)]
            tail = [("need_rows", "select", 0.0, lambda st: _hip.check(L.m3d_need_rows(
                key.data_ptr(), B, A, HW, int(k_pre[0]), thresh.data_ptr(), need.data_ptr(), rows.data_ptr(), n_rows.data_ptr(),
                ws.data_ptr(), nb, st)), OpCost(B * R * 4 * 4))]
            dense_heads = {"bbox_x3d", "bbox_y3d"} if with_center else set()

            def rows_op(op):
                name, kind, flops, _, arr = op
                hs = name[:-len(".mlp")].split("+")
                mask = sum(1 << i for i, h in enumerate(hs) if h not in dense_heads)
                n = len(hs)
                return (name, kind, flops, lambda st: _hip.check(L.m3d_head_mlp_forward_rows(
                    arr, n, rows.data_ptr(), n_rows.data_ptr(), mask, st)), arr)

            def gated_op(op, p):
                om, kx, ky, mi = align_args[p]
                return op[:3] + (lambda st: _hip.check(L.m3d_align_offsets_gated(
                    sel_idx.data_ptr(), sel_prob.data_ptr(), 0.5, box_ptr(kx), box_ptr(ky), P["anchor_wh"].data_ptr(),
                    float(means[mi]), float(stds[mi]), float(means[mi + 1]), float(stds[mi + 1]), need.data_ptr(), om.ptr, om.cs,
                    B, A, HW, 11 * A * HW, st)), op[4])

            attend_rows = getattr(plan, "anab_attend", None) if ANAB_ROWS else None

            for op in plan.ops[t0:-1]:
                if op[1] == "head_mlp<3,64>":
                    op = rows_op(op)
                elif op[0] == "anab.attend" and attend_rows is not None:
                    op = op[:3] + (attend_rows(L.m3d_anab_attend_f32_rows, rows.data_ptr(), n_rows.data_ptr()), op[4])
                elif op[0] == "center_align2d.offsets":
                    op = gated_op(op, "center_align2d")
                tail.append(op)
            plan.tail, plan.tail_start = tail, t0
        return plan


    def _dla102_levels(self, plan, l1, maxpool):
        P = self.P
        B = l1.n
        b = "base.base"
        chs = BACKBONE_CHANNELS["dla102"]

        def bottleneck(p, x, res, out, stride):
            cb = P[p + ".conv1"].cout
            t1 = self._buf(plan, B, x.h, x.w, cb)
            self._conv(plan, p + ".conv1", P[p + ".conv1"], x, t1, 1, 0, act=1)
            t2 = self._buf(plan, B, out.h, out.w, cb)
            self._conv(plan, p + ".conv2", P[p + ".conv2"], t1, t2, stride, 1, act=1)
            self._conv(plan, p + ".conv3", P[p + ".conv3"], t2, out, 1, 0, act=1, res=res)

        def tree(p, levels, x, co, stride, out, level_root=False, root_dim=0, cat=None, pos=None, bottom=None):
            ci = x.c
            if root_dim == 0:
                root_dim = 2 * co
            if level_root:
                root_dim += ci
            h, w = x.h // stride, x.w // stride
            if cat is None:
                cat = self._buf(plan, B, h, w, root_dim + co * (levels - 1))
                pos = [2 * co]
            if stride == 1:
                bottom = x
            elif bottom is None:
                if level_root:
                    bottom = cat.slice(pos[0], ci)
                    pos[0] += ci
                else:
                    bottom = self._buf(plan, B, h, w, ci)
                maxpool(p + ".downsample", x, bottom)
            if levels == 1:
                if (p + ".project") in P:
                    res = self._buf(plan, B, h, w, co)
                    self._conv(plan, p + ".project", P[p + ".project"], bottom, res, 1, 0, act=0)
                else:
                    res = bottom
                assert cat.c == root_dim, (p, cat.c, root_dim)
                x2v, x1v = cat.slice(0, co), cat.slice(co, co)
                bottleneck(p + ".tree1", x, res, x1v, stride)
                bottleneck(p + ".tree2", x1v, x1v, x2v, 1)
                self._conv(plan, p + ".root", P[p + ".root"], cat, out, 1, 0, act=1, res=x2v)
                return
            x1 = cat.slice(pos[0], co)
            pos[0] += co
            tree(p + ".tree1", levels - 1, x, co, stride, x1, bottom=bottom if stride > 1 else None)
            tree(p + ".tree2", levels - 1, x1, co, 1, out, root_dim=root_dim + co, cat=cat, pos=pos)

        outs = []
        x = l1
        for lv in (2, 3, 4, 5):
            h, w = x.h // 2, x.w // 2
            out = self._buf(plan, B, h, w, chs[lv], name="level%d" % lv)
            tree("%s.level%d" % (b, lv), DLA102_LEVELS[lv], x, chs[lv], 2, out, level_root=lv > 2)
            outs.append(out)
            x = out
        return outs[1], outs[2], outs[3]

    def _anab_ops(self, plan, x, out, scale, shift, act, res_mode):
        L, P = self.L, self.P
        B, fh, fw = x.n, x.h, x.w
        HW = fh * fw
        ctot, off = self.anab_ctot, self.anab_off
        qkvs = self._buf(plan, B, fh, fw, ctot, _rup(ctot, 32))
        self._conv(plan, "anab.qkvs", P["anab.qkvs"], x, qkvs, 1, 0, act=0, sigmoid_from=off["s"], affine=False)
        items, bin_scale, bin_slots, bin_inv = self._anab_items(fh, fw)
        n_bins, max_slots = len(bin_scale), int(bin_slots.max())
        fused = FUSED_ANAB and ((self.cv == 128 and self.ck in (64, 128, 168)) or (self.cv == 256 and self.ck == 168)) \
            and HW % 128 == 0
        wave_ok = (not fused) and USE_ANAB_WAVE and USE_CONV_WAVE and HW % 32 == 0 and self.ck_pad % 32 == 0 and self.cv % 128 == 0
        nw = B * HW // 32
        wave_logits = wave_ok and nw * (_rup(n_bins, 128) // 128) >= 900
        keys_pad = _rup(n_bins, 128) if wave_logits else _rup(n_bins, 32)
        wave_pv = wave_ok and keys_pad % 32 == 0 and nw * (self.cv // 128) >= 900
        frag = (1 if wave_logits else 0) | (2 if wave_pv else 0)
        d_items = torch.from_numpy(items).to(self.device)
        d_bscale = torch.from_numpy(bin_scale).to(self.device)
        d_bslots = torch.from_numpy(bin_slots).to(self.device)
        d_binv = torch.from_numpy(bin_inv).to(self.device)
        ckv = self.ck + self.cv
        partial = torch.empty(B * n_bins * max_slots * ckv, device=self.device, dtype=torch.float32)
        khat = torch.zeros(B * keys_pad * self.ck_pad, device=self.device, dtype=torch.float32)
        vhatT = torch.zeros(B * self.cv * keys_pad, device=self.device, dtype=torch.float32)
        plan.keep += [d_items, d_bscale, d_bslots, d_binv, partial, khat, vhatT]
        plan.named["anab.khat"], plan.named["anab.vhatT"] = khat, vhatT
        kvv, sv = qkvs.slice(off["k"], ckv), qkvs.slice(off["s"], self.ns)
        if fh % 16 == 0 and fw % 16 == 0 and PSP_SIZES == (1, 4, 8, 16) and USE_ANAB_NESTED:
            scratch = torch.empty(L.m3d_anab_pool_nested_scratch_bytes(B, ckv) // 4, device=self.device, dtype=torch.float32)
            plan.keep.append(scratch)
            self._op(plan, "anab.pool_nested", "anab_pool", lambda st: _hip.check(L.m3d_anab_pool_nested(
                kvv.ptr, kvv.cs, sv.ptr, sv.cs, B, fh, fw, self.ck, self.cv, scratch.data_ptr(), khat.data_ptr(), keys_pad,
                self.ck_pad, vhatT.data_ptr(), frag, st)), nbytes=B * HW * (ckv + self.ns) * 4)
        else:
            self._op(plan, "anab.pool_partial", "anab_pool", lambda st: _hip.check(L.m3d_anab_pool_partial(
                kvv.ptr, kvv.cs, sv.ptr, sv.cs, d_items.data_ptr(), items.shape[0], d_bscale.data_ptr(), n_bins,
                partial.data_ptr(), max_slots, B, fh, fw, ckv, st)))
            self._op(plan, "anab.pool_finish", "anab_pool", lambda st: _hip.check(L.m3d_anab_pool_finish(
                partial.data_ptr(), d_bslots.data_ptr(), d_binv.data_ptr(), n_bins, max_slots, self.ck, self.cv,
                khat.data_ptr(), keys_pad, self.ck_pad, vhatT.data_ptr(), B, frag, st)))
        qv = qkvs.slice(off["q"], self.ck_pad)
        if fused:
            rp, rcs = (x.ptr, x.cs) if x is not None else (None, 0)
            sp = scale.data_ptr() if scale is not None else None
            hp = shift.data_ptr() if shift is not None else None

            def attend(fn, *row_list):
                return lambda st: _hip.check(fn(
                    qv.ptr, qv.cs, khat.data_ptr(), self.ck_pad, vhatT.data_ptr(), B, HW, self.ck, n_bins, keys_pad, self.cv, rp,
                    rcs, res_mode, sp, hp, 1 if act else 0, out.ptr, out.cs, *row_list, st))

            plan.anab_attend = attend
            self._op(plan, "anab.attend", "anab_attend", attend(L.m3d_anab_attend_f32),
                     flops=2.0 * B * HW * n_bins * (self.ck + self.cv),
                nbytes=B * HW * (self.ck + 3 * self.cv) * 4 + B * keys_pad * (self.ck + self.cv) * 4)
            return

        def image(v, i):
            return View(v.t, 1, v.h, v.w, v.c, v.cs, v.ptr + 4 * i * v.h * v.w * v.cs)

        def image_gemm(name, inp, outv, wgt, stride, frag, res=None, **kw):
            if frag or HW % 64 == 0:
                self._conv(plan, name, None, inp, outv, 1, 0, res=res, wgt_ptr=wgt.data_ptr(), wgt_img_stride=stride, kh=1, kw=1,
                           wgt_frag=frag, **kw)
                return
            sub = _Plan()
            for i in range(B):
                self._conv(sub, name, None, image(inp, i), image(outv, i), 1, 0, res=None if res is None else image(res, i),
                           wgt_ptr=wgt.data_ptr() + 4 * i * stride, kh=1, kw=1, **kw)
            assert len(sub.ops) == B and len({op[1] for op in sub.ops}) == 1, [op[:2] for op in sub.ops]
            plan.keep += sub.keep
            fns = [op[3] for op in sub.ops]
            plan.ops.append((name, sub.ops[0][1][:-1] + ",per_image>", sum(op[2] for op in sub.ops),
                             lambda st: [fn(st) for fn in fns], sub.ops[0][4]))

        logits = self._buf(plan, B, fh, fw, keys_pad)
        image_gemm("anab.logits", qv, logits, khat, keys_pad * self.ck_pad, wave_logits, act=0, affine=False, cout=n_bins,
                   cout_pad=keys_pad, cin_true=self.ck)
        self._op(plan, "anab.softmax", "softmax", lambda st: _hip.check(L.m3d_softmax_rows(
            logits.ptr, B * HW, n_bins, keys_pad, st)), nbytes=B * HW * n_bins * 8)
        image_gemm("anab.pv", logits, out, vhatT, self.cv * keys_pad, wave_pv, res=x, act=act, res_mode=res_mode, cout=self.cv,
                   cout_pad=_rup(self.cv, 32), scale=scale, shift=shift, cin_true=n_bins)

    @classmethod
    def anab_standalone(cls, mod, x):
        eng = cls.__new__(cls)
        eng.L, eng.device, eng.profile, eng.P = _hip.lib(), x.t.device, None, {}
        eng._pack_anab(eng.P, mod.query_conv.weight, mod.key_conv.weight, mod.value_conv.weight,
                       mod.spatial_conv.weight)
        plan = _Plan()
        out = eng._buf(plan, x.n, x.h, x.w, x.c)
        eng._anab_ops(plan, x, out, None, None, act=0, res_mode=0)
        eng.run_plan(plan)
        out.keep = plan
        return out

    @staticmethod
    def _anab_items(H, W):
        rchunk, cchunk = max(1, math.ceil(H / 16)), max(1, math.ceil(W / 4))
        items, bin_scale, bin_slots, bin_inv = [], [], [], []
        b = 0
        for si, s in enumerate(PSP_SIZES):
            for i in range(s):
                h0, h1 = (i * H) // s, -((-(i + 1) * H) // s)
                for j in range(s):
                    w0, w1 = (j * W) // s, -((-(j + 1) * W) // s)
                    slot = 0
                    for r0 in range(h0, h1, rchunk):
                        for c0 in range(w0, w1, cchunk):
                            items.append((b, r0, min(r0 + rchunk, h1), c0, min(c0 + cchunk, w1), slot))
                            slot += 1
                    bin_scale.append(si)
                    bin_slots.append(slot)
                    bin_inv.append(1.0 / ((h1 - h0) * (w1 - w0)))
                    b += 1
        return (np.asarray(items, dtype=np.int32), np.asarray(bin_scale, dtype=np.int32),
                np.asarray(bin_slots, dtype=np.int32), np.asarray(bin_inv, dtype=np.float32))

    def plan_for(self, B, H, W):
        key = (B, H, W)
        if key not in self.plans:
            if H % 32 or W % 32:
                raise RuntimeError("input H and W must be multiples of 32 (got %dx%d)" % (H, W))
            with torch.cuda.device(self.device):
                self.plans[key] = self._build_plan(B, H, W)
        return self.plans[key]

    def _run_to(self, plan, fresh):
        n = plan.named
        owned = (n["cls"], n["prob"], n["bbox_2d"], n["bbox_3d"])
        if not fresh:
            self.run_plan(plan)
            return owned
        dst = n["out_dst"]
        outs = [torch.empty_like(t) for t in owned]
        dst[:] = outs
        try:
            self.run_plan(plan)
        finally:
            dst[:] = owned
        return tuple(outs)

    def forward(self, x, fresh=False):
        if not x.is_cuda:
            raise NotImplementedError("M3DSSD HIP engine: input must be a ROCm device tensor")
        if x.device != self.device:
            raise RuntimeError("M3DSSD HIP engine on %s got an input on %s" % (self.device, x.device))
        B, _, H, W = x.shape
        plan = self.plan_for(B, H, W)
        x = x.contiguous()
        plan.named["input_ptr"][0] = x.data_ptr()
        plan.named["input_u8"][0] = 0
        return self._run_to(plan, fresh)

    def forward_u8(self, frames, size=None, fresh=False):
        if not frames.is_cuda or frames.dtype != torch.uint8 or frames.dim() != 4 or frames.shape[3] != 3:
            raise NotImplementedError("forward_u8: uint8 [B, h, w, 3] ROCm device tensor expected")
        H, W = (int(v) for v in (size if size is not None else self.conf.crop_size))
        B, h, w, _ = frames.shape
        if frames.device != self.device:
            raise RuntimeError("M3DSSD HIP engine on %s got frames on %s" % (self.device, frames.device))
        if h > H or w > W:
            raise RuntimeError("forward_u8: frame %dx%d does not fit the padded size %dx%d" % (h, w, H, W))
        plan = self.plan_for(B, H, W)
        frames = frames.contiguous()
        plan.named["input_u8"][:] = [frames.data_ptr(), h, w]
        try:
            return self._run_to(plan, fresh)
        finally:
            plan.named["input_u8"][0] = 0

    def forward_backbone(self, x):
        B, _, H, W = x.shape
        plan = self.plan_for(B, H, W)
        x = x.contiguous()
        plan.named["input_ptr"][0] = x.data_ptr()
        self.run_plan(plan)
        return plan.named["feats0"]

    def run_plan(self, plan, start=0, end=None, tail=False):
        with torch.cuda.device(self.device):
            if not tail:
                return self._run_plan(plan, start, end)
            if getattr(plan, "tail", None) is None:
                raise RuntimeError("run_plan(tail=True): this plan has no detection-only tail")
            if end != len(plan.ops) - 1 or not 0 <= start <= plan.tail_start:
                raise RuntimeError("run_plan(tail=True): ops [%r, %r) do not end in front of bundle_outputs (op %d) behind a start "
                                   "in [0, %d]" % (start, end, len(plan.ops) - 1, plan.tail_start))
            self._run_plan(plan, start, end, plan.ops[start:plan.tail_start] + plan.tail)

    def sparse_heads_default(self, plan, k):
        if getattr(plan, "tail", None) is None:
            return False
        hw = plan.feat[0] * plan.feat[1]
        return min(int(k), hw) <= SPARSE_HEADS_MAX_FRACTION * hw

    def _run_plan(self, plan, start, end, ops=None):
        st = _Stream.current(self.device)
        tail = ops is not None
        if not tail:
            ops = plan.ops[start:end]
        if self.profile is None:
            brs = [] if tail else [br for br in getattr(plan, "branches", ()) if lo_hi_contains(start, end, len(plan.ops), br)]
            if brs:
                lo, hi = start, (len(plan.ops) if end is None else end)
                main = torch.cuda.current_stream(self.device)
                if getattr(self, "_side", None) is None:
                    self._side = torch.cuda.Stream(self.device)
                side = self._side
                sst = ctypes.c_void_p(side.cuda_stream)
                forks = {br[0] for br in brs}
                joins = {br[2] for br in brs}
                on_side = set()
                for b0, b1, _ in brs:
                    on_side.update(range(b0, b1))
                for i in range(lo, hi):
                    if i in joins:
                        main.wait_stream(side)
                    if i in forks:
                        side.wait_stream(main)
                    plan.ops[i][3](sst if i in on_side else st)
                if hi in joins:
                    main.wait_stream(side)
                return
            for op in ops:
                op[3](st)
            return
        L = self.L
        evs = []
        for op in ops:
            if self.profile_kinds is not None and op[1] not in self.profile_kinds:
                op[3](st)
                continue
            e0, e1 = ctypes.c_void_p(), ctypes.c_void_p()
            _hip.check(L.m3d_event_create(ctypes.byref(e0)))
            _hip.check(L.m3d_event_create(ctypes.byref(e1)))
            _hip.check(L.m3d_event_record(e0, st))
            op[3](st)
            _hip.check(L.m3d_event_record(e1, st))
            evs.append((op, e0, e1))
        self._pending += evs

    def flush_profile(self):
        L = self.L
        for op, e0, e1 in self._pending:
            ms = ctypes.c_float()
            _hip.check(L.m3d_event_elapsed_ms(e0, e1, ctypes.byref(ms)))
            self.profile.append((op[0], op[1], op[2], ms.value))
            L.m3d_event_destroy(e0)
            L.m3d_event_destroy(e1)
        self._pending = []
```

Before: 1552 images/sec.

## Prefetch Winograd weights from conv_wave kernels and add in-launch split-K fixup

Lets conv_wave kernels that run shortly before a wino44 conv read the next conv's transformed weights into cache, replacing a standalone touch kernel launch. Also adds an optional wino44 split-K mode in which the last-arriving workgroup, chosen through atomic ticket counters, reduces the partial slices and applies the epilogue inside the same launch. The fixup path is off by default. The touch path adds extra loads at kernel start and could disturb cache contents needed by the carrier kernel.

```diff
diff --git a/include/m3dssd_hip.h b/include/m3dssd_hip.h
--- a/include/m3dssd_hip.h
+++ b/include/m3dssd_hip.h
@@ -54,6 +54,8 @@
 int m3d_conv_wave_splitk_plan(const m3d_conv_desc *d, int *splits, long long *ws_bytes);
 int m3d_conv_wave_forward(const m3d_conv_desc *d, m3d_stream_t stream);
 int m3d_conv_wave_forward_wgsplit(const m3d_conv_desc *d, m3d_stream_t stream);
+int m3d_conv_wave_forward_touch(const m3d_conv_desc *d, const void *touch, long long touch_bytes, m3d_stream_t stream);
+int m3d_conv_wave_forward_wgsplit_touch(const m3d_conv_desc *d, const void *touch, long long touch_bytes, m3d_stream_t stream);
 int m3d_conv_wave_wgsplit_width(const m3d_conv_desc *d, int *slices, int *width);
 
 int m3d_wino_conv3x3_forward(const m3d_conv_desc *d, m3d_stream_t stream);
@@ -66,6 +68,9 @@
 int m3d_wino44_kpair(const m3d_conv_desc *d);
 int m3d_wino44_splitk_plan(const m3d_conv_desc *d, int *splits, long long *ws_bytes);
 int m3d_wino44_conv3x3_forward_touch(const m3d_conv_desc *d, int nb, const void *touch, long long touch_bytes, m3d_stream_t stream);
+long long m3d_wino44_fixup_tickets_bytes(const m3d_conv_desc *d);
+int m3d_wino44_conv3x3_forward_fixup(const m3d_conv_desc *d, int nb, const void *touch, long long touch_bytes, void *tickets,
+                                     long long tickets_bytes, m3d_stream_t stream);
 
 int m3d_cache_touch(const void *p, long long bytes, m3d_stream_t stream);
 int m3d_upload_indirect(const void *const *src_slot, void *dst, long long bytes, m3d_stream_t stream);
diff --git a/m3dssd_amd/_hip.py b/m3dssd_amd/_hip.py
--- a/m3dssd_amd/_hip.py
+++ b/m3dssd_amd/_hip.py
@@ -147,6 +147,10 @@
     "m3d_wino44_conv3x3_forward_ex": (c_int, [ctypes.POINTER(ConvDesc), c_int, P]),
     "m3d_wino44_kpair": (c_int, [ctypes.POINTER(ConvDesc)]),
     "m3d_wino44_conv3x3_forward_touch": (c_int, [ctypes.POINTER(ConvDesc), c_int, P, c_ll, P]),
+    "m3d_wino44_fixup_tickets_bytes": (c_ll, [ctypes.POINTER(ConvDesc)]),
+    "m3d_wino44_conv3x3_forward_fixup": (c_int, [ctypes.POINTER(ConvDesc), c_int, P, c_ll, P, c_ll, P]),
+    "m3d_conv_wave_forward_touch": (c_int, [ctypes.POINTER(ConvDesc), P, c_ll, P]),
+    "m3d_conv_wave_forward_wgsplit_touch": (c_int, [ctypes.POINTER(ConvDesc), P, c_ll, P]),
     "m3d_cache_touch": (c_int, [P, c_ll, P]),
     "m3d_upload_indirect": (c_int, [P, P, c_ll, P]),
     "m3d_wino44_splitk_plan": (c_int, [ctypes.POINTER(ConvDesc), ctypes.POINTER(c_int), ctypes.POINTER(c_ll)]),
diff --git a/m3dssd_amd/csrc/common.h b/m3dssd_amd/csrc/common.h
--- a/m3dssd_amd/csrc/common.h
+++ b/m3dssd_amd/csrc/common.h
@@ -50,6 +50,10 @@
 {
     asm volatile("buffer_store_dwordx4 %0, %1, %2, %3 offen\n\ts_nop 1" : : "v"(v), "v"(voffset), "s"(r), "s"(soffset) : "memory");
 }
+__device__ __forceinline__ void buf_store_f32x4_sc1_nop(f32x4 v, __amdgpu_buffer_rsrc_t r, unsigned voffset, unsigned soffset)
+{
+    asm volatile("buffer_store_dwordx4 %0, %1, %2, %3 offen sc1\n\ts_nop 1" : : "v"(v), "v"(voffset), "s"(r), "s"(soffset) : "memory");
+}
 __device__ __forceinline__ void global_store_u32x4_nop(void *p, u32x4 v)
 {
     asm volatile("global_store_dwordx4 %0, %1, off\n\ts_nop 1" : : "v"(p), "v"(v) : "memory");
diff --git a/m3dssd_amd/csrc/dcn_wave.hip b/m3dssd_amd/csrc/dcn_wave.hip
--- a/m3dssd_amd/csrc/dcn_wave.hip
+++ b/m3dssd_amd/csrc/dcn_wave.hip
@@ -17,6 +17,8 @@
     float *ws;
     int splits, ss_per, base_waves;
     unsigned ws_bytes;
+    const char *touch;
+    int touch_lines;
 #ifdef CONV_TRACE
     long long *trace;
 #endif
@@ -51,6 +53,12 @@
         const int nblk = gridDim.x, bid = blockIdx.x;
         const int q = nblk >> 3, r = nblk & 7, xcd = bid & 7, loc = bid >> 3;
         blk = (xcd < r ? xcd * (q + 1) : r * (q + 1) + (xcd - r) * q) + loc;
+    }
+    float touched = 0.f;
+    if (a.touch) {
+        const long long nthr = (long long)gridDim.x * (64 * S);
+        for (long long i = (long long)blockIdx.x * (64 * S) + threadIdx.x; i < a.touch_lines; i += nthr)
+            touched = *reinterpret_cast<const volatile float *>(a.touch + (size_t)i * 128);
     }
     int split = wv;
     if (S == 1 && a.splits > 1) {
@@ -200,6 +208,7 @@
 #pragma unroll
     for (int j = 0; j < 4; ++j) rd_off[j] = (unsigned)(l31 * 32 + (((2 * j + h) ^ ((l31 >> 1) & 7)) * 4));
 
+    asm volatile("" : : "v"(touched));
     TRACE();
     for (int st = ss0; st < ss1; ++st) {
         TRACE();
@@ -512,9 +521,10 @@
     }
 }
 
-static int conv_wave_run(const m3d_conv_desc *d_, hipStream_t stream, bool wgsplit)
+static int conv_wave_run(const m3d_conv_desc *d_, hipStream_t stream, bool wgsplit, const void *touch = nullptr, long long touch_bytes = 0)
 {
     M3D_REQUIRE(d_ && d_->in && d_->wgt && d_->out, "conv_wave: null pointer");
+    M3D_REQUIRE(touch_bytes >= 0 && touch_bytes / 128 < (1ll << 31), "conv_wave: touch range");
     m3d_conv_desc dd = *d_;
     static float dummy;
     if (wgsplit) { dd.splitk_ws = &dummy; dd.splitk_ws_bytes = 0; }
@@ -555,6 +565,7 @@
     a.trace = g_conv_trace;
 #endif
     a.ws = nullptr; a.splits = 1; a.ss_per = ss_per; a.base_waves = waves; a.ws_bytes = 0;
+    a.touch = (touch && touch_bytes >= 128) ? (const char *)touch : nullptr; a.touch_lines = a.touch ? (int)(touch_bytes / 128) : 0;
     if (splits > 1 && wgsplit) {
         const int S = splits <= 2 ? 2 : (splits <= 4 ? 4 : 8);
         M3D_REQUIRE(splits <= 8, "conv_wave: %d K slices do not fit a workgroup", splits);
@@ -616,6 +627,11 @@
     return conv_wave_run(d, (hipStream_t)stream, false);
 }
 
+extern "C" int m3d_conv_wave_forward_touch(const m3d_conv_desc *d, const void *touch, long long touch_bytes, m3d_stream_t stream)
+{
+    return conv_wave_run(d, (hipStream_t)stream, false, touch, touch_bytes);
+}
+
 extern "C" int m3d_conv_wave_wgsplit_width(const m3d_conv_desc *d, int *slices, int *width)
 {
     M3D_REQUIRE(d && slices && width, "conv_wave_wgsplit_width: null pointer");
@@ -633,3 +649,8 @@
 {
     return conv_wave_run(d, (hipStream_t)stream, true);
 }
+
+extern "C" int m3d_conv_wave_forward_wgsplit_touch(const m3d_conv_desc *d, const void *touch, long long touch_bytes, m3d_stream_t stream)
+{
+    return conv_wave_run(d, (hipStream_t)stream, true, touch, touch_bytes);
+}
diff --git a/m3dssd_amd/csrc/wino44_conv.hip b/m3dssd_amd/csrc/wino44_conv.hip
--- a/m3dssd_amd/csrc/wino44_conv.hip
+++ b/m3dssd_amd/csrc/wino44_conv.hip
@@ -16,6 +16,11 @@
     long long ws_slice;
     const char *touch;
     int touch_lines;
+    int *tickets;
+    int fx_splits;
+    float *fx_out;
+    const float *fx_scale, *fx_shift, *fx_res;
+    int fx_out_cs, fx_res_cs, fx_cout, fx_act, fx_res_mode, fx_vec_out;
 #ifdef WINO_TRACE
     long long *trace;
 #endif
@@ -82,10 +87,11 @@
     y3 = d2 * 8.f + d1 + m5;
 }
 
-template <int NB, int OCC, int KS = 1>
+template <int NB, int OCC, int KS = 1, bool FIX = false>
 __global__ __launch_bounds__(256 * KS) __attribute__((amdgpu_waves_per_eu(OCC, OCC))) void wino44_kernel(const Wino44Args a)
 {
     static_assert(KS == 1 || (KS == 2 && NB == 1 && OCC == 2), "K-pair form: 64-channel waves, two per SIMD");
+    static_assert(!FIX || (NB == 1 && KS == 1), "in-launch reduction: the 64-channel, 256-thread split form");
     __shared__ __attribute__((aligned(16))) float Vs_all[KS * 2 * 36 * 256];
     __shared__ int pixb[16];
     const int tid8 = threadIdx.x, lane = tid8 & 63;
@@ -357,7 +363,8 @@
                     else if constexpr (MODE == 1) v = v * sc + sh + rvv[k];
                     else v = v * sc + sh;
                     v = __builtin_elementwise_max(v, v * slope);
-                    buf_store_f32x4_nop(v, rout, ovoff, osoff);
+                    if constexpr (FIX) buf_store_f32x4_sc1_nop(v, rout, ovoff, osoff);
+                    else buf_store_f32x4_nop(v, rout, ovoff, osoff);
                 }
             };
             if (!a.res) body(std::integral_constant<int, 0>{});
@@ -383,6 +390,85 @@
                     if (a.act == 1) v = fmaxf(v, v * M3D_LEAKY_SLOPE);
                     __builtin_amdgcn_raw_buffer_store_b32(__builtin_bit_cast(unsigned, v), rout, ovoff + em, osoff, 0);
                 }
+            }
+        }
+    }
+    if constexpr (FIX) {
+        asm volatile("s_waitcnt vmcnt(0)" ::: "memory");
+        __syncthreads();
+        int *const last_flag = reinterpret_cast<int *>(Vs_all);
+        if (tid8 == 0) {
+            int *const tk = a.tickets + by * (int)gridDim.x + bx;
+            const int drawn = __hip_atomic_fetch_add(tk, 1, __ATOMIC_RELAXED, __HIP_MEMORY_SCOPE_AGENT);
+            const int last = drawn == a.fx_splits - 1 ? 1 : 0;
+            if (last) {
+                __builtin_amdgcn_fence(__ATOMIC_ACQUIRE, "agent");
+                asm volatile("s_waitcnt vmcnt(0)" ::: "memory");
+                __hip_atomic_store(tk, 0, __ATOMIC_RELAXED, __HIP_MEMORY_SCOPE_AGENT);
+            }
+            *last_flag = last;
+        }
+        __syncthreads();
+        if (*last_flag) {
+            const int px = tid8 >> 4, co0 = by * 64 + (tid8 & 15) * 4;
+            const int pixo = (px >> 2) * a.W + (px & 3);
+            const float slope = a.fx_act == 1 ? M3D_LEAKY_SLOPE : 1.f;
+            auto reduce = [&](auto stag) __attribute__((always_inline)) {
+                constexpr int S = decltype(stag)::value;
+                constexpr int U = S >= 8 ? 4 : 8;
+                float sc[4], sh[4];
+#pragma unroll
+                for (int q = 0; q < 4; ++q) {
+                    const bool cok = co0 + q < a.fx_cout;
+                    sc[q] = (cok && a.fx_scale) ? a.fx_scale[co0 + q] : 1.f;
+                    sh[q] = (cok && a.fx_shift) ? a.fx_shift[co0 + q] : 0.f;
+                }
+                for (int k0 = 0; k0 < 16; k0 += U) {
+                    f32x4 part[U][S], rv[U];
+                    size_t m[U];
+                    int pb[U];
+#pragma unroll
+                    for (int u = 0; u < U; ++u) {
+                        pb[u] = pixb[k0 + u];
+                        m[u] = (size_t)((pb[u] >= 0 ? pb[u] : 0) + pixo);
+                        const float *p = a.out + m[u] * a.out_cs + co0;
+#pragma unroll
+                        for (int sl = 0; sl < S; ++sl) part[u][sl] = *reinterpret_cast<const f32x4 *>(p + sl * a.ws_slice);
+#pragma unroll
+                        for (int q = 0; q < 4; ++q)
+                            rv[u][q] = (a.fx_res && co0 + q < a.fx_cout) ? a.fx_res[m[u] * a.fx_res_cs + co0 + q] : 0.f;
+                    }
+#pragma unroll
+                    for (int u = 0; u < U; ++u) {
+                        if (pb[u] < 0) continue;
+                        f32x4 v = part[u][0];
+#pragma unroll
+                        for (int sl = 1; sl < S; ++sl) v = v + part[u][sl];
+                        f32x4 o;
+#pragma unroll
+                        for (int q = 0; q < 4; ++q) {
+                            float x = v[q];
+                            if (co0 + q < a.fx_cout) {
+                                x = conv_epi_affine(x, sc[q], sh[q], rv[u][q], a.fx_res != nullptr, a.fx_res_mode);
+                                x = conv_epi_act(x, false, slope);
+                            }
+                            o[q] = x;
+                        }
+                        float *op = a.fx_out + m[u] * a.fx_out_cs + co0;
+                        if (a.fx_vec_out && co0 + 3 < a.fx_cout) {
+                            *reinterpret_cast<f32x4 *>(op) = o;
+                        } else {
+#pragma unroll
+                            for (int q = 0; q < 4; ++q)
+                                if (co0 + q < a.fx_cout) op[q] = o[q];
+                        }
+                    }
+                }
+            };
+            if (co0 < a.fx_cout) {
+                if (a.fx_splits == 2) reduce(std::integral_constant<int, 2>{});
+                else if (a.fx_splits == 4) reduce(std::integral_constant<int, 4>{});
+                else reduce(std::integral_constant<int, 8>{});
             }
         }
     }
@@ -523,7 +609,8 @@
 static int w44_scratch_bytes()
 {
 #ifndef WINO_TRACE
-    static const int v = m3d_scratch_bytes(&wino44_kernel<1, 1>, &wino44_kernel<2, 1>, &wino44_kernel<1, 2>, &wino44_kernel<1, 2, 2>);
+    static const int v = m3d_scratch_bytes(&wino44_kernel<1, 1>, &wino44_kernel<2, 1>, &wino44_kernel<1, 2>, &wino44_kernel<1, 2, 2>,
+                                           &wino44_kernel<1, 2, 1, true>);
     return v < 0 ? 0 : v;
 #else
     return 0;
@@ -577,8 +664,16 @@
     return (w44_occ2() && wgs <= kpair_max && ns % 2 == 0 && ns / 2 >= 4) ? 1 : 0;
 }
 
-extern "C" int m3d_wino44_conv3x3_forward_touch(const m3d_conv_desc *d, int nb, const void *touch, long long touch_bytes,
-                                                m3d_stream_t stream)
+extern "C" long long m3d_wino44_fixup_tickets_bytes(const m3d_conv_desc *d)
+{
+    int splits = 1;
+    long long ws = 0;
+    if (!d || w44_split_nb() != 1 || m3d_wino44_splitk_plan(d, &splits, &ws) != M3D_OK || splits <= 1) return 0;
+    return (long long)cdiv(d->N * (d->H / 4) * (d->W / 4), 16) * (d->Cout_pad / 64) * 4;
+}
+
+static int w44_run(const m3d_conv_desc *d, int nb, const void *touch, long long touch_bytes, bool fixup, void *tickets,
+                   long long tickets_bytes, m3d_stream_t stream)
 {
     M3D_REQUIRE(d && d->in && d->wgt && d->out, "wino44: null pointer");
     M3D_REQUIRE(m3d_wino44_applicable(d), "wino44: 3x3 / stride 1 / pad 1, H %% 4 == W %% 4 == 0, Cin %% 16 == 0, Cout_pad %% 64 == 0 only");
@@ -597,6 +692,8 @@
     a.nsl = d->Cin / 16; a.ws_slice = 0;
     M3D_REQUIRE(touch_bytes >= 0 && touch_bytes / 128 < (1ll << 31), "wino44: touch range");
     a.touch = touch_bytes >= 128 ? (const char *)touch : nullptr; a.touch_lines = touch ? (int)(touch_bytes / 128) : 0;
+    a.tickets = nullptr; a.fx_splits = 1; a.fx_out = nullptr; a.fx_scale = a.fx_shift = a.fx_res = nullptr;
+    a.fx_out_cs = a.fx_res_cs = a.fx_cout = a.fx_act = a.fx_res_mode = a.fx_vec_out = 0;
 #ifdef WINO_TRACE
     a.trace = g_w44_trace;
 #endif
@@ -614,6 +711,22 @@
             a.out = d->splitk_ws; a.out_cs = d->Cout_pad; a.out_bytes = (unsigned)(pix * d->Cout_pad * 4);
             a.ws_slice = pix * d->Cout_pad; a.nsl = d->Cin / 16 / splits;
             a.scale = a.shift = a.res = nullptr; a.res_bytes = 0; a.act = 0; a.res_mode = 0; a.Cout = d->Cout_pad;
+            if (fixup) {
+                M3D_REQUIRE(w44_split_nb() == 1, "wino44 fixup: the 64-channel split form only (M3D_W44_SPLIT_NB = 1)");
+                const long long tneed = (long long)strips * (d->Cout_pad / 64) * 4;
+                M3D_REQUIRE(tickets && tickets_bytes >= tneed && ((uintptr_t)tickets & 3) == 0,
+                            "wino44 fixup: ticket buffer missing, too small (%lld of %lld bytes, see m3d_wino44_fixup_tickets_bytes) or "
+                            "misaligned", tickets_bytes, tneed);
+                M3D_REQUIRE(splits == 2 || splits == 4 || splits == 8, "wino44 fixup: %d K slices (the kernel reduces 2, 4 or 8)", splits);
+                a.tickets = (int *)tickets; a.fx_splits = splits;
+                a.fx_out = d->out; a.fx_scale = d->scale; a.fx_shift = d->shift; a.fx_res = d->res;
+                a.fx_out_cs = d->out_cs; a.fx_res_cs = d->res_cs; a.fx_cout = d->Cout; a.fx_act = d->act; a.fx_res_mode = d->res_mode;
+                a.fx_vec_out = (d->out_cs % 4 == 0) && (((uintptr_t)d->out & 15) == 0);
+                hipLaunchKernelGGL((wino44_kernel<1, 2, 1, true>), dim3(strips, d->Cout_pad / 64, splits), dim3(256), 0,
+                                   (hipStream_t)stream, a);
+                M3D_LAUNCH_CHECK();
+                return M3D_OK;
+            }
             if (w44_split_nb() == 1)
                 hipLaunchKernelGGL((wino44_kernel<1, 2>), dim3(strips, d->Cout_pad / 64, splits), dim3(256), 0, (hipStream_t)stream, a);
             else if (w44_split_nb() == 3) {
@@ -643,6 +756,18 @@
     return M3D_OK;
 }
 
+extern "C" int m3d_wino44_conv3x3_forward_touch(const m3d_conv_desc *d, int nb, const void *touch, long long touch_bytes,
+                                                m3d_stream_t stream)
+{
+    return w44_run(d, nb, touch, touch_bytes, false, nullptr, 0, stream);
+}
+
+extern "C" int m3d_wino44_conv3x3_forward_fixup(const m3d_conv_desc *d, int nb, const void *touch, long long touch_bytes, void *tickets,
+                                                long long tickets_bytes, m3d_stream_t stream)
+{
+    return w44_run(d, nb, touch, touch_bytes, true, tickets, tickets_bytes, stream);
+}
+
 extern "C" int m3d_wino44_conv3x3_forward_ex(const m3d_conv_desc *d, int nb, m3d_stream_t stream)
 {
     return m3d_wino44_conv3x3_forward_touch(d, nb, nullptr, 0, stream);
diff --git a/m3dssd_amd/engine.py b/m3dssd_amd/engine.py
--- a/m3dssd_amd/engine.py
+++ b/m3dssd_amd/engine.py
@@ -148,6 +148,8 @@
 WINO44_TOUCH = os.environ.get("M3D_WINO44_TOUCH", "1") != "0"
 WINO44_TOUCH_SPAN = int(os.environ.get("M3D_WINO44_TOUCH_SPAN", "2"))
 USE_WINO44_SPLITK = os.environ.get("M3D_WINO44_SPLITK", "1") != "0"
+USE_WINO44_FIXUP = os.environ.get("M3D_WINO44_FIXUP", "0") != "0"
+WINO44_TOUCH_WAVE = os.environ.get("M3D_WINO44_TOUCH_WAVE", "1") != "0"
 W44_SPLIT_NB = 2 if os.environ.get("M3D_W44_SPLIT_NB", "1") == "2" else 1
 W44_SPLIT_KPAIR = os.environ.get("M3D_W44_SPLIT_NB", "1") == "3"
 WINO44_MIN_WGS = int(os.environ.get("M3D_WINO44_MIN_WGS", "1000000"))
@@ -172,6 +174,9 @@
         self.keep = []
         self.named = {}
         self.w44_prev = None
+        self.wave_prev = None
+        self.w44_touch = {}
+        self.w44_tickets = {}
         self.branches = []
         self.tail = None
         self.tail_start = None
@@ -404,14 +409,31 @@
             nxt = {"ptr": None, "bytes": 0}
             if WINO44_TOUCH:
                 nbytes = u44.numel() * 4
+                carrier = None
                 if plan.w44_prev is not None and len(plan.ops) - plan.w44_prev[0] <= WINO44_TOUCH_SPAN:
-                    plan.w44_prev[1]["ptr"], plan.w44_prev[1]["bytes"] = u44.data_ptr(), nbytes
+                    carrier = plan.w44_prev
+                elif (WINO44_TOUCH_WAVE and plan.wave_prev is not None and plan.wave_prev[1]["ptr"] is None
+                      and len(plan.ops) - plan.wave_prev[0] <= WINO44_TOUCH_SPAN):
+                    carrier = plan.wave_prev
+                if carrier is not None:
+                    carrier[1]["ptr"], carrier[1]["bytes"] = u44.data_ptr(), nbytes
+                    plan.w44_touch[name] = carrier
                 else:
+                    plan.w44_touch[name] = (len(plan.ops), None)
                     plan.ops.append((name + ".touch", "touch", 0.0,
                                      lambda st: _hip.check(L.m3d_cache_touch(u44.data_ptr(), nbytes, st)), OpCost(nbytes)))
             plan.w44_prev = (len(plan.ops), nxt)
             kp = ",kpair" if (nb == 1 and ((ks44 == 1 and L.m3d_wino44_kpair(ref) == 1) or (ks44 > 1 and W44_SPLIT_KPAIR))) else ""
-            plan.ops.append((name, "wino44<16,%d%s%s>" % (16 * nb, ",splitk%d" % ks44 if ks44 > 1 else "", kp), flops,
+            kind = "wino44<16,%d%s%s>" % (16 * nb, ",splitk%d" % ks44 if ks44 > 1 else "", kp)
+            tbytes = L.m3d_wino44_fixup_tickets_bytes(ref) if (ks44 > 1 and USE_WINO44_FIXUP) else 0
+            if tbytes > 0:
+                tickets = torch.zeros(tbytes // 4, device=self.device, dtype=torch.int32)
+                plan.keep.append(tickets)
+                plan.w44_tickets[name] = tickets
+                plan.ops.append((name, kind, flops, lambda st: _hip.check(L.m3d_wino44_conv3x3_forward_fixup(
+                    ref, nb, nxt["ptr"], nxt["bytes"], tickets.data_ptr(), tbytes, st)), d))
+                return
+            plan.ops.append((name, kind, flops,
                              lambda st: _hip.check(L.m3d_wino44_conv3x3_forward_touch(ref, nb, nxt["ptr"], nxt["bytes"], st)), d))
             return
         if (pc is not None and wgt_ptr is None and getattr(pc, "wino", None) is not None and kh == 3 and kw == 3
@@ -437,7 +459,9 @@
             assert wgt_ptr is not None and planar is None and x.cs % 32 == 0 and x.ptr % 128 == 0, name
             if L.m3d_conv_wave_applicable(ref) <= 0:
                 raise RuntimeError("%s: fragment-ordered weights but the wave kernel does not apply" % name)
-            plan.ops.append((name, "conv_wave", flops_true, lambda st: _hip.check(L.m3d_conv_wave_forward(ref, st)), d))
+            wnxt = self._wave_carrier(plan)
+            plan.ops.append((name, "conv_wave", flops_true,
+                             lambda st: _hip.check(L.m3d_conv_wave_forward_touch(ref, wnxt["ptr"], wnxt["bytes"], st)), d))
             return
         if (pc is not None and wgt_ptr is None and planar is None and (USE_DCN_WAVE if om is not None else USE_CONV_WAVE)
                 and x.cs % 32 == 0 and x.ptr % 128 == 0 and pc.cin_pad == x.c):
@@ -447,7 +471,9 @@
                 frag = pc.frag()
                 d.wgt = frag.data_ptr()
                 kind = "conv_wave<%s>" % ",".join((["deform"] if om is not None else []) + ["wgsplit%d" % wsplits.value])
-                plan.ops.append((name, kind, flops_true, lambda st: _hip.check(L.m3d_conv_wave_forward_wgsplit(ref, st)), d))
+                wnxt = self._wave_carrier(plan)
+                plan.ops.append((name, kind, flops_true, lambda st: _hip.check(
+                    L.m3d_conv_wave_forward_wgsplit_touch(ref, wnxt["ptr"], wnxt["bytes"], st)), d))
                 return
             ws = None
             if wsplits.value > 1 and wbytes.value > 0:
@@ -461,7 +487,9 @@
                 kind = "conv_wave%s" % ("<%s>" % ",".join(
                     (["deform"] if om is not None else []) + (["splitk%d" % wsplits.value] if wsplits.value > 1 else []))
                     if (om is not None or wsplits.value > 1) else "")
-                plan.ops.append((name, kind, flops_true, lambda st: _hip.check(L.m3d_conv_wave_forward(ref, st)), d))
+                wnxt = self._wave_carrier(plan)
+                plan.ops.append((name, kind, flops_true,
+                                 lambda st: _hip.check(L.m3d_conv_wave_forward_touch(ref, wnxt["ptr"], wnxt["bytes"], st)), d))
                 return
             d.splitk_ws, d.splitk_ws_bytes = None, 0
         bm, bn, bk, grid = ctypes.c_int(), ctypes.c_int(), ctypes.c_int(), ctypes.c_int()
@@ -479,6 +507,12 @@
             cin_true = pc.cin if (pc is not None and wgt_ptr is None) else x.c
         flops = 2.0 * x.n * d.Ho * d.Wo * d.Cout * kh * kw * cin_true
         plan.ops.append((name, kind, flops, lambda st: _hip.check(L.m3d_conv2d_forward(ref, st)), d))
+
+    @staticmethod
+    def _wave_carrier(plan):
+        wnxt = {"ptr": None, "bytes": 0}
+        plan.wave_prev = (len(plan.ops), wnxt)
+        return wnxt
 
     def _op(self, plan, name, kind, fn, flops=0.0, nbytes=None):
         plan.ops.append((name, kind, float(flops), fn, OpCost(nbytes) if nbytes is not None else None))
```

Result: no change. 1560 images/sec (median of 6 runs) (+0.5%).
